# Owen-Liuyuxuan/FSNet

Hardware: AMD Instinct MI355X
Metric: training samples/sec (3-frame triplets) at 192x640, ResNet-18 depth+pose (higher is better)
Workload: dtype bf16; 1 GPU; KITTI Eigen-Zhou-shaped synthetic triplets, ResNet-18 depth+pose, 192x640, bf16, batch 12/GPU, full step (fwd+loss+bwd+clip35+Adam); inputs HBM-resident, no H2D in the timed region; global_batch=12, parallelism=dp1, encoder_pass=two chains (depth and pose encoder on two streams), autotune_steps=0, hipgraph_replays=557

## Files before the change

fsnet_amd/csrc/bn.hip:

```cpp
#include "bn_coeffs.h"
#include <algorithm>
#include <cstdlib>

namespace {

__device__ __forceinline__ int pow2_shift(int v) { return (v & (v - 1)) == 0 ? __ffs(v) - 1 : -1; }
__device__ __forceinline__ void split_vec(long i, int CG, int sh, int& cg, long& m) {
  if (sh >= 0) { cg = (int)(i & (CG - 1)); m = i >> sh; }
  else if (i < (1L << 31)) { const unsigned u = (unsigned)i, q = u / (unsigned)CG; cg = (int)(u - q * CG); m = q; }
  else { cg = (int)(i % CG); m = i / CG; }
}
__device__ __forceinline__ void split_row(long m, int H, int W, long& n, int& h, int& w) {
  if (m < (1L << 31)) {
    const unsigned u = (unsigned)m, q = u / (unsigned)W, nn = q / (unsigned)H;
    w = (int)(u - q * W); h = (int)(q - nn * H); n = nn;
  } else {
    w = (int)(m % W); const long q = m / W; h = (int)(q % H); n = q / H;
  }
}


constexpr int MAXC = 2048;

template <typename A> __host__ __device__ inline int bn_groups(const A& a) { return a.groups > 1 ? a.groups : 1; }
// ... 481 lines not shown
  }
  reduce_tail<V>(p, red, s1, s2, z, CG, cgl, pl, c, true);
}

template <typename T>
__global__ __launch_bounds__(256) void bn_bwd_apply_pool_kernel(const FsDual<FsBnBwdArgs, FsNoGeom> d) {
  extern __shared__ float bn_smem[];
  int G, z;
  const FsBnBwdArgs& p = bn_problem(d, G, z);
  constexpr int V = VecN<T>::N;
  const int C = p.C, CG = C / V, PL = 256 / CG;
  float* s_a = bn_smem; float* s_b = bn_smem + C; float* s_k = bn_smem + 2 * C;
  float* s_mean = bn_smem + 3 * C; float* s_istd = bn_smem + 4 * C; float* s_sh = bn_smem + 5 * C;
  const double* sums = p.sums + (long)z * FS_STAT_SLOTS * 2 * C;
  const double* sums_local = p.sums_local ? p.sums_local + (long)z * FS_STAT_SLOTS * 2 * C : nullptr;
  bn_bwd_coeffs(p, sums, sums_local, G, z, 0, C, true, bn_smem);
  const int cgl = threadIdx.x % CG, pl = threadIdx.x / CG, c = cgl * V;
  const T* __restrict__ yv = reinterpret_cast<const T*>(p.y);
  const T* __restrict__ xv = reinterpret_cast<const T*>(p.x);
  T* __restrict__ dx = reinterpret_cast<T*>(p.dx);
  const int H = p.H, W = p.W, Ho = H >> 1, Wo = W >> 1;
  const unsigned Qg = (unsigned)(p.M / G) / 4;
  for (unsigned q = blockIdx.x * PL + pl; q < Qg; q += gridDim.x * PL) {
    const unsigned qq = (unsigned)z * Qg + q, r = qq / (unsigned)Wo, nn = r / (unsigned)Ho;
    const int b = (int)(qq - r * Wo), a = (int)(r - nn * Ho);
    float g[4][V], x[4][V];
#pragma unroll
    for (int k = 0; k < 4; ++k) loadv<T>(xv + (((long)nn * H + 2 * a + (k >> 1)) * W + 2 * b + (k & 1)) * C + c, x[k]);
    pool_quad<T>(p, nn, a, b, c, g);
#pragma unroll
    for (int k = 0; k < 4; ++k) {
      const long m = ((long)nn * H + 2 * a + (k >> 1)) * W + 2 * b + (k & 1);
      pool_mask<T>(p, yv, m, c, x[k], s_k + c, s_sh + c, g[k]);
      float o[V];
#pragma unroll
      for (int j = 0; j < V; ++j) o[j] = bn_dx(g[k][j], x[k][j], s_mean[c + j], s_istd[c + j], s_k[c + j], s_a[c + j], s_b[c + j]);
      storev<T>(dx + m * C + c, o);
    }
  }
}

template <typename T, int CGB, bool POOL = false>
__global__ __launch_bounds__(256) void bn_bwd_reduce_kernel(const FsDual<FsBnBwdArgs, FsNoGeom> d) {
  int G, z;
  const FsBnBwdArgs& p = bn_problem(d, G, z);
  constexpr int V = VecN<T>::N;
  constexpr int PL = 256 / CGB;
  __shared__ float red[2][V][256];
  const int C = p.C, CG = C / V;
  const int cgl = threadIdx.x % CGB, pl = threadIdx.x / CGB;
  const int cg = blockIdx.y * CGB + cgl;
  const bool act = cg < CG;
  const int c = cg * V;
  const T* __restrict__ dout = reinterpret_cast<const T*>(p.dout);
  const T* __restrict__ yv = reinterpret_cast<const T*>(p.y);
  const T* __restrict__ xv = reinterpret_cast<const T*>(p.x);
  const long Mg = p.M / G, m_end = (z + 1) * Mg;
  float mean[V], istd[V], s1[V], s2[V];
#pragma unroll
  for (int j = 0; j < V; ++j) { mean[j] = act ? p.save_mean[z * C + c + j] : 0.f; istd[j] = act ? p.save_invstd[z * C + c + j] : 0.f; s1[j] = 0.f; s2[j] = 0.f; }
  if constexpr (POOL) {
    if (act) {
      float sc[V], sh[V];
#pragma unroll
      for (int j = 0; j < V; ++j) {
        sc[j] = p.gamma[c + j] * istd[j];
        sh[j] = (p.beta ? p.beta[c + j] : 0.f) - mean[j] * sc[j];
      }
      const long stride = (long)gridDim.x * PL;
      long m = z * Mg + (long)blockIdx.x * PL + pl;
      for (; m + stride < m_end; m += 2 * stride) {
        float g0[V], x0[V], g1[V], x1[V];
        loadv<T>(xv + m * C + c, x0);
        loadv<T>(xv + (m + stride) * C + c, x1);
        pool_grad<T>(p, m, c, g0);
        pool_grad<T>(p, m + stride, c, g1);
        pool_mask<T>(p, yv, m, c, x0, sc, sh, g0);
        pool_mask<T>(p, yv, m + stride, c, x1, sc, sh, g1);
#pragma unroll
        for (int j = 0; j < V; ++j) {
          s1[j] += g0[j] + g1[j];
          s2[j] += g0[j] * (x0[j] - mean[j]) * istd[j] + g1[j] * (x1[j] - mean[j]) * istd[j];
        }
      }
      for (; m < m_end; m += stride) {
        float g0[V], x0[V];
        loadv<T>(xv + m * C + c, x0);
        pool_grad<T>(p, m, c, g0);
        pool_mask<T>(p, yv, m, c, x0, sc, sh, g0);
#pragma unroll
        for (int j = 0; j < V; ++j) { s1[j] += g0[j]; s2[j] += g0[j] * (x0[j] - mean[j]) * istd[j]; }
      }
    }
  } else
  if (act) {
    const long stride = (long)gridDim.x * PL;
    long m = z * Mg + (long)blockIdx.x * PL + pl;
    if (dense_grad(p)) {
      const bool relu = p.relu != 0;
      long left = m < m_end ? (m_end - m + stride - 1) / stride : 0;
      long off = m * C + c;
      const long step = stride * C;
      uint4 d0, x0, y0, d1, x1, y1, d2, x2, y2;
      d0 = x0 = y0 = d1 = x1 = y1 = d2 = x2 = y2 = make_uint4(0, 0, 0, 0);
      auto req = [&](long o, uint4& dd, uint4& xx, uint4& yy) {
        dd = *reinterpret_cast<const uint4*>(dout + o); xx = *reinterpret_cast<const uint4*>(xv + o);
        if (relu) yy = *reinterpret_cast<const uint4*>(yv + o);
      };
      if constexpr (sizeof(T) == 2) {
        if (left > 0) req(off, d0, x0, y0);
        if (left > 1) req(off + step, d1, x1, y1);
        if (left > 2) req(off + 2 * step, d2, x2, y2);
        while (left > 0) {
          float g[V], xr[V];
          Unit<T>::unpack(d0, g); Unit<T>::unpack(x0, xr);
          if (relu) {
            float yy[V];
            Unit<T>::unpack(y0, yy);
#pragma unroll
            for (int j = 0; j < V; ++j) g[j] = yy[j] > 0.f ? g[j] : 0.f;
          }
          d0 = d1; x0 = x1; y0 = y1; d1 = d2; x1 = x2; y1 = y2;
          --left; off += step;
          if (left > 2) req(off + 2 * step, d2, x2, y2);
#pragma unroll
          for (int j = 0; j < V; ++j) { s1[j] += g[j]; s2[j] += g[j] * (xr[j] - mean[j]) * istd[j]; }
        }
        m = m_end;
      }
    }
    for (; m + stride < m_end; m += 2 * stride) {
      float g0[V], g1[V], x0[V], x1[V];
      masked_grad<T>(p, dout, yv, m, c, g0);
      masked_grad<T>(p, dout, yv, m + stride, c, g1);
      loadv<T>(xv + m * C + c, x0);
      loadv<T>(xv + (m + stride) * C + c, x1);
#pragma unroll
      for (int j = 0; j < V; ++j) {
        s1[j] += g0[j] + g1[j];
        s2[j] += g0[j] * (x0[j] - mean[j]) * istd[j] + g1[j] * (x1[j] - mean[j]) * istd[j];
      }
    }
    for (; m < m_end; m += stride) {
      float g0[V], x0[V];
      masked_grad<T>(p, dout, yv, m, c, g0);
      loadv<T>(xv + m * C + c, x0);
#pragma unroll
      for (int j = 0; j < V; ++j) { s1[j] += g0[j]; s2[j] += g0[j] * (x0[j] - mean[j]) * istd[j]; }
    }
  }
  reduce_tail<V>(p, red, s1, s2, z, CGB, cgl, pl, c, act);
}

template <typename T, bool POOL = false>
__global__ __launch_bounds__(256) void bn_bwd_apply_kernel(const FsDual<FsBnBwdArgs, FsNoGeom> d) {
  extern __shared__ float bn_smem[];
  int G, z;
  const FsBnBwdArgs& p = bn_problem(d, G, z);
  const int C = p.C;
  constexpr int V = VecN<T>::N;
  const int CG = C / V, cg_sh = pow2_shift(CG);
  const int SCG = gridDim.y > 1 ? 32 : CG, scg_sh = gridDim.y > 1 ? 5 : cg_sh;
  const int SC = SCG * V, c0 = (int)blockIdx.y * SC;
  float* s_a = bn_smem; float* s_b = bn_smem + SC; float* s_k = bn_smem + 2 * SC;
  float* s_mean = bn_smem + 3 * SC; float* s_istd = bn_smem + 4 * SC;
  const int Mg = p.M / G;
  const double* sums = p.sums + (long)z * FS_STAT_SLOTS * 2 * C;
  const double* sums_local = p.sums_local ? p.sums_local + (long)z * FS_STAT_SLOTS * 2 * C : nullptr;
  const T* __restrict__ dout = reinterpret_cast<const T*>(p.dout);
  const T* __restrict__ yv = reinterpret_cast<const T*>(p.y);
  const T* __restrict__ xv = reinterpret_cast<const T*>(p.x);
  const long total = (long)Mg * SCG;
  const long i0 = (long)blockIdx.x * 256 + threadIdx.x;
  float pg[V], px[V];
  if (i0 < total) {
    int cg; long m;
    split_vec(i0, SCG, scg_sh, cg, m);
    m += (long)z * Mg;
    if constexpr (POOL) pool_grad<T>(p, m, c0 + cg * V, pg);
    else masked_grad<T>(p, dout, yv, m, c0 + cg * V, pg);
    loadv<T>(xv + m * C + c0 + cg * V, px);
  }
  bn_bwd_coeffs(p, sums, sums_local, G, z, c0, SC, POOL, bn_smem);
  T* __restrict__ dx = reinterpret_cast<T*>(p.dx);
  T* __restrict__ gout = reinterpret_cast<T*>(p.g_out);
  const long stride = (long)gridDim.x * 256;
  if constexpr (!POOL) {
    if (scg_sh >= 0 && dense_grad(p)) {
      if (i0 >= total) return;
      const int cl = (int)(i0 & (SCG - 1)) * V;
      const long rows = stride >> scg_sh, step = rows * C;
      long off = ((long)z * Mg + (i0 >> scg_sh)) * C + c0 + cl;
      long left = (total - i0 + stride - 1) / stride;
      const bool relu = p.relu != 0;
      float ka[V], kb[V], kk[V], km[V], ki[V];
#pragma unroll
      for (int j = 0; j < V; ++j) { ka[j] = s_a[cl + j]; kb[j] = s_b[cl + j]; kk[j] = s_k[cl + j]; km[j] = s_mean[cl + j]; ki[j] = s_istd[cl + j]; }
      uint4 d1, x1, y1, d2, x2, y2;
      d1 = x1 = y1 = d2 = x2 = y2 = make_uint4(0, 0, 0, 0);
      if (left > 1) {
        d1 = *reinterpret_cast<const uint4*>(dout + off + step); x1 = *reinterpret_cast<const uint4*>(xv + off + step);
        if (relu) y1 = *reinterpret_cast<const uint4*>(yv + off + step);
      }
      if (left > 2) {
        d2 = *reinterpret_cast<const uint4*>(dout + off + 2 * step); x2 = *reinterpret_cast<const uint4*>(xv + off + 2 * step);
        if (relu) y2 = *reinterpret_cast<const uint4*>(yv + off + 2 * step);
      }
      float g[V], xr[V], o[V];
#pragma unroll
      for (int j = 0; j < V; ++j) { g[j] = pg[j]; xr[j] = px[j]; }
      for (;;) {
#pragma unroll
        for (int j = 0; j < V; ++j) o[j] = bn_dx(g[j], xr[j], km[j], ki[j], kk[j], ka[j], kb[j]);
        storev<T>(dx + off, o);
        if (gout) storev<T>(gout + off, g);
        if (--left == 0) break;
        off += step;
        Unit<T>::unpack(d1, g); Unit<T>::unpack(x1, xr);
        if (relu) {
          float yy[V];
          Unit<T>::unpack(y1, yy);
#pragma unroll
          for (int j = 0; j < V; ++j) g[j] = yy[j] > 0.f ? g[j] : 0.f;
        }
        d1 = d2; x1 = x2; y1 = y2;
        if (left > 2) {
          d2 = *reinterpret_cast<const uint4*>(dout + off + 2 * step); x2 = *reinterpret_cast<const uint4*>(xv + off + 2 * step);
          if (relu) y2 = *reinterpret_cast<const uint4*>(yv + off + 2 * step);
        }
      }
      return;
    }
  }
  for (long i = i0; i < total; i += stride) {
    int cg; long m;
    split_vec(i, SCG, scg_sh, cg, m);
    m += (long)z * Mg;
    const int cl = cg * V, c = c0 + cl;
    float g[V], xr[V], o[V];
#pragma unroll
    for (int j = 0; j < V; ++j) { g[j] = pg[j]; xr[j] = px[j]; }
    if (i + stride < total) {
      int cg2; long m2;
      split_vec(i + stride, SCG, scg_sh, cg2, m2);
      m2 += (long)z * Mg;
      if constexpr (POOL) pool_grad<T>(p, m2, c0 + cg2 * V, pg);
      else masked_grad<T>(p, dout, yv, m2, c0 + cg2 * V, pg);
      loadv<T>(xv + m2 * C + c0 + cg2 * V, px);
    }
    if constexpr (POOL) pool_mask<T>(p, yv, m, c, xr, s_k + cl, bn_smem + 5 * SC + cl, g);
#pragma unroll
    for (int j = 0; j < V; ++j) o[j] = bn_dx(g[j], xr[j], s_mean[cl + j], s_istd[cl + j], s_k[cl + j], s_a[cl + j], s_b[cl + j]);
    storev<T>(dx + m * C + c, o);
    if (gout) storev<T>(gout + m * C + c, g);
  }
}

int bn_slabs(int CG) { return (CG > 32 && (CG & (CG - 1)) == 0) ? CG / 32 : 1; }

bool bn_pool_quads(int CG) { return CG >= 1 && CG <= 32 && (CG & (CG - 1)) == 0; }

int grid_for(long items) {
  long b = (items + 255) / 256;
  const long cap = 512;
  if (b > cap) b = cap;
  if (b < 1) b = 1;
  return (int)b;
}

}

extern "C" int fs_bn_finalize(const FsBnApplyArgs* a, float* scale, float* shift, void* stream) {
  if (!a || !a->gamma || !a->beta || !a->save_mean || !a->save_invstd || !scale || !shift) return FS_EINVAL;
  if (!a->stats && (!a->running_mean || !a->running_var)) return FS_EINVAL;
  if (a->C <= 0 || a->C > MAXC || a->gamma2) return FS_EINVAL;
  const int G = bn_groups(*a);
  if (G > 1 && !a->stats) return FS_EINVAL;
  hipLaunchKernelGGL(bn_finalize_kernel, dim3((a->C + 255) / 256, G), dim3(256), 0, reinterpret_cast<hipStream_t>(stream),
                     *a, scale, shift);
  return fs_launch_status();
}

namespace {
int bn_apply_check(const FsBnApplyArgs* a) {
  if (!a || !a->x || (!a->y && !a->pool_y) || !a->gamma || !a->beta || !a->save_mean || !a->save_invstd) return FS_EINVAL;
  if (a->pool_y) {
    if (!a->pool_idx || !a->stats || a->res || a->gamma2 || a->pad_out || a->H <= 0 || a->W <= 0 || (a->H & 1) || (a->W & 1))
      return FS_EINVAL;
    if (a->M % (a->H * a->W) != 0 || (long)a->M * (a->C / 4) >= 0x7fffffffL) return FS_EINVAL;
    if (a->y && !dense(a->yN, a->yH, a->yW, a->H, a->W, a->C)) return FS_EINVAL;
  }
  if (!a->stats && (!a->running_mean || !a->running_var)) return FS_EINVAL;
  if (a->C % 8 != 0 || a->C > MAXC || a->M <= 0) return FS_EINVAL;
  if (a->gamma2 && (!a->res || !a->beta2 || !a->save_mean2 || !a->save_invstd2)) return FS_EINVAL;
  if (a->gamma2 && !a->stats2 && (!a->running_mean2 || !a->running_var2)) return FS_EINVAL;
  const int G = bn_groups(*a);
  if (a->M % G != 0 || (G > 1 && !a->stats)) return FS_EINVAL;
  return FS_OK;
}
int bn_bwd_check(const FsBnBwdArgs* a, bool apply) {
  if (!a || (!a->dout && !a->pool_dy) || !a->x || !a->sums || !a->save_mean || !a->save_invstd) return FS_EINVAL;
  if (apply && (!a->dx || !a->gamma)) return FS_EINVAL;
  if (a->C % 8 != 0 || a->C > MAXC || a->M <= 0) return FS_EINVAL;
  const int G = bn_groups(*a);
  if (a->M % G != 0) return FS_EINVAL;
  if (a->pool_dy) {
    if (!a->pool_idx || !a->gamma || a->fold || a->g_out || a->H <= 0 || a->W <= 0 || (a->H & 1) || (a->W & 1)) return FS_EINVAL;
    if (a->relu && !a->y && !a->beta) return FS_EINVAL;
    const long hw = (long)a->H * a->W;
    if (a->M % hw != 0 || (a->M / G) % hw != 0 || (long)a->M >= 0x7fffffffL) return FS_EINVAL;
    if (a->dout && !dense(a->gN, a->gH, a->gW, a->H, a->W, a->C)) return FS_EINVAL;
    if (a->y && !dense(a->yN, a->yH, a->yW, a->H, a->W, a->C)) return FS_EINVAL;
    return FS_OK;
  }
  if (a->relu && !a->y) return FS_EINVAL;
  return FS_OK;
}

template <typename A>
struct BnPair {
  FsDual<A, FsNoGeom> d;
  int G, G1;
  template <typename F> long larger(F extent) const {
    const long e = extent(d.a[0], G);
    return d.nprob == 2 ? std::max(e, (long)extent(d.a[1], G1)) : e;
  }
};
template <typename A, typename P, typename Check, typename Single>
bool bn_pair(const A* a, const A* b, P A::*pool, Check check, Single single, BnPair<A>& pr, int& status) {
  if ((status = check(a)) != FS_OK) return false;
  if (b) {
    if ((status = check(b)) != FS_OK) return false;
    const bool pooled = a->*pool != nullptr;
    if (b->C != a->C || pooled != (b->*pool != nullptr) || (pooled && (a->H != b->H || a->W != b->W))) {
      status = single(a);
      if (status == FS_OK) status = single(b);
      return false;
    }
  }
  pr.d.a[0] = *a; pr.d.a[1] = b ? *b : *a;
  pr.d.g[0].unused = pr.d.g[1].unused = 0;
  pr.d.nb0 = pr.G = bn_groups(*a);
  pr.d.nprob = b ? 2 : 1;
  pr.G1 = b ? bn_groups(*b) : 0;
  return true;
}

template <typename T> struct Elem { using type = T; };
template <typename F>
int by_dtype(int dtype, F launch) {
  if (dtype == FS_DTYPE_BF16) launch(Elem<bf16>{});
  else if (dtype == FS_DTYPE_F32) launch(Elem<float>{});
  else return FS_EINVAL;
  return fs_launch_status();
}
int dtype_lanes(int dtype) { return dtype == FS_DTYPE_BF16 ? 8 : 4; }

dim3 quad_grid(const long Qg, int CG, long cap, int groups) {
  return dim3((unsigned)std::min<long>((Qg + 256 / CG - 1) / (256 / CG), cap), 1, groups);
}
template <typename A> long quads_per_group(const A& x, int G) { return (x.M / G) / 4; }
template <typename A> long rows_per_group(const A& x, int G) { return x.M / G; }

template <int CGB>
int launch_reduce(const BnPair<FsBnBwdArgs>& pr, int dtype, hipStream_t st, int CG, long rows_per_block, long max_blocks) {
  const long Mg = pr.larger(rows_per_group<FsBnBwdArgs>);
  const dim3 grid((unsigned)std::min<long>((Mg + rows_per_block - 1) / rows_per_block, max_blocks), (CG + CGB - 1) / CGB,
                  pr.G + pr.G1);
  return by_dtype(dtype, [&](auto e) {
    using T = typename decltype(e)::type;
    if (pr.d.a[0].pool_dy) hipLaunchKernelGGL((bn_bwd_reduce_kernel<T, CGB, true>), grid, dim3(256), 0, st, pr.d);
    else hipLaunchKernelGGL((bn_bwd_reduce_kernel<T, CGB>), grid, dim3(256), 0, st, pr.d);
  });
}
}

extern "C" int fs_bn_apply2(const FsBnApplyArgs* a, const FsBnApplyArgs* b, int dtype, void* stream) {
  BnPair<FsBnApplyArgs> pr;
  int r;
  if (!bn_pair(a, b, &FsBnApplyArgs::pool_y, bn_apply_check,
               [&](const FsBnApplyArgs* x) { return fs_bn_apply2(x, nullptr, dtype, stream); }, pr, r)) return r;
  hipStream_t st = reinterpret_cast<hipStream_t>(stream);
  const int vec = dtype_lanes(dtype), nz = pr.G + pr.G1;
  const long items = pr.larger([&](const FsBnApplyArgs& x, int G) { return (long)(x.M / G) * (x.C / vec); });
  if (a->pool_y) {
    dim3 pgrid(std::min(2 * grid_for(items / 4), (int)((items / 4 + 255) / 256)), 1, nz);
    if (pgrid.x < 1) pgrid.x = 1;
    const unsigned plds = 2u * a->C * sizeof(float);
    return by_dtype(dtype, [&](auto e) {
      hipLaunchKernelGGL(bn_apply_pool_kernel<typename decltype(e)::type>, pgrid, dim3(256), plds, st, pr.d);
    });
  }
  const int nslab = bn_slabs(a->C / vec);
  dim3 grid(std::min(grid_for(items / nslab), std::max(32, grid_for(1L << 40) / nslab)), nslab, nz);
  const unsigned lds = ((a->gamma2 || (b && b->gamma2)) ? 4u : 2u) * (a->C / nslab) * sizeof(float);
  return by_dtype(dtype, [&](auto e) {
    hipLaunchKernelGGL(bn_apply_kernel<typename decltype(e)::type>, grid, dim3(256), lds, st, pr.d);
  });
}

extern "C" int fs_bn_apply(const FsBnApplyArgs* a, int dtype, void* stream) { return fs_bn_apply2(a, nullptr, dtype, stream); }

extern "C" int fs_bn_bwd_reduce2(const FsBnBwdArgs* a, const FsBnBwdArgs* b, int dtype, void* stream) {
  BnPair<FsBnBwdArgs> pr;
  int r;
  if (!bn_pair(a, b, &FsBnBwdArgs::pool_dy, [](const FsBnBwdArgs* x) { return bn_bwd_check(x, false); },
               [&](const FsBnBwdArgs* x) { return fs_bn_bwd_reduce2(x, nullptr, dtype, stream); }, pr, r)) return r;
  hipStream_t st = reinterpret_cast<hipStream_t>(stream);
  const int CG = a->C / dtype_lanes(dtype), nz = pr.G + pr.G1;
  if (a->pool_dy && bn_pool_quads(CG)) {
    const dim3 grid = quad_grid(pr.larger(quads_per_group<FsBnBwdArgs>), CG, 1024, nz);
    return by_dtype(dtype, [&](auto e) {
      hipLaunchKernelGGL(bn_bwd_reduce_pool_kernel<typename decltype(e)::type>, grid, dim3(256), 0, st, pr.d);
    });
  }
  const long wide_cap = std::max<long>(32, std::min<long>(512, 1024 / ((long)((CG + 31) / 32) * nz)));
  if (CG >= 32) return launch_reduce<32>(pr, dtype, st, CG, 16, wide_cap);
  if (CG >= 8) return launch_reduce<8>(pr, dtype, st, CG, 64, 1024);
  if (CG >= 4) return launch_reduce<4>(pr, dtype, st, CG, 128, 1024);
  return launch_reduce<2>(pr, dtype, st, CG, 256, 1024);
}

extern "C" int fs_bn_bwd_reduce(const FsBnBwdArgs* a, int dtype, void* stream) { return fs_bn_bwd_reduce2(a, nullptr, dtype, stream); }

extern "C" int fs_bn_bwd_apply2(const FsBnBwdArgs* a, const FsBnBwdArgs* b, int dtype, void* stream) {
  BnPair<FsBnBwdArgs> pr;
  int r;
  if (!bn_pair(a, b, &FsBnBwdArgs::pool_dy, [](const FsBnBwdArgs* x) { return bn_bwd_check(x, true); },
               [&](const FsBnBwdArgs* x) { return fs_bn_bwd_apply2(x, nullptr, dtype, stream); }, pr, r)) return r;
  hipStream_t st = reinterpret_cast<hipStream_t>(stream);
  const int vec = dtype_lanes(dtype), CG = a->C / vec, nz = pr.G + pr.G1;
  const int nslab = a->pool_dy ? 1 : bn_slabs(CG);
  const unsigned lds = (a->pool_dy ? 6u : 5u) * (a->C / nslab) * sizeof(float);
  if (a->pool_dy && bn_pool_quads(CG)) {
    const dim3 qgrid = quad_grid(pr.larger(quads_per_group<FsBnBwdArgs>), CG, 2048, nz);
    return by_dtype(dtype, [&](auto e) {
      hipLaunchKernelGGL(bn_bwd_apply_pool_kernel<typename decltype(e)::type>, qgrid, dim3(256), lds, st, pr.d);
    });
  }
  const long items = pr.larger([&](const FsBnBwdArgs& x, int G) { return (long)(x.M / G) * (x.C / vec); });
  dim3 grid(std::min(grid_for(items / nslab), std::max(32, grid_for(1L << 40) / nslab)), nslab, nz);
  return by_dtype(dtype, [&](auto e) {
    using T = typename decltype(e)::type;
    if (a->pool_dy) hipLaunchKernelGGL((bn_bwd_apply_kernel<T, true>), grid, dim3(256), lds, st, pr.d);
    else hipLaunchKernelGGL((bn_bwd_apply_kernel<T>), grid, dim3(256), lds, st, pr.d);
  });
}

extern "C" int fs_bn_bwd_apply(const FsBnBwdArgs* a, int dtype, void* stream) { return fs_bn_bwd_apply2(a, nullptr, dtype, stream); }
```

fsnet_amd/csrc/heads.hip:

```cpp
#include "common.h"
#include "fsnet_hip_internal.h"
#include <algorithm>

namespace {

template <int K>
__device__ __forceinline__ void head_fwd_row(const float* __restrict__ logits, const float* sb, float* __restrict__ depth,
                                             float* __restrict__ disp, long m, int Cl, float inv_rng, float max_d,
                                             float sc = 0.f, float min_d = 0.f) {
  float v[K];
  float mx = -INFINITY;
#pragma unroll
  for (int k = 0; k < K; k += 4) {
    float4 t = *reinterpret_cast<const float4*>(logits + m * Cl + k);
    v[k] = t.x; v[k + 1] = t.y; v[k + 2] = t.z; v[k + 3] = t.w;
  }
#pragma unroll
  for (int k = 0; k < K; ++k) { v[k] = fminf(fmaxf(v[k], -10.f), 10.f); mx = fmaxf(mx, v[k]); }
  float se = 0.f, sd = 0.f;
#pragma unroll
  for (int k = 0; k < K; ++k) { float e = expf(v[k] - mx); se += e; sd += e * sb[k]; }
  float d = sd / se;
  if (sc != 0.f) {
    d = d * sc;
    const float mn = min_d * sc, mx2 = max_d * sc;
    depth[m] = d;
    disp[m] = (1.f / d - 1.f / mx2) / (1.f / mn - 1.f / mx2);
    return;
  }
  depth[m] = d;
  disp[m] = (1.f / d - 1.f / max_d) * inv_rng;
}

template <int K, typename T>
__device__ __forceinline__ void head_bwd_row(const float* __restrict__ logits, const float* sb,
                                             const float* __restrict__ d_depth, const float* __restrict__ d_disp,
                                             T* __restrict__ dlogits, long m, int Cl, float inv_rng,
                                             float sc = 0.f, float min_d = 0.f, float max_d = 0.f) {
  float v[K], raw[K];
  float mx = -INFINITY;
#pragma unroll
  for (int k = 0; k < K; k += 4) {
    float4 t = *reinterpret_cast<const float4*>(logits + m * Cl + k);
    raw[k] = t.x; raw[k + 1] = t.y; raw[k + 2] = t.z; raw[k + 3] = t.w;
  }
#pragma unroll
  for (int k = 0; k < K; ++k) { v[k] = fminf(fmaxf(raw[k], -10.f), 10.f); mx = fmaxf(mx, v[k]); }
  float se = 0.f, sd = 0.f;
#pragma unroll
  for (int k = 0; k < K; ++k) { v[k] = expf(v[k] - mx); se += v[k]; sd += v[k] * sb[k]; }
  float d = sd / se;
  float g = (d_depth ? d_depth[m] : 0.f);
  if (sc != 0.f) {
    const float ds = d * sc;
    if (d_disp) g += d_disp[m] * (-1.f / (ds * ds)) / (1.f / (min_d * sc) - 1.f / (max_d * sc));
    g *= sc;
  } else if (d_disp) g += d_disp[m] * (-inv_rng / (d * d));
  float o[K];
#pragma unroll
  for (int k = 0; k < K; ++k) {
    float pk = v[k] / se;
    bool inside = raw[k] >= -10.f && raw[k] <= 10.f;
    o[k] = inside ? pk * (sb[k] - d) * g : 0.f;
  }
#pragma unroll
  for (int k = 0; k < K; k += 4) store4<T>(dlogits + m * Cl + k, &o[k]);
}

template <int K>
__global__ __launch_bounds__(256) void depth_head_fwd_kernel(const float* __restrict__ logits,
                                                             const float* __restrict__ bins, float* __restrict__ depth,
                                                             float* __restrict__ disp, long M, int Cl, float min_d,
                                                             float max_d) {
  __shared__ float sb[K];
  if (threadIdx.x < K) sb[threadIdx.x] = bins[threadIdx.x];
  __syncthreads();
  const float inv_rng = 1.f / (1.f / min_d - 1.f / max_d);
  for (long m = (long)blockIdx.x * 256 + threadIdx.x; m < M; m += (long)gridDim.x * 256)
    head_fwd_row<K>(logits, sb, depth, disp, m, Cl, inv_rng, max_d);
}

template <int K, typename T>
__global__ __launch_bounds__(256) void depth_head_bwd_kernel(const float* __restrict__ logits,
                                                             const float* __restrict__ bins,
                                                             const float* __restrict__ d_depth,
                                                             const float* __restrict__ d_disp, T* __restrict__ dlogits,
                                                             long M, int Cl, float min_d, float max_d) {
  __shared__ float sb[K];
  if (threadIdx.x < K) sb[threadIdx.x] = bins[threadIdx.x];
  __syncthreads();
  const float inv_rng = 1.f / (1.f / min_d - 1.f / max_d);
  for (long m = (long)blockIdx.x * 256 + threadIdx.x; m < M; m += (long)gridDim.x * 256)
    head_bwd_row<K, T>(logits, sb, d_depth, d_disp, dlogits, m, Cl, inv_rng);
}

struct HeadBlocks { int start[FS_HEAD_MAX + 1]; };

template <int K>
__global__ __launch_bounds__(256) void depth_head_fwd_multi_kernel(const FsHeadBatch hb, const HeadBlocks blk,
                                                                   const float* __restrict__ bins, int Cl, float min_d,
                                                                   float max_d) {
  __shared__ float sb[K];
  if (threadIdx.x < K) sb[threadIdx.x] = bins[threadIdx.x];
  __syncthreads();
  const float inv_rng = 1.f / (1.f / min_d - 1.f / max_d);
  int s = 0;
  while (s + 1 < hb.n && (int)blockIdx.x >= blk.start[s + 1]) ++s;
  const long nb = blk.start[s + 1] - blk.start[s], lb = blockIdx.x - blk.start[s];
  const long rows_img = hb.nimg > 0 ? hb.M[s] / hb.nimg : 0;
  for (long m = lb * 256 + threadIdx.x; m < hb.M[s]; m += nb * 256) {
    const float sc = hb.P2 ? hb.P2[(m / rows_img) * 12] / hb.base_fx : 0.f;
    head_fwd_row<K>(hb.logits[s], sb, hb.depth[s], hb.disp[s], m, Cl, inv_rng, max_d, sc, min_d);
  }
}

template <int K, typename T>
__global__ __launch_bounds__(256) void depth_head_bwd_multi_kernel(const FsHeadBatch hb, const HeadBlocks blk,
                                                                   const float* __restrict__ bins, int Cl, float min_d,
                                                                   float max_d) {
  __shared__ float sb[K];
  if (threadIdx.x < K) sb[threadIdx.x] = bins[threadIdx.x];
  __syncthreads();
  const float inv_rng = 1.f / (1.f / min_d - 1.f / max_d);
  int s = 0;
  while (s + 1 < hb.n && (int)blockIdx.x >= blk.start[s + 1]) ++s;
  const long nb = blk.start[s + 1] - blk.start[s], lb = blockIdx.x - blk.start[s];
  const long rows_img = hb.nimg > 0 ? hb.M[s] / hb.nimg : 0;
  for (long m = lb * 256 + threadIdx.x; m < hb.M[s]; m += nb * 256) {
    const float sc = hb.P2 ? hb.P2[(m / rows_img) * 12] / hb.base_fx : 0.f;
    head_bwd_row<K, T>(hb.logits[s], sb, hb.d_depth[s], hb.d_disp[s], reinterpret_cast<T*>(hb.dlogits[s]), m, Cl, inv_rng,
                       sc, min_d, max_d);
  }
}

struct Dual {
  float v; float d[6];
};
__device__ inline Dual dconst(float c) { Dual r; r.v = c; for (int i = 0; i < 6; ++i) r.d[i] = 0.f; return r; }
__device__ inline Dual dvar(float c, int i) { Dual r = dconst(c); r.d[i] = 1.f; return r; }
__device__ inline Dual operator+(const Dual& a, const Dual& b) { Dual r; r.v = a.v + b.v; for (int i = 0; i < 6; ++i) r.d[i] = a.d[i] + b.d[i]; return r; }
__device__ inline Dual operator-(const Dual& a, const Dual& b) { Dual r; r.v = a.v - b.v; for (int i = 0; i < 6; ++i) r.d[i] = a.d[i] - b.d[i]; return r; }
__device__ inline Dual operator*(const Dual& a, const Dual& b) { Dual r; r.v = a.v * b.v; for (int i = 0; i < 6; ++i) r.d[i] = a.d[i] * b.v + a.v * b.d[i]; return r; }
__device__ inline Dual operator/(const Dual& a, const Dual& b) { Dual r; r.v = a.v / b.v; for (int i = 0; i < 6; ++i) r.d[i] = (a.d[i] - r.v * b.d[i]) / b.v; return r; }
__device__ inline Dual dneg(const Dual& a) { Dual r; r.v = -a.v; for (int i = 0; i < 6; ++i) r.d[i] = -a.d[i]; return r; }
__device__ inline Dual dsqrt(const Dual& a) { Dual r; r.v = sqrtf(a.v); float k = r.v > 0.f ? 0.5f / r.v : 0.f; for (int i = 0; i < 6; ++i) r.d[i] = k * a.d[i]; return r; }
__device__ inline Dual dsin(const Dual& a) { Dual r; r.v = sinf(a.v); float k = cosf(a.v); for (int i = 0; i < 6; ++i) r.d[i] = k * a.d[i]; return r; }
__device__ inline Dual dcos(const Dual& a) { Dual r; r.v = cosf(a.v); float k = -sinf(a.v); for (int i = 0; i < 6; ++i) r.d[i] = k * a.d[i]; return r; }

__device__ inline void pose_matrix(const float in[6], int invert, Dual M[3][4]) {
  Dual vx = dvar(in[0], 0), vy = dvar(in[1], 1), vz = dvar(in[2], 2);
  Dual tx = dvar(in[3], 3), ty = dvar(in[4], 4), tz = dvar(in[5], 5);
  Dual angle = dsqrt(vx * vx + vy * vy + vz * vz);
  Dual den = angle + dconst(1e-7f);
  Dual x = vx / den, y = vy / den, z = vz / den;
  Dual ca = dcos(angle), sa = dsin(angle);
  Dual Cc = dconst(1.f) - ca;
  Dual xs = x * sa, ys = y * sa, zs = z * sa;
  Dual xC = x * Cc, yC = y * Cc, zC = z * Cc;
  Dual xyC = x * yC, yzC = y * zC, zxC = z * xC;
  Dual R[3][3];
  R[0][0] = x * xC + ca; R[0][1] = xyC - zs;    R[0][2] = zxC + ys;
  R[1][0] = xyC + zs;    R[1][1] = y * yC + ca; R[1][2] = yzC - xs;
  R[2][0] = zxC - ys;    R[2][1] = yzC + xs;    R[2][2] = z * zC + ca;
  if (!invert) {
    for (int i = 0; i < 3; ++i) for (int j = 0; j < 3; ++j) M[i][j] = R[i][j];
    M[0][3] = tx; M[1][3] = ty; M[2][3] = tz;
  } else {
    Dual nt[3] = {dneg(tx), dneg(ty), dneg(tz)};
    for (int i = 0; i < 3; ++i) {
      for (int j = 0; j < 3; ++j) M[i][j] = R[j][i];
      M[i][3] = R[0][i] * nt[0] + R[1][i] * nt[1] + R[2][i] * nt[2];
    }
  }
}

__global__ __launch_bounds__(64) void pose_tail_fwd_kernel(const float* __restrict__ x, float* __restrict__ axisangle,
                                                           float* __restrict__ translation, float* __restrict__ Tm,
                                                           int hw, int Cx, int nframes, int invert, float scale) {
  const int b = blockIdx.x, lane = threadIdx.x;
  const int nout = 6 * nframes;
  __shared__ float mean[64];
  for (int c = 0; c < nout; ++c) {
    float s = 0.f;
    for (int i = lane; i < hw; i += 64) s += x[((long)b * hw + i) * Cx + c];
    s = wave_sum(s);
    if (lane == 0) mean[c] = scale * (s / (float)hw);
  }
  __syncthreads();
  if (lane < nout) {
    int f = lane / 6, k = lane % 6;
    if (k < 3) axisangle[((long)b * nframes + f) * 3 + k] = mean[lane];
    else translation[((long)b * nframes + f) * 3 + (k - 3)] = mean[lane];
  }
  if (lane == 0) {
    float in[6] = {mean[0], mean[1], mean[2], mean[3], mean[4], mean[5]};
    Dual M[3][4];
    pose_matrix(in, invert, M);
    float* o = Tm + (long)b * 16;
    for (int i = 0; i < 3; ++i) for (int j = 0; j < 4; ++j) o[i * 4 + j] = M[i][j].v;
    o[12] = 0.f; o[13] = 0.f; o[14] = 0.f; o[15] = 1.f;
  }
}

template <typename T>
__global__ __launch_bounds__(64) void pose_tail_bwd_kernel(const float* __restrict__ x, const float* __restrict__ dT,
                                                           T* __restrict__ dx, int hw, int Cx, int nframes,
                                                           int invert, float scale) {
  const int b = blockIdx.x, lane = threadIdx.x;
  __shared__ float mean[8];
  __shared__ float gin[8];
  for (int c = 0; c < 6; ++c) {
    float s = 0.f;
    for (int i = lane; i < hw; i += 64) s += x[((long)b * hw + i) * Cx + c];
    s = wave_sum(s);
    if (lane == 0) mean[c] = scale * (s / (float)hw);
  }
  __syncthreads();
  if (lane == 0) {
    float in[6] = {mean[0], mean[1], mean[2], mean[3], mean[4], mean[5]};
    Dual M[3][4];
    pose_matrix(in, invert, M);
    const float* g = dT + (long)b * 16;
    for (int k = 0; k < 6; ++k) {
      float a = 0.f;
      for (int i = 0; i < 3; ++i) for (int j = 0; j < 4; ++j) a += g[i * 4 + j] * M[i][j].d[k];
      gin[k] = a * scale / (float)hw;
    }
  }
  __syncthreads();
  for (int i = lane; i < hw * Cx; i += 64) {
    int c = i % Cx;
    dx[(long)b * hw * Cx + i] = ElemTraits<T>::from_f(c < 6 ? gin[c] : 0.f);
  }
}

int grid_for(long items) {
  long b = (items + 255) / 256;
  return (int)std::max<long>(1, std::min<long>(b, 8192));
}

}

extern "C" int fs_depth_head_fwd(const float* logits, const float* bins, float* depth, float* disp, int64_t M, int K,
                                 int Cl, float min_depth, float max_depth, void* stream) {
  if (!logits || !bins || !depth || !disp || Cl < K) return FS_EINVAL;
  hipStream_t st = reinterpret_cast<hipStream_t>(stream);
  dim3 grid(grid_for(M));
  if (K == 16) hipLaunchKernelGGL(depth_head_fwd_kernel<16>, grid, dim3(256), 0, st, logits, bins, depth, disp, (long)M, Cl, min_depth, max_depth);
  else if (K == 32) hipLaunchKernelGGL(depth_head_fwd_kernel<32>, grid, dim3(256), 0, st, logits, bins, depth, disp, (long)M, Cl, min_depth, max_depth);
  else if (K == 64) hipLaunchKernelGGL(depth_head_fwd_kernel<64>, grid, dim3(256), 0, st, logits, bins, depth, disp, (long)M, Cl, min_depth, max_depth);
  else return FS_EINVAL;
  return fs_launch_status();
}

extern "C" int fs_depth_head_bwd(const float* logits, const float* bins, const float* d_depth, const float* d_disp,
                                 void* dlogits, int64_t M, int K, int Cl, float min_depth, float max_depth, int dtype,
                                 void* stream) {
  if (!logits || !bins || !dlogits || Cl < K) return FS_EINVAL;
  hipStream_t st = reinterpret_cast<hipStream_t>(stream);
  dim3 grid(grid_for(M));
#define FS_DH(KK, TT) hipLaunchKernelGGL((depth_head_bwd_kernel<KK, TT>), grid, dim3(256), 0, st, logits, bins, d_depth, d_disp, (TT*)dlogits, (long)M, Cl, min_depth, max_depth)
  if (dtype == FS_DTYPE_BF16) {
    if (K == 16) FS_DH(16, bf16); else if (K == 32) FS_DH(32, bf16); else if (K == 64) FS_DH(64, bf16); else return FS_EINVAL;
  } else if (dtype == FS_DTYPE_F32) {
    if (K == 16) FS_DH(16, float); else if (K == 32) FS_DH(32, float); else if (K == 64) FS_DH(64, float); else return FS_EINVAL;
  } else return FS_EINVAL;
#undef FS_DH
  return fs_launch_status();
}

namespace {
bool head_blocks(const FsHeadBatch* hb, bool bwd, HeadBlocks& blk, int& total) {
  if (!hb || hb->n < 1 || hb->n > FS_HEAD_MAX) return false;
  if (hb->P2 && (hb->nimg < 1 || !(hb->base_fx > 0.f))) return false;
  total = 0;
  for (int s = 0; s < hb->n; ++s) {
    if (!hb->logits[s] || hb->M[s] <= 0) return false;
    if (hb->P2 && hb->M[s] % hb->nimg != 0) return false;
    if (bwd ? !hb->dlogits[s] : (!hb->depth[s] || !hb->disp[s])) return false;
    blk.start[s] = total;
    total += grid_for(hb->M[s]);
  }
  blk.start[hb->n] = total;
  return true;
}
}

extern "C" int fs_depth_head_fwd_multi(const FsHeadBatch* hb, const float* bins, int K, int Cl, float min_depth,
                                       float max_depth, void* stream) {
  HeadBlocks blk; int total = 0;
  if (!bins || Cl < K || !head_blocks(hb, false, blk, total)) return FS_EINVAL;
  hipStream_t st = reinterpret_cast<hipStream_t>(stream);
  dim3 grid(total);
  if (K == 16) hipLaunchKernelGGL(depth_head_fwd_multi_kernel<16>, grid, dim3(256), 0, st, *hb, blk, bins, Cl, min_depth, max_depth);
  else if (K == 32) hipLaunchKernelGGL(depth_head_fwd_multi_kernel<32>, grid, dim3(256), 0, st, *hb, blk, bins, Cl, min_depth, max_depth);
  else if (K == 64) hipLaunchKernelGGL(depth_head_fwd_multi_kernel<64>, grid, dim3(256), 0, st, *hb, blk, bins, Cl, min_depth, max_depth);
  else return FS_EINVAL;
  return fs_launch_status();
}

extern "C" int fs_depth_head_bwd_multi(const FsHeadBatch* hb, const float* bins, int K, int Cl, float min_depth,
                                       float max_depth, int dtype, void* stream) {
  HeadBlocks blk; int total = 0;
  if (!bins || Cl < K || !head_blocks(hb, true, blk, total)) return FS_EINVAL;
  hipStream_t st = reinterpret_cast<hipStream_t>(stream);
  dim3 grid(total);
#define FS_DHM(KK, TT) hipLaunchKernelGGL((depth_head_bwd_multi_kernel<KK, TT>), grid, dim3(256), 0, st, *hb, blk, bins, Cl, min_depth, max_depth)
  if (dtype == FS_DTYPE_BF16) {
    if (K == 16) FS_DHM(16, bf16); else if (K == 32) FS_DHM(32, bf16); else if (K == 64) FS_DHM(64, bf16); else return FS_EINVAL;
  } else if (dtype == FS_DTYPE_F32) {
    if (K == 16) FS_DHM(16, float); else if (K == 32) FS_DHM(32, float); else if (K == 64) FS_DHM(64, float); else return FS_EINVAL;
  } else return FS_EINVAL;
#undef FS_DHM
  return fs_launch_status();
}

extern "C" int fs_pose_tail_fwd(const float* x, float* axisangle, float* translation, float* T, int B, int hw, int Cx,
                                int nframes, int invert, float scale, void* stream) {
  if (!x || !axisangle || !translation || !T || nframes < 1 || 6 * nframes > Cx || 6 * nframes > 64) return FS_EINVAL;
  hipStream_t st = reinterpret_cast<hipStream_t>(stream);
  hipLaunchKernelGGL(pose_tail_fwd_kernel, dim3(B), dim3(64), 0, st, x, axisangle, translation, T, hw, Cx, nframes, invert, scale);
  return fs_launch_status();
}

extern "C" int fs_pose_tail_bwd(const float* x, const float* dT, void* dx, int B, int hw, int Cx, int nframes,
                                int invert, float scale, int dtype, void* stream) {
  if (!x || !dT || !dx || 6 * nframes > Cx) return FS_EINVAL;
  hipStream_t st = reinterpret_cast<hipStream_t>(stream);
  if (dtype == FS_DTYPE_BF16) hipLaunchKernelGGL(pose_tail_bwd_kernel<bf16>, dim3(B), dim3(64), 0, st, x, dT, (bf16*)dx, hw, Cx, nframes, invert, scale);
  else if (dtype == FS_DTYPE_F32) hipLaunchKernelGGL(pose_tail_bwd_kernel<float>, dim3(B), dim3(64), 0, st, x, dT, (float*)dx, hw, Cx, nframes, invert, scale);
  else return FS_EINVAL;
  return fs_launch_status();
}
```

fsnet_amd/csrc/pool_upsample.hip:

```cpp
#include "common.h"
#include "fsnet_hip_internal.h"
#include <algorithm>

namespace {

struct FsPoolPair { const void* in1; void* out1; uint8_t* idx1; const void* add1; int n0; };

template <typename T>
__global__ __launch_bounds__(256) void maxpool_fwd_kernel(const T* __restrict__ x, T* __restrict__ y,
                                                          uint8_t* __restrict__ idx, int N, int H, int W, int C,
                                                          int Ho, int Wo, FsPoolPair pr) {
  constexpr int VN = VecN<T>::N;
  const int CG = C / VN;
  const long total = (long)N * Ho * Wo * CG;
  for (long i = (long)blockIdx.x * 256 + threadIdx.x; i < total; i += (long)gridDim.x * 256) {
    int cg = (int)(i % CG); long m = i / CG;
    int wo = (int)(m % Wo); long q = m / Wo; int ho = (int)(q % Ho); long n = q / Ho;
    const T* xs = x; T* ys = y; uint8_t* is = idx;
    if (n >= pr.n0) {
      n -= pr.n0; m -= (long)pr.n0 * Ho * Wo;
      xs = reinterpret_cast<const T*>(pr.in1); ys = reinterpret_cast<T*>(pr.out1); is = pr.idx1;
    }
    float best[VN];
    int bi[VN];
// ... 122 lines not shown
    if (i < ta) {
      int cg = (int)(i % CGa); long m = i / CGa;
      int x = (int)(m % w); long q = m / w; int y = (int)(q % h); long n = q / h;
      float acc[V];
#pragma unroll
      for (int j = 0; j < V; ++j) acc[j] = 0.f;
      for (int dy = 0; dy < 2; ++dy)
        for (int dx = 0; dx < 2; ++dx) {
          float g[V];
          fold_load<T, V>(dpad, n, 2 * y + dy, 2 * x + dx, H, W, C, cg * V, g);
#pragma unroll
          for (int j = 0; j < V; ++j) acc[j] += g[j];
        }
      stc<T, V>(da + m * Ca + cg * V, acc);
    } else {
      long k = i - ta;
      int cg = (int)(k % CGb); long m = k / CGb;
      int x = (int)(m % W); long q = m / W; int y = (int)(q % H); long n = q / H;
      float g[V];
      fold_load<T, V>(dpad, n, y, x, H, W, C, Ca + cg * V, g);
      stc<T, V>(db + m * Cb + cg * V, g);
    }
  }
}

template <typename T> __device__ __forceinline__ float round_to(float v);
template <> __device__ __forceinline__ float round_to<float>(float v) { return v; }
template <> __device__ __forceinline__ float round_to<bf16>(float v) { return bf16_bits_to_f(f_to_bf16_bits(v)); }

template <typename T, int V>
__global__ __launch_bounds__(256) void upcat_pad_bwd_bn_kernel(const T* __restrict__ dpad, T* __restrict__ da,
                                                               T* __restrict__ db, int N, int h, int w, int Ca, int Cb,
                                                               const T* __restrict__ yact, const T* __restrict__ xraw,
                                                               const float* __restrict__ mean,
                                                               const float* __restrict__ invstd, double* __restrict__ sums,
                                                               const int nA) {
  const int H = 2 * h, W = 2 * w, C = Ca + Cb;
  const int CGa = Ca / V, CGb = Cb / V;
  if ((int)blockIdx.x >= nA) {
    const long tb = (long)N * H * W * CGb;
    const int bx = (int)blockIdx.x - nA, nB = (int)gridDim.x - nA;
    for (long k = (long)bx * 256 + threadIdx.x; k < tb; k += (long)nB * 256) {
      int cg = (int)(k % CGb); long m = k / CGb;
      int x = (int)(m % W); long q = m / W; int y = (int)(q % H); long n = q / H;
      float g[V];
      fold_load<T, V>(dpad, n, y, x, H, W, C, Ca + cg * V, g);
      stc<T, V>(db + m * Cb + cg * V, g);
    }
    return;
  }
  __shared__ float red[2][V][256];
  const int cg = threadIdx.x % CGa, c = cg * V;
  float mu[V], is[V], s1[V], s2[V];
#pragma unroll
  for (int j = 0; j < V; ++j) { mu[j] = mean[c + j]; is[j] = invstd[c + j]; s1[j] = 0.f; s2[j] = 0.f; }
  const long ta = (long)N * h * w * CGa;
  for (long i = (long)blockIdx.x * 256 + threadIdx.x; i < ta; i += (long)nA * 256) {
    long m = i / CGa;
    int x = (int)(m % w); long q = m / w; int y = (int)(q % h); long n = q / h;
    float acc[V], yy[V], xr[V];
    ldc<T, V>(yact + m * Ca + c, yy);
    ldc<T, V>(xraw + m * Ca + c, xr);
#pragma unroll
    for (int j = 0; j < V; ++j) acc[j] = 0.f;
    for (int dy = 0; dy < 2; ++dy)
      for (int dx = 0; dx < 2; ++dx) {
        float g[V];
        fold_load<T, V>(dpad, n, 2 * y + dy, 2 * x + dx, H, W, C, c, g);
#pragma unroll
        for (int j = 0; j < V; ++j) acc[j] += g[j];
      }
#pragma unroll
    for (int j = 0; j < V; ++j) {
      const float g = yy[j] > 0.f ? round_to<T>(acc[j]) : 0.f;
      acc[j] = g;
      s1[j] += g; s2[j] += g * (xr[j] - mu[j]) * is[j];
    }
    stc<T, V>(da + m * Ca + c, acc);
  }
#pragma unroll
  for (int j = 0; j < V; ++j) { red[0][j][threadIdx.x] = s1[j]; red[1][j][threadIdx.x] = s2[j]; }
  __syncthreads();
  const int PL = 256 / CGa;
  for (int t = threadIdx.x; t < CGa * 2 * V; t += 256) {
    const int g2 = t % CGa, kj = t / CGa, kind = kj / V, j = kj % V;
    float a = 0.f;
    for (int k = 0; k < PL; ++k) a += red[kind][j][k * CGa + g2];
    double* sl = sums + (long)(blockIdx.x % FS_STAT_SLOTS) * 2 * Ca;
    atomicAdd(sl + kind * Ca + g2 * V + j, (double)a);
  }
}

template <typename T, int VL>
__device__ __forceinline__ void channel_sum_body(const T* __restrict__ x, float* __restrict__ out, long M, int C, int Creal,
                                                 int CGB, int bx, int by, int gx) {
  __shared__ float red[VL][256];
  const int CG = C / VL;
  const int PL = 256 / CGB;
  const int cgl = threadIdx.x % CGB, pl = threadIdx.x / CGB;
  const int cg = by * CGB + cgl;
  float s[VL];
#pragma unroll
  for (int j = 0; j < VL; ++j) s[j] = 0.f;
  auto ld = [&](long m, float* v) {
    if constexpr (VL == 4) load4<T>(x + m * C + cg * 4, v);
    else loadv<T>(x + m * C + cg * VL, v);
  };
  if (cg < CG) {
    const long stride = (long)gx * PL;
    long m = (long)bx * PL + pl;
    for (; m + 3 * stride < M; m += 4 * stride) {
      float v0[VL], v1[VL], v2[VL], v3[VL];
      ld(m, v0); ld(m + stride, v1); ld(m + 2 * stride, v2); ld(m + 3 * stride, v3);
#pragma unroll
      for (int j = 0; j < VL; ++j) s[j] += (v0[j] + v1[j]) + (v2[j] + v3[j]);
    }
    for (; m < M; m += stride) {
      float v0[VL];
      ld(m, v0);
#pragma unroll
      for (int j = 0; j < VL; ++j) s[j] += v0[j];
    }
  }
#pragma unroll
  for (int j = 0; j < VL; ++j) red[j][threadIdx.x] = s[j];
  __syncthreads();
  if (cg < CG) {
    for (int j = pl; j < VL; j += PL) {
      float a = 0.f;
      for (int k = 0; k < PL; ++k) a += red[j][k * CGB + cgl];
      if (cg * VL + j < Creal) atomicAdd(out + cg * VL + j, a);
    }
  }
}

template <typename T, int VL>
__global__ __launch_bounds__(256) void channel_sum_kernel(const T* __restrict__ x, float* __restrict__ out, long M,
                                                          int C, int Creal, int CGB) {
  channel_sum_body<T, VL>(x, out, M, C, Creal, CGB, (int)blockIdx.x, (int)blockIdx.y, (int)gridDim.x);
}

constexpr int FS_CSUM_MAX = 16;
struct CsumBatch { const void* x[FS_CSUM_MAX]; float* out[FS_CSUM_MAX]; long M[FS_CSUM_MAX]; int C[FS_CSUM_MAX], Creal[FS_CSUM_MAX],
                   CGB[FS_CSUM_MAX], gx[FS_CSUM_MAX], start[FS_CSUM_MAX + 1]; int n; };
template <typename T, int VL>
__global__ __launch_bounds__(256) void channel_sum_multi_kernel(const CsumBatch c) {
  int k = 0;
  while (k + 1 < c.n && (int)blockIdx.x >= c.start[k + 1]) ++k;
  const int lb = (int)blockIdx.x - c.start[k];
  const int gx = c.gx[k];
  channel_sum_body<T, VL>(reinterpret_cast<const T*>(c.x[k]), c.out[k], c.M[k], c.C[k], c.Creal[k], c.CGB[k], lb % gx, lb / gx, gx);
}

int grid_for(long items) {
  long b = (items + 255) / 256;
  return (int)std::max<long>(1, std::min<long>(b, 8192));
}

}

#define DISPATCH(KERNEL, GRID, ...)                                                                   \
  if (dtype == FS_DTYPE_BF16) hipLaunchKernelGGL(KERNEL<bf16>, GRID, dim3(256), 0, st, __VA_ARGS__);  \
  else if (dtype == FS_DTYPE_F32) hipLaunchKernelGGL(KERNEL<float>, GRID, dim3(256), 0, st, __VA_ARGS__); \
  else return FS_EINVAL;

extern "C" int fs_maxpool_fwd2(const void* x, void* y, uint8_t* idx, int N, const void* x1, void* y1, uint8_t* idx1, int N1,
                               int H, int W, int C, int dtype, void* stream) {
  const int vn = dtype == FS_DTYPE_BF16 ? 8 : 4;
  if (!x || !y || !idx || C % vn != 0 || N <= 0) return FS_EINVAL;
  if (x1 && (!y1 || !idx1 || N1 <= 0)) return FS_EINVAL;
  if (!x1) N1 = 0;
  hipStream_t st = reinterpret_cast<hipStream_t>(stream);
  int Ho = (H + 2 - 3) / 2 + 1, Wo = (W + 2 - 3) / 2 + 1;
  const FsPoolPair pr{x1, y1, idx1, nullptr, x1 ? N : 0x7fffffff};
  dim3 grid(grid_for((long)(N + N1) * Ho * Wo * (C / vn)));
  if (dtype == FS_DTYPE_BF16)
    hipLaunchKernelGGL(maxpool_fwd_kernel<bf16>, grid, dim3(256), 0, st, (const bf16*)x, (bf16*)y, idx, N + N1, H, W, C, Ho, Wo, pr);
  else if (dtype == FS_DTYPE_F32)
    hipLaunchKernelGGL(maxpool_fwd_kernel<float>, grid, dim3(256), 0, st, (const float*)x, (float*)y, idx, N + N1, H, W, C, Ho, Wo, pr);
  else return FS_EINVAL;
  return fs_launch_status();
}

extern "C" int fs_maxpool_fwd(const void* x, void* y, uint8_t* idx, int N, int H, int W, int C, int dtype,
                              void* stream) {
  return fs_maxpool_fwd2(x, y, idx, N, nullptr, nullptr, nullptr, 0, H, W, C, dtype, stream);
}

extern "C" int fs_maxpool_bwd2(const void* dy, const uint8_t* idx, const void* addend, void* dx, int N, const void* dy1,
                               const uint8_t* idx1, const void* addend1, void* dx1, int N1, int H, int W, int C, int dtype,
                               void* stream) {
  const int vn = dtype == FS_DTYPE_BF16 ? 8 : 4;
  if (!dy || !dx || !idx || C % vn != 0 || N <= 0) return FS_EINVAL;
  if (dy1 && (!dx1 || !idx1 || N1 <= 0)) return FS_EINVAL;
  if (!dy1) N1 = 0;
  hipStream_t st = reinterpret_cast<hipStream_t>(stream);
  int Ho = (H + 2 - 3) / 2 + 1, Wo = (W + 2 - 3) / 2 + 1;
  const FsPoolPair pr{dy1, dx1, const_cast<uint8_t*>(idx1), addend1, dy1 ? N : 0x7fffffff};
  dim3 grid(grid_for((long)(N + N1) * H * W * (C / vn)));
  if (dtype == FS_DTYPE_BF16)
    hipLaunchKernelGGL(maxpool_bwd_kernel<bf16>, grid, dim3(256), 0, st, (const bf16*)dy, idx, (const bf16*)addend, (bf16*)dx, N + N1, H, W, C, Ho, Wo, pr);
  else if (dtype == FS_DTYPE_F32)
    hipLaunchKernelGGL(maxpool_bwd_kernel<float>, grid, dim3(256), 0, st, (const float*)dy, idx, (const float*)addend, (float*)dx, N + N1, H, W, C, Ho, Wo, pr);
  else return FS_EINVAL;
  return fs_launch_status();
}

extern "C" int fs_maxpool_bwd(const void* dy, const uint8_t* idx, const void* addend, void* dx, int N, int H, int W,
                              int C, int dtype, void* stream) {
  return fs_maxpool_bwd2(dy, idx, addend, dx, N, nullptr, nullptr, nullptr, nullptr, 0, H, W, C, dtype, stream);
}

extern "C" int fs_upcat_pad_fwd(const void* a, const void* b, void* out, int N, int h, int w, int Ca, int Cb,
                                int dtype, void* stream) {
  if (!a || !out || (Cb > 0 && !b) || Ca % 4 != 0 || Cb % 4 != 0) return FS_EINVAL;
  hipStream_t st = reinterpret_cast<hipStream_t>(stream);
  const bool wide = dtype == FS_DTYPE_BF16 && Ca % 8 == 0 && Cb % 8 == 0;
  dim3 grid(grid_for((long)N * (2 * h + 2) * (2 * w + 2) * ((Ca + Cb) / (wide ? 8 : 4))));
  if (wide)
    hipLaunchKernelGGL((upcat_pad_fwd_kernel<bf16, 8>), grid, dim3(256), 0, st, (const bf16*)a, (const bf16*)b, (bf16*)out, N, h, w, Ca, Cb);
  else if (dtype == FS_DTYPE_BF16)
    hipLaunchKernelGGL((upcat_pad_fwd_kernel<bf16, 4>), grid, dim3(256), 0, st, (const bf16*)a, (const bf16*)b, (bf16*)out, N, h, w, Ca, Cb);
  else if (dtype == FS_DTYPE_F32)
    hipLaunchKernelGGL((upcat_pad_fwd_kernel<float, 4>), grid, dim3(256), 0, st, (const float*)a, (const float*)b, (float*)out, N, h, w, Ca, Cb);
  else return FS_EINVAL;
  return fs_launch_status();
}

extern "C" int fs_upcat_pad_bwd(const void* dpad, void* da, void* db, int N, int h, int w, int Ca, int Cb, int dtype,
                                void* stream) {
  if (!dpad || !da || (Cb > 0 && !db) || Ca % 4 != 0 || Cb % 4 != 0) return FS_EINVAL;
  hipStream_t st = reinterpret_cast<hipStream_t>(stream);
  const bool wide = dtype == FS_DTYPE_BF16 && Ca % 8 == 0 && Cb % 8 == 0;
  const int V = wide ? 8 : 4;
  dim3 grid(grid_for((long)N * h * w * (Ca / V) + (long)N * 4 * h * w * (Cb / V)));
  if (wide)
    hipLaunchKernelGGL((upcat_pad_bwd_kernel<bf16, 8>), grid, dim3(256), 0, st, (const bf16*)dpad, (bf16*)da, (bf16*)db, N, h, w, Ca, Cb);
  else if (dtype == FS_DTYPE_BF16)
    hipLaunchKernelGGL((upcat_pad_bwd_kernel<bf16, 4>), grid, dim3(256), 0, st, (const bf16*)dpad, (bf16*)da, (bf16*)db, N, h, w, Ca, Cb);
  else if (dtype == FS_DTYPE_F32)
    hipLaunchKernelGGL((upcat_pad_bwd_kernel<float, 4>), grid, dim3(256), 0, st, (const float*)dpad, (float*)da, (float*)db, N, h, w, Ca, Cb);
  else return FS_EINVAL;
  return fs_launch_status();
}

extern "C" int fs_upcat_pad_bwd_bn(const void* dpad, void* da, void* db, int N, int h, int w, int Ca, int Cb, const void* y,
                                   const void* x, const float* mean, const float* invstd, double* sums, int dtype,
                                   void* stream) {
  if (!dpad || !da || (Cb > 0 && !db) || !y || !x || !mean || !invstd || !sums || Ca % 4 != 0 || Cb % 4 != 0 || Ca <= 0)
    return FS_EINVAL;
  hipStream_t st = reinterpret_cast<hipStream_t>(stream);
  const bool wide = dtype == FS_DTYPE_BF16 && Ca % 8 == 0 && Cb % 8 == 0;
  const int V = wide ? 8 : 4;
  const int CGa = Ca / V;
  if (CGa > 256 || 256 % CGa != 0) return FS_EINVAL;
  const long ta = (long)N * h * w * CGa, tb = (long)N * 4 * h * w * (Cb / V);
  const int nA = (int)std::max<long>(1, std::min<long>((ta + 511) / 512, 512));
  const int nB = Cb > 0 ? grid_for(tb) : 0;
  dim3 grid(nA + nB);
  if (wide)
    hipLaunchKernelGGL((upcat_pad_bwd_bn_kernel<bf16, 8>), grid, dim3(256), 0, st, (const bf16*)dpad, (bf16*)da, (bf16*)db, N, h, w, Ca, Cb,
                       (const bf16*)y, (const bf16*)x, mean, invstd, sums, nA);
  else if (dtype == FS_DTYPE_BF16)
    hipLaunchKernelGGL((upcat_pad_bwd_bn_kernel<bf16, 4>), grid, dim3(256), 0, st, (const bf16*)dpad, (bf16*)da, (bf16*)db, N, h, w, Ca, Cb,
                       (const bf16*)y, (const bf16*)x, mean, invstd, sums, nA);
  else if (dtype == FS_DTYPE_F32)
    hipLaunchKernelGGL((upcat_pad_bwd_bn_kernel<float, 4>), grid, dim3(256), 0, st, (const float*)dpad, (float*)da, (float*)db, N, h, w, Ca, Cb,
                       (const float*)y, (const float*)x, mean, invstd, sums, nA);
  else return FS_EINVAL;
  return fs_launch_status();
}

extern "C" int fs_channel_sum_multi(const void* const* x, float* const* out, const int64_t* M, const int32_t* C,
                                    const int32_t* Creal, int n, int dtype, void* stream) {
  if (!x || !out || !M || !C || !Creal || n < 1 || n > FS_CSUM_MAX) return FS_EINVAL;
  const int es = dtype == FS_DTYPE_BF16 ? 2 : 4;
  const int VW = 16 / es;
  CsumBatch b;
  int blocks = 0;
  bool wide = true;
  for (int i = 0; i < n; ++i) {
    if (!x[i] || !out[i] || C[i] % 4 != 0 || M[i] <= 0) return FS_EINVAL;
    wide = wide && (C[i] % VW == 0 && VW != 4);
  }
  const int VL = wide ? VW : 4;
  for (int i = 0; i < n; ++i) {
    const int CG = C[i] / VL;
    int CGB = 1;
    while (CGB < CG && CGB < 64) CGB <<= 1;
    const int PL = 256 / CGB;
    const int gx = (int)std::max<long>(1, std::min<long>((M[i] + 4L * PL - 1) / (4L * PL), 256));
    const int gy = (CG + CGB - 1) / CGB;
    b.x[i] = x[i]; b.out[i] = out[i]; b.M[i] = M[i]; b.C[i] = C[i]; b.Creal[i] = Creal[i]; b.CGB[i] = CGB; b.gx[i] = gx;
    b.start[i] = blocks;
    blocks += gx * gy;
  }
  b.start[n] = blocks; b.n = n;
  hipStream_t st = reinterpret_cast<hipStream_t>(stream);
  if (dtype == FS_DTYPE_BF16) {
    if (wide) hipLaunchKernelGGL((channel_sum_multi_kernel<bf16, 8>), dim3(blocks), dim3(256), 0, st, b);
    else hipLaunchKernelGGL((channel_sum_multi_kernel<bf16, 4>), dim3(blocks), dim3(256), 0, st, b);
  } else if (dtype == FS_DTYPE_F32) {
    hipLaunchKernelGGL((channel_sum_multi_kernel<float, 4>), dim3(blocks), dim3(256), 0, st, b);
  } else return FS_EINVAL;
  return fs_launch_status();
}

extern "C" int fs_channel_sum(const void* x, float* out, int64_t M, int C, int Creal, int dtype, void* stream) {
  if (!x || !out || C % 4 != 0 || M <= 0) return FS_EINVAL;
  hipStream_t st = reinterpret_cast<hipStream_t>(stream);
  const int es = dtype == FS_DTYPE_BF16 ? 2 : 4;
// ... 17 lines not shown
```

fsnet_amd/engine/nets.py:

```python
import os
import weakref

import torch

from ..hip import ops
from ..hip.binding import raw_stream
from ..hip.conv import ConvOp, run_specs
from .runtime import RT, grad_of

STAT_SLOTS = ops.STAT_SLOTS
FOLD_BN = os.environ.get("FSNET_AMD_BN_FOLD", "1").strip().lower() not in ("0", "off", "false", "no")


class StatsPool:

    def __init__(self, device, capacity=1 << 21):
        self.buf = torch.zeros(capacity, dtype=torch.float64, device=device)
        self.off = 0
        self.high = 0
        self.dirty = False
        self.epoch = -1
        ops.register_prezero(self, StatsPool._prezero, device)

    def _prezero(self):
        self.off = 0
        self.epoch = ops.PREZERO_EPOCH[0]
        if not self.dirty:
            return []
        self.dirty = False
        return [self.buf[:self.high]]

    def reset(self):
        if self.dirty:
            self.buf[:self.high].zero_()
            self.dirty = False
        self.off = 0

    def span(self, a, b):
        if a is None or b is None or a.untyped_storage().data_ptr() != self.buf.untyped_storage().data_ptr() \
                or b.untyped_storage().data_ptr() != self.buf.untyped_storage().data_ptr():
            return None
        oa, ob = a.storage_offset(), b.storage_offset()
        if oa + a.numel() != ob:
            return None
        return self.buf[oa:ob + b.numel()]

    def take(self, C, groups=1):
        n = groups * STAT_SLOTS * 2 * C
        shape = (STAT_SLOTS, 2, C) if groups == 1 else (groups, STAT_SLOTS, 2, C)
        if self.off + n > self.buf.numel():
            return torch.zeros(shape, dtype=torch.float64, device=self.buf.device)
        v = self.buf[self.off:self.off + n].view(shape)
        self.off += n
        self.high = max(self.high, self.off)
        self.dirty = True
        return v


_PENDING_JOIN = set()
_PENDING_KEEP = []
_DEFERRED = {}
_CALLBACK_QUEUED = [None]
_ACTIVE_CHAINS = set()


_STREAM_OBJS = {}


def _current_stream(device=None):
    from ..hip.binding import raw_stream
    idx = torch.cuda.current_device() if device is None or device.index is None else device.index
    key = (idx, raw_stream(idx))
    s = _STREAM_OBJS.get(key)
    if s is None:
        s = _STREAM_OBJS[key] = torch.cuda.current_stream(idx)
    return s


def _run_param_grads(*item, bias_later=None):
    lanes = item[1] if item[0] == "lanes" else [item]
    run_specs([op.wgrad_spec(dc, x, gw, pro=pro) for (op, dc, x, gw, gb, nb, pro) in lanes])
    for (op, dc, x, gw, gb, nb, pro) in lanes:
        if gb is not None:
            if bias_later is not None:
                bias_later.append((dc, gb, nb))
            else:
                ops.channel_sum(dc, gb, nb)


_INLINE_BIAS = {}


def _inline_bias_list(dev):
    if not (RT.dp is not None and dev.type == "cuda"):
        return None
    cur = _current_stream(dev)
    return _INLINE_BIAS.setdefault(cur.cuda_stream, (cur, []))[1]


def drop_inline_bias():
    for ent in _INLINE_BIAS.values():
        ent[1].clear()


def flush_inline_bias(cur=None):
    for key in ([cur.cuda_stream] if cur is not None else list(_INLINE_BIAS.keys())):
        ent = _INLINE_BIAS.get(key)
        if ent is None or not ent[1]:
            continue
        chain, items = ent
        with torch.cuda.stream(chain):
            ops.channel_sum_multi(items)
        items.clear()


def accumulate_param_grads_multi(cls, ops_, dcs, xs, pros):
    lanes = []
    for cl, op, dc, x, pro in zip(cls, ops_, dcs, xs, pros):
        gw = grad_of(cl.m.weight)
        gb = grad_of(cl.m.bias) if cl.m.bias is not None else None
        if gw is None:
            if gb is not None:
                ops.channel_sum(dc, gb, cl.m.bias.numel())
            continue
        lanes.append((op, dc, x, gw, gb, cl.m.bias.numel() if gb is not None else 0, pro))
    if not lanes:
        return
    item = lanes[0] if len(lanes) == 1 else ("lanes", lanes)
    dc0 = lanes[0][1]
    mode = RT.wgrad_streams if (dc0.is_cuda and RT.overlap and (RT.dp is None or RT.dp.wgrad_companions)) else 0
    if mode:
        _defer_param_grads(_current_stream(dc0.device), item)
        return
    _run_param_grads(*item, bias_later=_inline_bias_list(dc0.device))


def _drop_stale():
    if _CALLBACK_QUEUED[0] is not None and _CALLBACK_QUEUED[0] != torch._C._current_graph_task_id():
        for stale in _DEFERRED.values():
            stale[1].clear()
        _ACTIVE_CHAINS.clear()
        _LATE.clear()
        _AT_END.clear()


def _defer_param_grads(cur, item):
    _drop_stale()
    ent = _DEFERRED.get(cur.cuda_stream)
    if ent is None:
        ent = _DEFERRED[cur.cuda_stream] = (cur, [])
    ent[1].append(item)
    _ACTIVE_CHAINS.add(cur.cuda_stream)
    _queue_end_of_backward()
    if len(ent[1]) >= (RT.wgrad_flush_even if RT.even_chains else RT.wgrad_flush):
        flush_deferred(cur)


_BATCH_NO = [0]
HANDOVERS = {"late": 0, "shared": 0}
_ENCODER_END = [False]
_AT_END = []
_LATE = []
_CHAINS_BEGUN = [None, []]


def _issue_batch(chain, ws, mine, ev=None):
    if ev is None:
        ws.wait_stream(chain)
    else:
        ws.wait_event(ev)
    with torch.cuda.stream(ws):
        if RT._marks is not None:
            _BATCH_NO[0] += 1
            tag = "wg.%s.%d" % ("pose" if RT.is_side(chain) else "depth", _BATCH_NO[0])
            RT.mark(tag + ".start")
        sums = []
        for it in mine:
            _run_param_grads(*it, bias_later=sums)
        if sums:
            ops.channel_sum_multi(sums)
        if RT._marks is not None:
            RT.mark(tag + ".end(%d)" % len(mine))
    _PENDING_JOIN.add((chain, ws))


def _position(chain):
    import ctypes as C
    from ..hip.binding import check, lib
    tok = C.c_ulonglong(0)
    check(lib.fs_capture_position(C.c_void_p(chain.cuda_stream), C.byref(tok)), "fs_capture_position")
    return tok.value


def issue_late(chain=None, advanced=False):
    if not _LATE:
        return
    mine = [e for e in _LATE if chain is None or e[1].cuda_stream == chain.cuda_stream]
    if advanced and mine:
        here = _position(chain)
        mine = [e for e in mine if e[4] != here]
    if not mine:
        return
    ids = {id(e) for e in mine}
    _LATE[:] = [e for e in _LATE if id(e) not in ids]
    for ent in mine:
        if ent[2] is None:
            ent[3](ent[0])
        else:
            _issue_batch(ent[1], ent[2], ent[3], ev=ent[0])


def issue_advanced(device):
    if _LATE:
        _drop_stale()
        issue_late(_current_stream(device), advanced=True)


def late_call(chain, fn):
    if not (RT.wgrad_late and torch.cuda.is_current_stream_capturing() and torch._C._current_graph_task_id() >= 0):
        return False
    _drop_stale()
    issue_late(chain, advanced=True)
    ev = torch.cuda.Event()
    ev.record(chain)
    _LATE.append((ev, chain, None, fn, _position(chain)))
    _queue_end_of_backward()
    return True


def flush_deferred(cur=None, now=False):
    late = (RT.wgrad_late and not now and torch.cuda.is_current_stream_capturing()
            and torch._C._current_graph_task_id() >= 0)
    for key in ([cur.cuda_stream] if cur is not None else list(_DEFERRED.keys())):
        ent = _DEFERRED.get(key)
        if ent is None or not ent[1]:
            continue
        chain, items = ent
        issue_late(chain, advanced=late)
        ws = RT.companion_stream(chain.device, chain)[1]
        ev = None
        capturing = late or torch.cuda.is_current_stream_capturing()
        if capturing:
            ev = torch.cuda.Event()
            ev.record(chain)
        mine = list(items)
        if (RT.wgrad_balance and RT.even_chains and capturing and _ENCODER_END[0] and RT.dp is None and not RT.is_side(chain)
                and len(items) >= 2 and torch._C._current_graph_task_id() >= 0):
            side = RT.side_stream(chain.device)
            others = [side, RT.companion_stream(chain.device, side)[1]][:RT.wgrad_balance]
            n = 1 + len(others)
            _AT_END.append((ev, chain, [(o, items[1 + k::n]) for k, o in enumerate(others)]))
            HANDOVERS["shared"] += 1
            mine = items[0::n]
        if late:
            _LATE.append((ev, chain, ws, mine, _position(chain)))
            HANDOVERS["late"] += 1
        else:
            _issue_batch(chain, ws, mine, ev=ev)
        _PENDING_KEEP.extend(items)
        ent[1].clear()
    if not late:
        issue_late(cur)


def chain_ends(device):
    if (RT.wgrad_late and (_LATE or _AT_END) and device.type == "cuda" and torch.cuda.is_current_stream_capturing()
            and torch._C._current_graph_task_id() >= 0):
        RT.nop(device)
        issue_late(_current_stream(device))


def chain_begins(device):
    if not (RT.wgrad_late and device.type == "cuda" and RT.overlap and RT.wgrad_streams
            and torch.cuda.is_current_stream_capturing()):
        return
    task = torch._C._current_graph_task_id()
    if task < 0:
        return
    _drop_stale()
    if _CHAINS_BEGUN[0] != task:
        _CHAINS_BEGUN[0], _CHAINS_BEGUN[1] = task, []
    cur = _current_stream(device)
    begun = _CHAINS_BEGUN[1]
    if any(c.cuda_stream == cur.cuda_stream for c in begun):
        return
    begun.append(cur)
    if len(begun) == 2:
        first = begun[0]
        ws = RT.companion_stream(device, first)[1]
        ws.wait_stream(cur)
        with torch.cuda.stream(ws):
            RT.nop(device)
        _PENDING_JOIN.add((first, ws))


def _end_of_backward():
    _CALLBACK_QUEUED[0] = None
    flush_tail()
    flush_inline_bias()
    flush_deferred(now=True)
    for ev, chain, parts in _AT_END:
        for ws, mine in parts:
            if mine:
                _issue_batch(chain, ws, mine, ev=ev)
    _AT_END.clear()
    _ENCODER_END[0] = False
    _ACTIVE_CHAINS.clear()
    _BATCH_NO[0] = 0
    join_companions()


def join_companions():
    if not _PENDING_JOIN:
        return
    if torch.cuda.is_current_stream_capturing():
        return
    for cur, ws in list(_PENDING_JOIN):
        cur.wait_stream(ws)
    _PENDING_JOIN.clear()
    _PENDING_KEEP.clear()


_TAIL_SINK = [None]
_TAIL = []


def _queue_end_of_backward():
    task = torch._C._current_graph_task_id()
    if _CALLBACK_QUEUED[0] != task:
        torch.autograd.Variable._execution_engine.queue_callback(_end_of_backward)
        _CALLBACK_QUEUED[0] = task


def defer_to_tail(items, runner, device):
    if _TAIL and _CALLBACK_QUEUED[0] != torch._C._current_graph_task_id():
        _TAIL.clear()
    chain = _current_stream(device)
    ev = torch.cuda.Event()
    ev.record(chain)
    runner.tail_pending = True
    _TAIL.append((ev, chain, items, runner))
    _queue_end_of_backward()


def flush_tail():
    for ev, chain, items, runner in _TAIL:
        side = RT.side_stream(chain.device)
        side.wait_event(ev)
        with torch.cuda.stream(side):
            sums = []
            for it in items:
                _run_param_grads(*it, bias_later=sums)
            if sums:
                ops.channel_sum_multi(sums)
            runner.tail_pending = False
            if RT.dp is not None and runner.m._pending == 0:
                RT.dp.grads_ready(runner.m)
        _PENDING_JOIN.add((chain, side))
        _PENDING_KEEP.extend(items)
    _TAIL.clear()


def pending_companions():
    return {ws for _, ws in _PENDING_JOIN}


def join_companions_final():
    flush_inline_bias()
    flush_deferred(now=True)
    issue_late()
    if not _PENDING_JOIN:
        return
    cur = torch.cuda.current_stream()
    for ws in {ws for _, ws in _PENDING_JOIN}:
        cur.wait_stream(ws)
    _PENDING_JOIN.clear()
    _PENDING_KEEP.clear()


_PACK_REGISTRY = {}
_PACK_TABLES = {}


def pack_everything(arena=None):
    for key in list(_PACK_REGISTRY.keys()):
        pack_all(key, arena)


_PACK_PENDING = {}


def pack_everything_async(arena):
    dev = arena.data.device if arena is not None else None
    if not (RT.pack_overlap and RT.overlap and dev is not None and dev.type == "cuda"):
        _PACK_PENDING.clear()
        pack_everything(arena)
        if arena is not None:
            arena.flush_zero()
        return
    cur = _current_stream(dev)
    ps = RT.pack_stream(dev)
    ps.wait_stream(cur)
    with torch.cuda.stream(ps):
        pack_everything(arena)
        ops.prezero_all(dev)
    arena.flush_zero()
    _PACK_PENDING[dev.index] = (ps, {ps.cuda_stream})


def join_pack(device):
    ent = _PACK_PENDING.get(device.index)
    if ent is None:
        return
    cur = _current_stream(device)
    if cur.cuda_stream in ent[1]:
        return
    cur.wait_stream(ent[0])
    ent[1].add(cur.cuda_stream)


def pack_all(key, arena=None):
    import ctypes as C
    from ..hip.binding import FsPackDesc, lib, check, stream_ptr
    from ..hip.conv import dtype_code
    dtype, device = key
    refs = _PACK_REGISTRY.get(key, [])
    alive = [(r, r()) for r in refs]
    if any(l is None for _, l in alive):
        refs[:] = [r for r, l in alive if l is not None]
    layers = [l for _, l in alive if l is not None and l._version() != l._packed and l.m.weight.is_cuda
              and (arena is None or arena.owns(l.m.weight))]
    if not layers:
        return
    sig = tuple((l.m.weight.data_ptr(), l._op.w_f.data_ptr(), l._op.w_d.data_ptr() if l._op.need_dgrad else 0,
                 l._op.Co, l._op.Ci, l._op.R, l._op.S, l._op.stride) for l in layers)
    ent = _PACK_TABLES.get((key, sig))
    if ent is None:
        arr = (FsPackDesc * len(layers))()
        blocks = 0
        for d, l in zip(arr, layers):
            op, w = l._op, l.m.weight
            assert w.dtype == torch.float32 and w.data.is_contiguous()
            d.w, d.dst_f = w.data_ptr(), op.w_f.data_ptr()
            d.Co, d.Ci, d.R, d.S = op.Co, op.Ci, op.R, op.S
            d.rows_f, d.cs_f, d.k_f = op.Co_p, op.Ci_p, op.kf_p
            if op.need_dgrad:
                d.dst_d, d.rows_d, d.cs_d, d.k_d = op.w_d.data_ptr(), op.rows_d, op.Co_p, op.kd_p
            else:
                d.dst_d, d.rows_d, d.cs_d, d.k_d = None, 0, 1, 1
            d.tap_order_d = 1 if getattr(op, "s2_classes", False) else 0
            d.block_start = blocks
            blocks += int(lib.fs_pack_tile_blocks(op.Co, op.Ci, op.R, op.S))
        raw = bytes(arr)
        tab = torch.frombuffer(bytearray(raw), dtype=torch.uint8).to(device)
        ent = _PACK_TABLES[(key, sig)] = (tab, len(layers), blocks)
    tab, n, blocks = ent
    check(lib.fs_pack_weights_multi(tab.data_ptr(), n, blocks, dtype_code(dtype), stream_ptr()), "pack_weights_multi")
    for l in layers:
        l._after_pack(device)


class ConvLayer:

    def __init__(self, conv, valid_over_padded=False, need_dgrad=True):
        self.m = conv
        k = conv.kernel_size
        self.R, self.S = int(k[0]), int(k[1])
        s = conv.stride
        self.stride = int(s[0]) if isinstance(s, (tuple, list)) else int(s)
        p = conv.padding
        pad = int(p[0]) if isinstance(p, (tuple, list)) else int(p)
        self.pad = 0 if valid_over_padded else pad
        self.need_dgrad = need_dgrad
        self._op = None
        self._key = None
        self._owner = None
        self._packed = None
        self._bias = None

    def ready(self, dtype, device):
        key = (dtype, device)
        if _PACK_PENDING:
            join_pack(device)
        if self._key != key or self._owner != id(self):
            w = self.m.weight
            self._op = ConvOp(w.shape[1], w.shape[0], self.R, self.S, self.stride, self.pad, dtype, device,
                              need_dgrad=self.need_dgrad)
            self._key, self._packed, self._owner = key, None, id(self)
            _PACK_REGISTRY.setdefault(key, []).append(weakref.ref(self))
        if self._version() != self._packed:
            pack_all(key)
        return self._op

    def _version(self):
        w = self.m.weight
        return (w._version, RT.weights_epoch, w.data_ptr())

    def _after_pack(self, device):
        b = self.m.bias
        if b is not None:
            if self._op.Co_p == b.numel():
                self._bias = b.data
            else:
                if self._bias is None or self._bias.numel() != self._op.Co_p or self._bias.data_ptr() == b.data_ptr():
                    self._bias = torch.zeros(self._op.Co_p, dtype=torch.float32, device=device)
                self._bias[: b.numel()].copy_(b.data)
        self._packed = self._version()

    @property
    def bias(self):
        return self._bias

    def accumulate_param_grads(self, op, dc, x, pro=None):
        gw = grad_of(self.m.weight)
        gb = grad_of(self.m.bias) if self.m.bias is not None else None
        if gw is None:
            if gb is not None:
                ops.channel_sum(dc, gb, self.m.bias.numel())
            return
        item = (op, dc, x, gw, gb, self.m.bias.numel() if gb is not None else 0, pro)
        if _TAIL_SINK[0] is not None:
            _TAIL_SINK[0].append(item)
            return
        mode = RT.wgrad_streams if (dc.is_cuda and RT.overlap and (RT.dp is None or RT.dp.wgrad_companions)) else 0
        if mode:
            _defer_param_grads(_current_stream(dc.device), item)
            return
        _run_param_grads(*item, bias_later=_inline_bias_list(dc.device))


def bn_tensors(bn):
    c = bn.__dict__.get("_fs_tensors")
    w = bn.weight
    if c is None or c[0] != w.data_ptr() or c[1] != bn.running_mean.data_ptr():
        d = {"weight": w.data, "bias": bn.bias.data, "running_mean": bn.running_mean,
             "running_var": bn.running_var, "num_batches_tracked": bn.num_batches_tracked}
        c = (w.data_ptr(), bn.running_mean.data_ptr(), d)
        bn.__dict__["_fs_tensors"] = c
    return c[2]


def _dp_stats(stats):
    if RT.dp is not None:
        RT.dp.allreduce_small(stats)
        return RT.dp.world
    return 1


_BWD_POOLS = {}


def bwd_pool_reset(device):
    key = (device, raw_stream(device.index))
    p = _BWD_POOLS.get(key)
    if p is None:
        p = _BWD_POOLS[key] = StatsPool(device)
    if p.epoch != ops.PREZERO_EPOCH[0]:
        p.reset()
    return p


def _bwd_sums(c, st):
    return _BWD_POOLS[(c.device, raw_stream(c.device.index))].take(c.shape[-1], st.groups)


def _bn_bwd(dout, y, c, bn, st, H, W, relu=True, fold=False, g_out=None, sums=None):
    dc = torch.empty_like(c)
    reduced = sums is not None
    if sums is None:
        sums = _bwd_sums(c, st)
    sync = RT.dp is not None and st.count != float("inf")
    ops.bn_backward(dout, y, c, bn.weight.data, st, dc, grad_of(bn.weight), grad_of(bn.bias), H, W, relu=relu,
                    fold=fold, g_out=g_out, sums=sums, sums_zeroed=True, reduced=reduced,
                    allreduce=(RT.dp.allreduce_small if sync else None))
    return dc


def _check_train_bn(bn, what):
    if not bn.training:
        raise NotImplementedError(
            "%s: BatchNorm in eval mode inside a training step is only implemented for the ResNet encoders "
            "(norm_eval / frozen_stages); the reference has no such switch for this module" % what)


def _exchange(pool, tensors, out_of_place=False):
    if RT.dp is None:
        return 1, list(tensors)
    base = pool.buf.untyped_storage().data_ptr() if pool is not None else None
    idx = [i for i, t in enumerate(tensors) if t is not None]
    inside = [i for i in idx if base is not None and tensors[i].untyped_storage().data_ptr() == base]
    res = list(tensors)
    runs, cur = [], []
    for i in sorted(inside, key=lambda i: tensors[i].storage_offset()):
        if cur and tensors[cur[-1]].storage_offset() + tensors[cur[-1]].numel() == tensors[i].storage_offset():
            cur.append(i)
        else:
            if cur:
                runs.append(cur)
            cur = [i]
    if cur:
        runs.append(cur)
    for run in runs:
        lo = tensors[run[0]].storage_offset()
        hi = tensors[run[-1]].storage_offset() + tensors[run[-1]].numel()
        view = pool.buf[lo:hi]
        if out_of_place:
            out = torch.empty_like(view)
            RT.dp.allreduce_small(view, out=out)
            for i in run:
                o = tensors[i].storage_offset() - lo
                res[i] = out[o:o + tensors[i].numel()].view(tensors[i].shape)
        else:
            RT.dp.allreduce_small(view)
    for i in idx:
        if i in inside:
            continue
        if out_of_place:
            res[i] = torch.empty_like(tensors[i])
            RT.dp.allreduce_small(tensors[i], out=res[i])
        else:
            RT.dp.allreduce_small(tensors[i])
    return RT.dp.world, res


class ResNetRunner:

    def __init__(self, module, first_stage=0, last_stage=None):
        self.m = module
        self.first_stage = first_stage
        self.stem = ConvLayer(module.conv1, need_dgrad=False) if first_stage == 0 else None
        self.stages = []
        for i in range(first_stage, module.num_stages if last_stage is None else last_stage):
            blocks = []
            for blk in getattr(module, "layer%d" % (i + 1)):
                if hasattr(blk, "conv3"):
                    units = [(ConvLayer(blk.conv1), blk.bn1), (ConvLayer(blk.conv2), blk.bn2),
                             (ConvLayer(blk.conv3), blk.bn3)]
                else:
                    units = [(ConvLayer(blk.conv1), blk.bn1), (ConvLayer(blk.conv2), blk.bn2)]
                ds = None
                if blk.downsample is not None:
                    ds = (ConvLayer(blk.downsample[0]), blk.downsample[1])
                blocks.append((units, ds))
            self.stages.append(blocks)
        self.pool = None
        self._solo = None

    def signature(self, train):
        sig = []

        def unit(cl, bn):
            w = cl.m.weight
            sig.append((tuple(w.shape[2:]), w.shape[0], cl.stride, cl.pad, bool(train and bn.training), w.requires_grad,
                        bn.weight.requires_grad, bn.bias.requires_grad))
        if self.stem is None:
            raise NotImplementedError("a pass entered after the stem does not run as a lane")
        unit(self.stem, self.m.bn1)
        sig[0] = sig[0][:1] + ("stem",) + sig[0][2:]
        for blocks in self.stages:
            for units, ds in blocks:
                for cl, bn in units:
                    unit(cl, bn)
                    sig[-1] = sig[-1] + (cl.m.weight.shape[1],)
                sig.append(None if ds is None else "ds")
                if ds is not None:
                    unit(*ds)
        return tuple(sig)

    def forward(self, x, train, groups=1):
        if self._solo is None:
            self._solo = EncoderPass([self])
        feats, ctx = self._solo.forward([x], train, [groups])
        return feats[0], ctx

    def backward(self, ctx, gfeats, in_mask=None):
        g = self._solo.backward(ctx, [gfeats], in_mask=(None if in_mask is None else [in_mask]))
        return None if g is None else g[0]


class EncoderPass:

    def __init__(self, runners, need_feat0=None):
        self.R = list(runners)
        self.nl = len(self.R)
        self.pool = None
        self.need_feat0 = list(need_feat0) if need_feat0 is not None else [True] * self.nl

    def _lanes(self, per_runner):
        return [per_runner(r) for r in self.R]

    def _ready(self, cls, xs):
        return [cl.ready(x.dtype, x.device) for cl, x in zip(cls, xs)]

    def _unit_fwd_fold(self, cls, bns, xs, pros):
        ops_ = self._ready(cls, xs)
        stats = [self.pool.take(op.Co_p, G) for op, G in zip(ops_, self.groups)]
        specs = [op.forward_spec(x, stats=s, stat_groups=G, pro=p) for op, x, s, G, p in zip(ops_, xs, stats, self.groups, pros)]
        run_specs(specs)
        world, _ = _exchange(self.pool, stats)
        cs, sts, fins = [], [], []
        for op, x, sp, s, G, bn in zip(ops_, xs, specs, stats, self.groups, bns):
            N, H, W, _ = x.shape
            Ho, Wo = op.out_hw(H, W)
            st = ops.BnState(op.Co_p, x.device, G, affine=True)
            st.count = float((N // G) * Ho * Wo * world)
            cs.append(sp.out); sts.append(st); fins.append((s, bn_tensors(bn), st.count, True))
        return cs, sts, fins

    def _can_fold(self, bns, nxt_cls, c_shapes, xs, train):
        if not (FOLD_BN and train and bns[0].training):
            return False
        for bn, ncl, (N, H, W), x, G in zip(bns, nxt_cls, c_shapes, xs, self.groups):
            nop = ncl.ready(x.dtype, x.device)
            if not (nop.can_fold_input(N, H, W) and nop.can_fuse_bn_bwd(N, H, W, G) and N * H * W >= 1):
                return False
        return True

    def _unit_fwd(self, cls, bns, xs, train, relu=True, res=None, ds_c=None, ds_stats=None, ds_bn=None, pros=None):
        nl = self.nl
        ops_ = self._ready(cls, xs)
        bt = train and bns[0].training
        assert all((train and bn.training) == bt for bn in bns), "lanes disagree on a BatchNorm's mode"
        assert ds_bn is None or all((train and b.training) == bt for b in ds_bn), "main and downsample BatchNorm modes differ"
        Gs = [G if bt else 1 for G in self.groups]
        stats = [self.pool.take(op.Co_p, G) if bt else None for op, G in zip(ops_, Gs)]
        pros = pros if pros is not None else [None] * nl
        specs = [op.forward_spec(x, stats=s, stat_groups=G, pro=p) for op, x, s, G, p in zip(ops_, xs, stats, Gs, pros)]
# ... 318 lines not shown
        y0 = ctx["y0"]
        add0 = [gfeats[l][0] for l in range(nl)]
        if RT.stem_flush:
            flush_deferred(_current_stream())
        if ctx.get("stem_fused"):
            dc0 = self._bn_bwd(add0, None, ctx["c0"], [r.m.bn1 for r in self.R], ctx["st0"], relu=True,
                               pools=[(dout[l], ctx["idx"][l]) for l in range(nl)])
        else:
            d0 = ops.maxpool_bwd_multi(dout, ctx["idx"], y0[0].shape[1], y0[0].shape[2], add0)
            dc0 = self._bn_bwd(d0, y0, ctx["c0"], [r.m.bn1 for r in self.R], ctx["st0"], relu=True)
        stems = [r.stem for r in self.R]
        self._param_grads(stems, self._ready(stems, xs), dc0, xs)
        RT.mark(tag + ".bwd.end")
        flush_deferred(_current_stream())
        _ENCODER_END[0] = False
        chain_ends(xs[0].device)


class DepthDecoderRunner:
    def __init__(self, module):
        self.m = module
        self.up0, self.up1, self.disp = {}, {}, {}
        for i in range(4, -1, -1):
            b0 = module.convs[("upconv", i, 0)]
            b1 = module.convs[("upconv", i, 1)]
            self.up0[i] = (ConvLayer(b0.sequence[0]), b0.sequence[1])
            self.up1[i] = (ConvLayer(b1.sequence[0], valid_over_padded=True), b1.sequence[1])
        for s in module.scales:
            self.disp[s] = ConvLayer(module.convs[("dispconv", s)], valid_over_padded=True)
        self.unc = {s: ConvLayer(module.convs[("uncertain_logz", s)], valid_over_padded=True)
                    for s in module.scales if ("uncertain_logz", s) in module.convs}
        self.pool = None
        self._border0 = None
        self.tail_pending = False

    def forward(self, feats, train, P2=None):
        m = self.m
        dev, dt = feats[-1].device, feats[-1].dtype
        if self.pool is None or self.pool.buf.device != dev:
            self.pool = StatsPool(dev)
        self.pool.reset()
        if train:
            _check_train_bn(self.up0[4][1], "DepthDecoder")
        base_fx = getattr(m, "base_fx", None)
        if base_fx is None or P2 is None:
            P2, base_fx = None, None
        else:
            P2 = P2.detach().to(dev, torch.float32).contiguous()
        ctx = {"lv": {}, "feats": feats, "P2": P2, "base_fx": base_fx}
        outs = {}
        x = feats[-1]
        K = int(m.num_output_channels)
        aside = bool(RT.overlap and dev.type == "cuda" and RT.wgrad_streams)
        cur = _current_stream(dev) if aside else None
        ws = RT.companion_stream(dev, cur)[1] if aside else None
        put_off, used_ws = None, False

        def head(i, lv, y1p):
            cld = self.disp[i]
            opd = cld.ready(dt, dev)
            lv["logits"] = opd.forward(y1p, bias=cld.bias, out_f32=True)
            if i in self.unc:
                clu = self.unc[i]
                opu = clu.ready(dt, dev)
                lv["unc"] = ops.sigmoid_head_fwd(opu.forward(y1p, bias=clu.bias, out_f32=True))

        for i in range(4, -1, -1):
            cl0, bn0 = self.up0[i]
            op0 = cl0.ready(dt, dev)
            N, h, w, _ = x.shape
            st_a = self.pool.take(op0.Co_p) if train else None
            c0 = op0.forward(x, bias=cl0.bias, stats=st_a)
            if put_off is not None:
                ev, j, lvj, yj = put_off
                ws.wait_event(ev)
                with torch.cuda.stream(ws):
                    head(j, lvj, yj)
                put_off, used_ws = None, True
            world = _dp_stats(st_a) if train else 1
            y0 = torch.empty(N, h, w, op0.Co_p, dtype=dt, device=dev)
            s0 = ops.BnState(op0.Co_p, dev)
            ops.bn_apply(c0, st_a, bn_tensors(bn0), s0, y0, h, w, N * h * w * world, relu=True, track=train)
            skip = feats[i - 1] if (m.use_skips and i > 0) else None
            xcat = ops.upcat_pad_fwd(y0, skip)
            cl1, bn1 = self.up1[i]
            op1 = cl1.ready(dt, dev)
            H2, W2 = 2 * h, 2 * w
            st_b = self.pool.take(op1.Co_p) if train else None
            c1 = op1.forward(xcat, bias=cl1.bias, stats=st_b)
            world = _dp_stats(st_b) if train else 1
            y1p = torch.empty(N, H2 + 2, W2 + 2, op1.Co_p, dtype=dt, device=dev)
            s1 = ops.BnState(op1.Co_p, dev)
            ops.bn_apply(c1, st_b, bn_tensors(bn1), s1, y1p, H2, W2, N * H2 * W2 * world, relu=True, pad_out=True,
                         track=train)
            lv = dict(x=x, c0=c0, y0=y0, s0=s0, xcat=xcat, c1=c1, y1p=y1p, s1=s1, h=h, w=w,
                      Cs=(skip.shape[3] if skip is not None else 0))
            if i in m.scales:
                if aside and i > 0:
                    ev = torch.cuda.Event()
                    ev.record(cur)
                    put_off = (ev, i, lv, y1p)
                else:
                    head(i, lv, y1p)
            ctx["lv"][i] = lv
            x = y1p[:, 1:-1, 1:-1]
        if used_ws:
            cur.wait_stream(ws)
        sc = [i for i in range(4, -1, -1) if "logits" in ctx["lv"][i]]
        if getattr(m, "sigmoid_head", False):
            a, bq = 1.0 / float(m.max_depth), 1.0 / float(m.min_depth) - 1.0 / float(m.max_depth)
            scale = None if P2 is None else (P2[:, 0, 0] / float(base_fx)).view(-1, 1, 1, 1)
            for i in sc:
                lv = ctx["lv"][i]
                u = ops.sigmoid_head_fwd(lv["logits"])
                inv = torch.reciprocal(a + bq * u)
                depth = inv if scale is None else inv * scale
                lv["sig"] = (u, depth)
                outs[i] = (lv["logits"], depth, u)
            return outs, ctx
        if sc:
            heads = ops.depth_head_fwd_multi([ctx["lv"][i]["logits"] for i in sc], m.depth_bins, K, m.min_depth,
                                             m.max_depth, P2=P2, base_fx=base_fx)
            for i, (depth, disp) in zip(sc, heads):
                lv = ctx["lv"][i]
                outs[i] = (lv["logits"], depth, disp) + ((lv["unc"],) if "unc" in lv else ())
        return outs, ctx

    def backward(self, ctx, g_depth, g_disp, g_unc=None):
        g_unc = g_unc or {}
        m = self.m
        feats = ctx["feats"]
        dev, dt = feats[-1].device, feats[-1].dtype
        K = int(m.num_output_channels)
        gfeats = [None] * 5
        bwd_pool_reset(dev)
        chain_begins(dev)
        RT.mark("ddec.bwd.start")
        tail = RT.dp is not None and RT.dp.decoder_tail and RT.overlap and dev.type == "cuda" and \
            torch._C._current_graph_task_id() >= 0
        if tail:
            _TAIL_SINK[0] = []
        try:
            return self._backward(ctx, g_depth, g_disp, g_unc, gfeats, dev, dt, K)
        finally:
            items, _TAIL_SINK[0] = _TAIL_SINK[0], None
            if items:
                defer_to_tail(items, self, dev)

    def _backward(self, ctx, g_depth, g_disp, g_unc, gfeats, dev, dt, K):
        m = self.m
        feats = ctx["feats"]

        sc = [i for i in range(5) if i in m.scales and (g_depth.get(i) is not None or g_disp.get(i) is not None)]
        dls = {}
        if sc and getattr(m, "sigmoid_head", False):
            a, bq = 1.0 / float(m.max_depth), 1.0 / float(m.min_depth) - 1.0 / float(m.max_depth)
            for i in sc:
                u, depth = ctx["lv"][i]["sig"]
                du = g_disp[i] if g_disp.get(i) is not None else torch.zeros_like(u)
                if g_depth.get(i) is not None:
                    du = du - g_depth[i] * depth * (bq / (a + bq * u))
                dls[i] = ops.sigmoid_head_bwd(u, du, self.disp[i].ready(dt, dev).Co_p, dt)
        elif sc:
            res = ops.depth_head_bwd_multi([ctx["lv"][i]["logits"] for i in sc], m.depth_bins,
                                           [g_depth.get(i) for i in sc], [g_disp.get(i) for i in sc], K, m.min_depth,
                                           m.max_depth, dt, P2=ctx["P2"], base_fx=ctx["base_fx"])
            dls = dict(zip(sc, res))

        def disp_grad(i):
            lv = ctx["lv"][i]
            y1p = lv["y1p"]
            G = None
            if i in dls:
                cld = self.disp[i]
                opd = cld.ready(dt, dev)
                dl = dls[i]
                cld.accumulate_param_grads(opd, dl, y1p)
                G = opd.dgrad(dl, y1p.shape[1], y1p.shape[2])
            if i in self.unc and g_unc.get(i) is not None:
                clu = self.unc[i]
                opu = clu.ready(dt, dev)
                dlu = ops.sigmoid_head_bwd(lv["unc"], g_unc[i], opu.Co_p, dt)
                clu.accumulate_param_grads(opu, dlu, y1p)
                G = opu.dgrad(dlu, y1p.shape[1], y1p.shape[2], addend=G)
            if G is not None:
                return G, False
            key = (tuple(y1p.shape), y1p.dtype, y1p.device)
            if self._border0 is None or self._border0[0] != key:
                self._border0 = (key, torch.zeros_like(y1p))
            return self._border0[1], True

        Gp, _ = disp_grad(0)
        for i in range(0, 5):
            issue_advanced(dev)
            lv = ctx["lv"][i]
            h, w = lv["h"], lv["w"]
            H2, W2 = 2 * h, 2 * w
            cl1, bn1 = self.up1[i]
            op1 = cl1.ready(dt, dev)
            y1_int = lv["y1p"][:, 1:-1, 1:-1]
            dc1 = _bn_bwd(Gp, y1_int, lv["c1"], bn1, lv["s1"], H2, W2, relu=True, fold=True)
            cl1.accumulate_param_grads(op1, dc1, lv["xcat"])
            dxcat = op1.dgrad(dc1, H2 + 2, W2 + 2)
            cl0, bn0 = self.up0[i]
            op0 = cl0.ready(dt, dev)
            sums0 = _bwd_sums(lv["c0"], lv["s0"])
            d_y0, d_skip = ops.upcat_pad_bwd(dxcat, h, w, op0.Co_p, lv["Cs"], bn=(lv["y0"], lv["c0"], lv["s0"], sums0))
            if i > 0 and lv["Cs"]:
                gfeats[i - 1] = d_skip
            dc0 = _bn_bwd(d_y0, None, lv["c0"], bn0, lv["s0"], h, w, sums=sums0)
            cl0.accumulate_param_grads(op0, dc0, lv["x"])
            if i < 4:
                Gp, fresh = disp_grad(i + 1)
                interior = Gp[:, 1:-1, 1:-1]
                op0.dgrad(dc0, h, w, out=interior, addend=None if fresh else interior)
            else:
                gfeats[4] = op0.dgrad(dc0, h, w)
        RT.mark("ddec.bwd.end")
        flush_deferred(_current_stream())
        return gfeats


class PoseDecoderRunner:
    def __init__(self, module):
        self.m = module
        self.cl = [ConvLayer(module.convs["squeeze"]), ConvLayer(module.convs[("pose", 0)]),
                   ConvLayer(module.convs[("pose", 1)]), ConvLayer(module.convs[("pose", 2)])]

    def forward(self, feat, invert):
        dt, dev = feat.dtype, feat.device
        acts = [feat]
        x = feat
        for j in range(3):
            op = self.cl[j].ready(dt, dev)
            x = op.forward(x, bias=self.cl[j].bias, relu=True)
            acts.append(x)
        op = self.cl[3].ready(dt, dev)
        x3 = op.forward(x, bias=self.cl[3].bias, out_f32=True)
        nf = int(self.m.num_frames_to_predict_for)
        if isinstance(invert, tuple):
            G = len(invert)
            B = x3.shape[0] // G
            outs = [ops.pose_tail_fwd(x3[g * B:(g + 1) * B], nf, invert[g]) for g in range(G)]
            aa, tr, T = (tuple(o[i] for o in outs) for i in range(3))
        else:
            aa, tr, T = ops.pose_tail_fwd(x3, nf, invert)
        return aa, tr, T, {"acts": acts, "x3": x3, "invert": invert, "nf": nf}

    def backward(self, ctx, dT):
        acts, x3 = ctx["acts"], ctx["x3"]
        dt, dev = acts[0].dtype, acts[0].device
        chain_begins(dev)
        RT.mark("pdec.bwd.start")
        if isinstance(ctx["invert"], tuple):
            G = len(ctx["invert"])
            B = x3.shape[0] // G
            d = torch.empty(x3.shape, dtype=dt, device=dev)
            for g in range(G):
                ops.pose_tail_bwd(x3[g * B:(g + 1) * B], dT[g], ctx["nf"], ctx["invert"][g], dt, out=d[g * B:(g + 1) * B])
        else:
            d = ops.pose_tail_bwd(x3, dT, ctx["nf"], ctx["invert"], dt)
        for j in range(3, -1, -1):
            op = self.cl[j].ready(dt, dev)
            xin = acts[j]
            self.cl[j].accumulate_param_grads(op, d, xin)
            d = op.dgrad(d, xin.shape[1], xin.shape[2], mask=(xin if j > 0 else None))
        if RT.lanes:
            flush_deferred(_current_stream())
        return d
```

fsnet_amd/hip/binding.py:

```python
import ctypes as C
import os

_HERE = os.path.dirname(os.path.abspath(__file__))
LIB_PATH = os.path.join(os.path.dirname(_HERE), "lib", "libfsnet_hip.so")

FS_DTYPE_F32 = 0
FS_DTYPE_BF16 = 1


class FsError(RuntimeError):
    pass


class FsConvArgs(C.Structure):
    _fields_ = [
        ("src", C.c_void_p), ("wgt", C.c_void_p), ("dst", C.c_void_p), ("bias", C.c_void_p),
        ("addend", C.c_void_p), ("mask", C.c_void_p), ("stats", C.c_void_p), ("ktab", C.c_void_p),
        ("sN", C.c_int64), ("sH", C.c_int64), ("sW", C.c_int64),
        ("dN", C.c_int64), ("dH", C.c_int64), ("dW", C.c_int64),
        ("aN", C.c_int64), ("aH", C.c_int64), ("aW", C.c_int64),
        ("mN", C.c_int64), ("mH", C.c_int64), ("mW", C.c_int64),
        ("src_bytes", C.c_int64), ("wgt_bytes", C.c_int64),
        ("Hs", C.c_int32), ("Ws", C.c_int32), ("Hd", C.c_int32), ("Wd", C.c_int32),
        ("M", C.c_int32), ("Co", C.c_int32), ("Co_p", C.c_int32), ("nchunks", C.c_int32), ("kg", C.c_int32),
        ("hb_mul", C.c_int32), ("hb_add", C.c_int32), ("sgn", C.c_int32), ("dshift", C.c_int32),
        ("relu", C.c_int32), ("out_f32", C.c_int32), ("N", C.c_int32), ("Cs", C.c_int32),
        ("wgt_row_bytes", C.c_int64),
        ("grp_imgs", C.c_int32), ("ncls", C.c_int32), ("cls_nch", C.c_int32 * 4), ("cls_ktab_off", C.c_int32 * 4), ("cls_wgt_off", C.c_int64 * 4),
        ("bnb_x", C.c_void_p), ("bnb_mean", C.c_void_p), ("bnb_invstd", C.c_void_p),
        ("stat_group_rows", C.c_int32),
        ("pro_a", C.c_void_p), ("pro_b", C.c_void_p), ("pro_c", C.c_void_p), ("pro_m", C.c_void_p), ("pro_src2", C.c_void_p),
        ("pro_mode", C.c_int32), ("pro_relu", C.c_int32), ("pro_group_imgs", C.c_int32), ("force_impl", C.c_int32),
        ("bnb_scale", C.c_void_p), ("bnb_shift", C.c_void_p),
        ("pro_stats", C.c_void_p), ("pro_stats_local", C.c_void_p),
        ("pro_gamma", C.c_void_p), ("pro_beta", C.c_void_p),
        ("pro_mean", C.c_void_p), ("pro_invstd", C.c_void_p),
        ("pro_save_a", C.c_void_p), ("pro_save_b", C.c_void_p),
        ("pro_running_mean", C.c_void_p), ("pro_running_var", C.c_void_p),
        ("pro_nbt", C.c_void_p),
        ("pro_dgamma", C.c_void_p), ("pro_dbeta", C.c_void_p),
        ("pro_dst", C.c_void_p),
        ("pro_count", C.c_double), ("pro_eps", C.c_float), ("pro_momentum", C.c_float),
        ("ds_src", C.c_void_p), ("ds_wgt", C.c_void_p), ("ds_wgt_row_bytes", C.c_int64),
    ]


class FsWgradArgs(C.Structure):
    _fields_ = [
        ("dy", C.c_void_p), ("x", C.c_void_p), ("dw", C.c_void_p), ("ktab", C.c_void_p),
        ("sN", C.c_int64), ("sH", C.c_int64), ("sW", C.c_int64),
        ("Hs", C.c_int32), ("Ws", C.c_int32), ("Hd", C.c_int32), ("Wd", C.c_int32),
        ("M", C.c_int32), ("Cd", C.c_int32),
        ("Co", C.c_int32), ("Ci", C.c_int32), ("R", C.c_int32), ("S", C.c_int32),
        ("stride", C.c_int32), ("pad", C.c_int32), ("ncolgroups", C.c_int32),
        ("workspace", C.c_void_p), ("workspace_elems", C.c_int64), ("x_bytes", C.c_int64), ("use_halo", C.c_int32),
        ("pix_per_split", C.c_int32), ("nsplit", C.c_int32), ("ws_rows", C.c_int32), ("ws_cols", C.c_int32),
        ("pro_a", C.c_void_p), ("pro_b", C.c_void_p), ("pro_relu", C.c_int32), ("pro_group_imgs", C.c_int32),
    ]


class FsPackDesc(C.Structure):
    _fields_ = [
        ("w", C.c_void_p), ("dst_f", C.c_void_p), ("dst_d", C.c_void_p),
        ("k_f", C.c_int64), ("k_d", C.c_int64), ("block_start", C.c_int64),
        ("Co", C.c_int32), ("Ci", C.c_int32), ("R", C.c_int32), ("S", C.c_int32),
        ("rows_f", C.c_int32), ("cs_f", C.c_int32), ("rows_d", C.c_int32), ("cs_d", C.c_int32),
        ("tap_order_d", C.c_int32),
    ]


class FsAugArgs(C.Structure):
    _fields_ = [
        ("src", C.c_void_p), ("minv", C.c_void_p), ("iplan", C.c_void_p), ("fplan", C.c_void_p),
        ("image", C.c_void_p), ("original", C.c_void_p), ("mask", C.c_void_p),
        ("mean", C.c_float * 3), ("std", C.c_float * 3),
        ("B", C.c_int32), ("F", C.c_int32), ("Hs", C.c_int32), ("Ws", C.c_int32), ("H", C.c_int32), ("W", C.c_int32),
    ]


class FsHeadBatch(C.Structure):
    _fields_ = [
        ("logits", C.c_void_p * 4), ("depth", C.c_void_p * 4), ("disp", C.c_void_p * 4),
        ("d_depth", C.c_void_p * 4), ("d_disp", C.c_void_p * 4), ("dlogits", C.c_void_p * 4),
        ("M", C.c_int64 * 4), ("n", C.c_int32), ("nimg", C.c_int32), ("P2", C.c_void_p), ("base_fx", C.c_float),
        ("reserved", C.c_int32),
    ]


class FsResizeArgs(C.Structure):
    _fields_ = [
        ("src", C.c_void_p), ("dims", C.c_void_p), ("image", C.c_void_p),
        ("mean", C.c_float * 3), ("std", C.c_float * 3),
        ("B", C.c_int32), ("F", C.c_int32), ("Hs", C.c_int32), ("Ws", C.c_int32), ("H", C.c_int32), ("W", C.c_int32),
        ("iplan", C.c_void_p), ("fplan", C.c_void_p), ("original", C.c_void_p), ("mask", C.c_void_p),
    ]


class FsBnApplyArgs(C.Structure):
    _fields_ = [
        ("x", C.c_void_p), ("res", C.c_void_p), ("y", C.c_void_p),
        ("stats", C.c_void_p), ("stats2", C.c_void_p),
        ("gamma", C.c_void_p), ("beta", C.c_void_p), ("gamma2", C.c_void_p), ("beta2", C.c_void_p),
        ("running_mean", C.c_void_p), ("running_var", C.c_void_p),
        ("running_mean2", C.c_void_p), ("running_var2", C.c_void_p),
        ("num_batches_tracked", C.c_void_p), ("num_batches_tracked2", C.c_void_p),
        ("save_mean", C.c_void_p), ("save_invstd", C.c_void_p),
        ("save_mean2", C.c_void_p), ("save_invstd2", C.c_void_p),
        ("count", C.c_double), ("eps", C.c_float), ("momentum", C.c_float),
        ("yN", C.c_int64), ("yH", C.c_int64), ("yW", C.c_int64),
        ("M", C.c_int32), ("C", C.c_int32), ("H", C.c_int32), ("W", C.c_int32),
        ("relu", C.c_int32), ("pad_out", C.c_int32), ("groups", C.c_int32),
        ("pool_y", C.c_void_p), ("pool_idx", C.c_void_p),
    ]


class FsBnBwdArgs(C.Structure):
    _fields_ = [
        ("dout", C.c_void_p), ("y", C.c_void_p), ("x", C.c_void_p), ("dx", C.c_void_p), ("g_out", C.c_void_p),
        ("sums", C.c_void_p), ("sums_local", C.c_void_p),
        ("gamma", C.c_void_p), ("save_mean", C.c_void_p), ("save_invstd", C.c_void_p),
        ("dgamma", C.c_void_p), ("dbeta", C.c_void_p),
        ("count", C.c_double),
        ("gN", C.c_int64), ("gH", C.c_int64), ("gW", C.c_int64),
        ("yN", C.c_int64), ("yH", C.c_int64), ("yW", C.c_int64),
        ("M", C.c_int32), ("C", C.c_int32), ("H", C.c_int32), ("W", C.c_int32),
        ("relu", C.c_int32), ("fold", C.c_int32), ("groups", C.c_int32),
        ("pool_dy", C.c_void_p), ("pool_idx", C.c_void_p), ("beta", C.c_void_p),
    ]


class FsPhotoArgs(C.Structure):
    _fields_ = [
        ("img0", C.c_void_p), ("img_src", C.c_void_p * 2), ("patched_mask", C.c_void_p),
        ("depth", C.c_void_p * 4), ("geo", C.c_void_p),
        ("pred", C.c_void_p), ("ov", C.c_void_p), ("ident", C.c_void_p), ("sel", C.c_void_p),
        ("loss_sums", C.c_void_p), ("mask_sum", C.c_void_p),
        ("d_depth", C.c_void_p * 4), ("dP", C.c_void_p), ("gout", C.c_void_p),
        ("dh", C.c_int32 * 4), ("dw", C.c_int32 * 4),
        ("B", C.c_int32), ("H", C.c_int32), ("W", C.c_int32), ("S", C.c_int32),
        ("noise_seed", C.c_int32), ("noise_seed_ptr", C.c_void_p),
        ("lut_ptrs", C.c_void_p), ("mei", C.c_void_p), ("warp_mask", C.c_void_p), ("motion_mask", C.c_void_p),
        ("no_overlap_mask", C.c_int32), ("reserved0", C.c_int32),
    ]


class FsSmoothArgs(C.Structure):
    _fields_ = [
        ("disp", C.c_void_p * 4), ("color", C.c_void_p * 4), ("d_disp", C.c_void_p * 4),
        ("disp_sum", C.c_void_p), ("sm_sums", C.c_void_p), ("dot", C.c_void_p), ("gout", C.c_void_p),
        ("h", C.c_int32 * 4), ("w", C.c_int32 * 4), ("scale_id", C.c_int32 * 4),
        ("B", C.c_int32), ("S", C.c_int32),
    ]


class FsPostOptArgs(C.Structure):
    _fields_ = [
        ("image", C.c_void_p), ("depth", C.c_void_p), ("vo", C.c_void_p), ("centres", C.c_void_p),
        ("out", C.c_void_p), ("labels", C.c_void_p), ("nseg", C.c_void_p),
        ("workspace", C.c_void_p), ("workspace_bytes", C.c_int64),
        ("rgb_mean", C.c_double * 3), ("rgb_std", C.c_double * 3),
        ("lab_dist_weight", C.c_float), ("depth_dist_weight", C.c_float), ("image_dist_weight", C.c_float),
        ("lambda0", C.c_double), ("lambda1", C.c_double), ("lambda2", C.c_double),
        ("B", C.c_int32), ("H", C.c_int32), ("W", C.c_int32), ("K", C.c_int32), ("iter_num", C.c_int32),
        ("max_points", C.c_int32),
    ]


class FsFlowArgs(C.Structure):
    _fields_ = [
        ("img0", C.c_void_p), ("img1", C.c_void_p), ("flow", C.c_void_p),
        ("workspace", C.c_void_p), ("workspace_bytes", C.c_int64),
        ("pyr_scale", C.c_double), ("poly_sigma", C.c_double),
        ("B", C.c_int32), ("H", C.c_int32), ("W", C.c_int32), ("levels", C.c_int32), ("winsize", C.c_int32),
        ("iterations", C.c_int32), ("poly_n", C.c_int32), ("flags", C.c_int32),
    ]


class FsMotionMaskArgs(C.Structure):
    _fields_ = [
        ("flow", C.c_void_p), ("P2", C.c_void_p), ("pose", C.c_void_p), ("mask", C.c_void_p),
        ("threshold", C.c_float), ("mode", C.c_int32),
        ("B", C.c_int32), ("H", C.c_int32), ("W", C.c_int32),
    ]


ABI_VERSION = 15
_lib = None


def load_library(path=None):
    global _lib
    if _lib is not None:
        return _lib
    path = path or os.environ.get("FSNET_HIP_LIB", LIB_PATH)
    import torch
    if not os.path.exists(path):
        raise FsError(
            "libfsnet_hip.so not found at %s — the HIP kernel library is required (no CPU fallback). "
            "Build it with `python fsnet_amd/csrc/build.py` or __graft_entry__.build()." % path)
    handle = C.CDLL(path)
    from . import signatures
    signatures.declare(handle)
    got = int(handle.fs_abi_version())
    if got != ABI_VERSION:
        raise FsError("libfsnet_hip.so at %s reports ABI %d, this binding is written against ABI %d (FS_ABI_VERSION "
                      "in include/fsnet_hip.h): rebuild it with `python fsnet_amd/csrc/build.py`" % (path, got, ABI_VERSION))
    _lib = handle
    return _lib


class _LazyLib:
    def __getattr__(self, name):
        return getattr(load_library(), name)


lib = _LazyLib()


def check(status, what=""):
    if status != 0:
        raise FsError("libfsnet_hip call %s failed with status %d" % (what, status))


def raw_stream(device_index=None):
    import torch
    if device_index is None:
        device_index = torch._C._cuda_getDevice()
    return torch._C._cuda_getCurrentRawStream(device_index)


def stream_ptr():
    return C.c_void_p(raw_stream())
```

fsnet_amd/hip/ops.py:

```python
import ctypes as C
import os

import torch

from .binding import (lib, check, stream_ptr, FsBnApplyArgs, FsBnBwdArgs, FsFlowArgs, FsMotionMaskArgs, FsPhotoArgs,
                      FsPostOptArgs, FsSmoothArgs)
from .conv import dtype_code, _timed, BN_EPS, BN_MOMENTUM, Spec, run_specs

STAT_SLOTS = 8


def _p(t):
    return t.data_ptr() if t is not None else None


def nchw_to_nhwc(a, b, cp, dtype, out=None):
    a = a.contiguous()
    N, Ca, H, W = a.shape
    Cb = 0
    if b is not None:
        b = b.contiguous()
        Cb = b.shape[1]
    if out is None:
        out = torch.empty(N, H, W, cp, dtype=dtype, device=a.device)
    assert out.shape == (N, H, W, cp) and out.is_contiguous() and out.dtype == dtype
    check(lib.fs_nchw_to_nhwc(a.data_ptr(), _p(b), out.data_ptr(), N, Ca, Cb, H, W, cp, dtype_code(dtype),
                              stream_ptr()), "nchw_to_nhwc")
    return out


class BnState:
    __slots__ = ("mean", "invstd", "count", "groups", "scale", "shift")

    def __init__(self, C, device, groups=1, affine=False):
        self.mean = torch.empty(groups * C, dtype=torch.float32, device=device)
        self.invstd = torch.empty(groups * C, dtype=torch.float32, device=device)
        self.count = 0.0
        self.groups = groups
        self.scale = torch.empty(groups * C, dtype=torch.float32, device=device) if affine else None
        self.shift = torch.empty(groups * C, dtype=torch.float32, device=device) if affine else None


def bn_finalize(stats, bn, st, Cc, count, track=True, groups=1):
    a = FsBnApplyArgs()
    a.groups = groups
    assert st.groups == groups and st.scale is not None
    a.stats = _p(stats)
    a.gamma, a.beta = bn["weight"].data_ptr(), bn["bias"].data_ptr()
    if track or stats is None:
        a.running_mean, a.running_var = bn["running_mean"].data_ptr(), bn["running_var"].data_ptr()
        a.num_batches_tracked = bn["num_batches_tracked"].data_ptr() if track else None
    a.save_mean, a.save_invstd = st.mean.data_ptr(), st.invstd.data_ptr()
    st.count = float(count)
    a.count, a.eps, a.momentum = float(count), BN_EPS, BN_MOMENTUM
    a.C = Cc
    check(lib.fs_bn_finalize(C.byref(a), st.scale.data_ptr(), st.shift.data_ptr(), stream_ptr()), "bn_finalize")
    return st


def bn_apply(x, stats, bn, st, y, H, W, count, **kw):
    run_specs([bn_apply_spec(x, stats, bn, st, y, H, W, count, **kw)])
    return y


def bn_apply_spec(x, stats, bn, st, y, H, W, count, relu=True, pad_out=False, res=None, stats2=None, bn2=None, st2=None,
                  track=True, groups=1, pool=None):
    a = FsBnApplyArgs()
    a.groups = groups
    assert st.groups == groups and (st2 is None or st2.groups == groups)
    Cc = x.shape[-1]
    a.x, a.res, a.y = x.data_ptr(), _p(res), _p(y)
    if pool is not None:
        assert pool[0].is_contiguous() and pool[1].is_contiguous() and pool[0].shape == (x.shape[0], H // 2, W // 2, Cc)
        assert stats is not None and res is None and bn2 is None and not pad_out and H % 2 == 0 and W % 2 == 0
        a.pool_y, a.pool_idx = pool[0].data_ptr(), pool[1].data_ptr()
    else:
        assert y is not None
    a.stats, a.stats2 = _p(stats), _p(stats2)
    a.gamma, a.beta = bn["weight"].data_ptr(), bn["bias"].data_ptr()
    if track or stats is None:
        a.running_mean, a.running_var = bn["running_mean"].data_ptr(), bn["running_var"].data_ptr()
        a.num_batches_tracked = bn["num_batches_tracked"].data_ptr()
    a.save_mean, a.save_invstd = st.mean.data_ptr(), st.invstd.data_ptr()
    st.count = float(count)
    if bn2 is not None:
        a.gamma2, a.beta2 = bn2["weight"].data_ptr(), bn2["bias"].data_ptr()
        if track or stats2 is None:
            a.running_mean2, a.running_var2 = bn2["running_mean"].data_ptr(), bn2["running_var"].data_ptr()
            a.num_batches_tracked2 = bn2["num_batches_tracked"].data_ptr() if track else None
        a.save_mean2, a.save_invstd2 = st2.mean.data_ptr(), st2.invstd.data_ptr()
        st2.count = float(count)
    a.count, a.eps, a.momentum = float(count), BN_EPS, BN_MOMENTUM
    if pad_out:
        assert y.shape[1] == H + 2 and y.shape[2] == W + 2
    if y is not None:
        a.yN, a.yH, a.yW = y.stride(0), y.stride(1), y.stride(2)
    a.M, a.C, a.H, a.W = x.shape[0] * H * W, Cc, H, W
    a.relu, a.pad_out = int(relu), int(pad_out)
    nb = x.numel() * x.element_size() * (1 + (y is not None) + (res is not None))
    if pool is not None:
        nb += pool[0].numel() * pool[0].element_size() + pool[1].numel()
    return Spec(["bn_apply"], a, dtype_code(x.dtype), "bn_apply_pool" if pool is not None else "bn_apply", nb,
                lambda: "[%d,%d,%d,%d]%s%s%s" % (x.shape[0], H, W, Cc, " +res" if res is not None else "",
                                                 " pad" if pad_out else "", " +pool" if pool is not None else ""),
                y, "bn_apply")


def bn_backward(dout, y, x, gamma, st, dx, dgamma, dbeta, H, W, relu=True, fold=False, g_out=None, sums=None,
                allreduce=None, sums_zeroed=False, reduced=False, phase="all", glob=None, pool=None):
    bn_backward_multi([dict(dout=dout, y=y, x=x, gamma=gamma, st=st, dx=dx, dgamma=dgamma, dbeta=dbeta, H=H, W=W, relu=relu,
                            fold=fold, g_out=g_out, sums=sums, sums_zeroed=sums_zeroed, reduced=reduced, glob=glob, pool=pool)],
                      allreduce=allreduce, phase=phase)
    return None if phase == "reduce" else dx


def _bn_bwd_call(dout, y, x, gamma, st, dx, dgamma, dbeta, H, W, relu=True, fold=False, g_out=None, sums=None,
                 sums_zeroed=False, reduced=False, glob=None, pool=None):
    if reduced:
        assert sums is not None and not fold and g_out is None
        relu, y = False, None
    Cc = x.shape[-1]
    a = FsBnBwdArgs()
    if sums is None:
        sums = torch.zeros(st.groups * STAT_SLOTS, 2, Cc, dtype=torch.float64, device=x.device)
    elif not sums_zeroed and not reduced:
        sums.zero_()
    a.dout, a.y, a.x, a.dx, a.g_out = _p(dout), _p(y), x.data_ptr(), _p(dx), _p(g_out)
    if pool is not None:
        assert not reduced and not fold and g_out is None and pool[0].is_contiguous() and pool[1].is_contiguous()
        assert (dout is None or dout.is_contiguous()) and (y is None or y.is_contiguous())
        a.pool_dy, a.pool_idx, a.beta = pool[0].data_ptr(), pool[1].data_ptr(), pool[2].data_ptr()
    else:
        assert dout is not None
    a.sums = sums.data_ptr()
    a.gamma, a.save_mean, a.save_invstd = gamma.data_ptr(), st.mean.data_ptr(), st.invstd.data_ptr()
    a.dgamma, a.dbeta = _p(dgamma), _p(dbeta)
    a.count = st.count
    a.groups = st.groups
    if dout is not None:
        a.gN, a.gH, a.gW = dout.stride(0), dout.stride(1), dout.stride(2)
    if y is not None:
        a.yN, a.yH, a.yW = y.stride(0), y.stride(1), y.stride(2)
    a.M, a.C, a.H, a.W = x.shape[0] * H * W, Cc, H, W
    a.relu, a.fold = int(relu), int(fold)
    shape = (x.shape[0], H, W, Cc)
    return dict(a=a, code=dtype_code(x.dtype), nb=x.numel() * x.element_size(), sums=sums, reduced=reduced, glob=glob,
                has_y=y is not None, has_g=g_out is not None, has_dout=dout is not None,
                shp=lambda: "[%d,%d,%d,%d]%s%s" % (shape + (" fold" if fold else "", " pool" if pool is not None else "")))


def bn_backward_multi(calls, allreduce=None, phase="all", span=None):
    cs = [_bn_bwd_call(**c) for c in calls]
    if phase != "apply":
        run_specs([Spec(["bn_bwd_reduce"], c["a"], c["code"], "bn_bwd_reduce", c["nb"] * (1 + c["has_dout"] + c["has_y"]), c["shp"], None,
                        "bn_bwd_reduce") for c in cs if not c["reduced"]])
    if phase == "reduce":
        return
    pending = [c for c in cs if c["glob"] is None] if allreduce is not None else []
    if len(pending) == 2 and span is not None:
        both = span(pending[0]["sums"], pending[1]["sums"])
        if both is not None:
            out = torch.empty_like(both)
            allreduce(both, out=out)
            n0 = pending[0]["sums"].numel()
            pending[0]["glob"] = out[:n0].view(pending[0]["sums"].shape)
            pending[1]["glob"] = out[n0:].view(pending[1]["sums"].shape)
            pending = []
    for c in pending:
        c["glob"] = torch.empty_like(c["sums"])
        allreduce(c["sums"], out=c["glob"])
    for c in cs:
        if c["glob"] is not None:
            c["a"].sums_local, c["a"].sums = c["sums"].data_ptr(), c["glob"].data_ptr()
    run_specs([Spec(["bn_bwd_apply"], c["a"], c["code"], "bn_bwd_apply", c["nb"] * (2 + c["has_dout"] + c["has_y"] + c["has_g"]), c["shp"],
                    None, "bn_bwd_apply") for c in cs])


def maxpool_fwd(x):
    return maxpool_fwd_multi([x])[0]


def maxpool_fwd_multi(xs):
    outs = []
    for x in xs:
        N, H, W, Cc = x.shape
        Ho, Wo = (H - 1) // 2 + 1, (W - 1) // 2 + 1
        outs.append((torch.empty(N, Ho, Wo, Cc, dtype=x.dtype, device=x.device),
                     torch.empty(N, Ho, Wo, Cc, dtype=torch.uint8, device=x.device)))
    if len(xs) == 2 and xs[0].shape[1:] == xs[1].shape[1:] and xs[0].dtype == xs[1].dtype:
        x, x1 = xs
        (y, idx), (y1, idx1) = outs
        N, H, W, Cc = x.shape
        _timed("maxpool_fwd", sum(t.numel() * t.element_size() * 1.25 + o[1].numel() for t, o in zip(xs, outs)),
               lambda: check(lib.fs_maxpool_fwd2(x.data_ptr(), y.data_ptr(), idx.data_ptr(), N, x1.data_ptr(), y1.data_ptr(),
                                                 idx1.data_ptr(), x1.shape[0], H, W, Cc, dtype_code(x.dtype), stream_ptr()),
                             "maxpool_fwd"), tag=str(tuple(x.shape)) + " || " + str(tuple(x1.shape)))
        return outs
    for x, (y, idx) in zip(xs, outs):
        N, H, W, Cc = x.shape
        _timed("maxpool_fwd", x.numel() * x.element_size() * 1.25 + idx.numel(),
               lambda: check(lib.fs_maxpool_fwd(x.data_ptr(), y.data_ptr(), idx.data_ptr(), N, H, W, Cc, dtype_code(x.dtype),
                                                stream_ptr()), "maxpool_fwd"), tag=str(tuple(x.shape)))
    return outs


def maxpool_bwd(dy, idx, H, W, addend=None):
    return maxpool_bwd_multi([dy], [idx], H, W, [addend])[0]


def maxpool_bwd_multi(dys, idxs, H, W, addends):
    dxs = [torch.empty(dy.shape[0], H, W, dy.shape[3], dtype=dy.dtype, device=dy.device) for dy in dys]
    work = lambda dx, idx, ad: dx.numel() * dx.element_size() * (1.25 + (ad is not None)) + idx.numel()
    if len(dys) == 2 and dys[0].shape[1:] == dys[1].shape[1:] and dys[0].dtype == dys[1].dtype:
        dy, dy1 = dys
        Cc = dy.shape[3]
        _timed("maxpool_bwd", sum(work(dx, i, a) for dx, i, a in zip(dxs, idxs, addends)),
               lambda: check(lib.fs_maxpool_bwd2(dy.data_ptr(), idxs[0].data_ptr(), _p(addends[0]), dxs[0].data_ptr(),
                                                 dy.shape[0], dy1.data_ptr(), idxs[1].data_ptr(), _p(addends[1]),
                                                 dxs[1].data_ptr(), dy1.shape[0], H, W, Cc, dtype_code(dy.dtype),
                                                 stream_ptr()), "maxpool_bwd"),
               tag=str(tuple(dxs[0].shape)) + " || " + str(tuple(dxs[1].shape)))
        return dxs
    for dy, idx, ad, dx in zip(dys, idxs, addends, dxs):
        _timed("maxpool_bwd", work(dx, idx, ad),
               lambda: check(lib.fs_maxpool_bwd(dy.data_ptr(), idx.data_ptr(), _p(ad), dx.data_ptr(), dy.shape[0], H, W,
                                                dy.shape[3], dtype_code(dy.dtype), stream_ptr()), "maxpool_bwd"),
               tag=str(tuple(dx.shape)))
    return dxs


def upcat_pad_fwd(a, b):
    N, h, w, Ca = a.shape
    Cb = b.shape[3] if b is not None else 0
    out = torch.empty(N, 2 * h + 2, 2 * w + 2, Ca + Cb, dtype=a.dtype, device=a.device)
    _timed("upcat_pad_fwd", (a.numel() + (b.numel() if b is not None else 0) + out.numel()) * a.element_size(),
           lambda: check(lib.fs_upcat_pad_fwd(a.data_ptr(), _p(b), out.data_ptr(), N, h, w, Ca, Cb, dtype_code(a.dtype),
                                              stream_ptr()), "upcat_pad_fwd"), tag=str(tuple(out.shape)))
    return out


def upcat_pad_bwd(dpad, h, w, Ca, Cb, bn=None):
    N = dpad.shape[0]
    da = torch.empty(N, h, w, Ca, dtype=dpad.dtype, device=dpad.device)
    db = torch.empty(N, 2 * h, 2 * w, Cb, dtype=dpad.dtype, device=dpad.device) if Cb else None
    nbytes = (da.numel() + (db.numel() if db is not None else 0) + dpad.numel()) * da.element_size()
    if bn is not None:
        y, x, st, sums = bn
        assert y.is_contiguous() and x.is_contiguous() and y.shape == da.shape == x.shape and st.groups == 1
        assert sums.dtype == torch.float64 and sums.numel() == STAT_SLOTS * 2 * Ca
        _timed("upcat_pad_bwd", nbytes + 2 * da.numel() * da.element_size(),
               lambda: check(lib.fs_upcat_pad_bwd_bn(dpad.data_ptr(), da.data_ptr(), _p(db), N, h, w, Ca, Cb, y.data_ptr(),
                                                     x.data_ptr(), st.mean.data_ptr(), st.invstd.data_ptr(), sums.data_ptr(),
                                                     dtype_code(dpad.dtype), stream_ptr()), "upcat_pad_bwd_bn"),
               tag=str(tuple(dpad.shape)) + " bn")
        return da, db
    _timed("upcat_pad_bwd", nbytes,
           lambda: check(lib.fs_upcat_pad_bwd(dpad.data_ptr(), da.data_ptr(), _p(db), N, h, w, Ca, Cb,
                                              dtype_code(dpad.dtype), stream_ptr()), "upcat_pad_bwd"),
           tag=str(tuple(dpad.shape)))
    return da, db


def channel_sum(x, out, creal):
    Cc = x.shape[-1]
    M = x.numel() // Cc
    _timed("channel_sum", x.numel() * x.element_size(),
           lambda: check(lib.fs_channel_sum(x.data_ptr(), out.data_ptr(), M, Cc, creal, dtype_code(x.dtype),
                                            stream_ptr()), "channel_sum"), tag=str(tuple(x.shape)))


def channel_sum_multi(items):
    items = list(items)
    if len(items) == 1:
        return channel_sum(*items[0])
    for i in range(0, len(items), 16):
        chunk = items[i:i + 16]
        n = len(chunk)
        code = dtype_code(chunk[0][0].dtype)
        assert all(dtype_code(x.dtype) == code for x, _, _ in chunk)
        xs = (C.c_void_p * n)(*[x.data_ptr() for x, _, _ in chunk])
        outs = (C.c_void_p * n)(*[o.data_ptr() for _, o, _ in chunk])
        Ms = (C.c_int64 * n)(*[x.numel() // x.shape[-1] for x, _, _ in chunk])
        Cs = (C.c_int32 * n)(*[x.shape[-1] for x, _, _ in chunk])
        Cr = (C.c_int32 * n)(*[int(cr) for _, _, cr in chunk])
        _timed("channel_sum", sum(x.numel() * x.element_size() for x, _, _ in chunk),
               lambda: check(lib.fs_channel_sum_multi(xs, outs, Ms, Cs, Cr, n, code, stream_ptr()), "channel_sum_multi"),
               tag="%d tensors" % n)


def depth_head_fwd(logits, bins, K, min_depth, max_depth):
    N, H, W, Cl = logits.shape
    depth = torch.empty(N, 1, H, W, dtype=torch.float32, device=logits.device)
    disp = torch.empty(N, 1, H, W, dtype=torch.float32, device=logits.device)
    check(lib.fs_depth_head_fwd(logits.data_ptr(), bins.data_ptr(), depth.data_ptr(), disp.data_ptr(), N * H * W, K,
                                Cl, float(min_depth), float(max_depth), stream_ptr()), "depth_head_fwd")
    return depth, disp


def depth_head_bwd(logits, bins, d_depth, d_disp, K, min_depth, max_depth, dtype):
    N, H, W, Cl = logits.shape
    dl = torch.empty(N, H, W, Cl, dtype=dtype, device=logits.device)
    check(lib.fs_depth_head_bwd(logits.data_ptr(), bins.data_ptr(), _p(d_depth), _p(d_disp), dl.data_ptr(),
                                N * H * W, K, Cl, float(min_depth), float(max_depth), dtype_code(dtype),
                                stream_ptr()), "depth_head_bwd")
    return dl


def _head_scale(hb, logits_list, P2, base_fx):
    if P2 is None or base_fx is None:
        return
    assert P2.is_cuda and P2.dtype == torch.float32 and P2.is_contiguous() and P2.shape[1:] == (3, 4)
    assert P2.shape[0] == logits_list[0].shape[0]
    hb.P2, hb.base_fx, hb.nimg = P2.data_ptr(), float(base_fx), P2.shape[0]


def depth_head_fwd_multi(logits_list, bins, K, min_depth, max_depth, P2=None, base_fx=None):
    from .binding import FsHeadBatch
    hb = FsHeadBatch()
    _head_scale(hb, logits_list, P2, base_fx)
    hb.n = len(logits_list)
    Cl = logits_list[0].shape[3]
    outs = []
    for s, lg in enumerate(logits_list):
        N, H, W, c = lg.shape
        assert c == Cl and lg.dtype == torch.float32 and lg.is_contiguous()
        depth = torch.empty(N, 1, H, W, dtype=torch.float32, device=lg.device)
        disp = torch.empty(N, 1, H, W, dtype=torch.float32, device=lg.device)
        hb.logits[s], hb.depth[s], hb.disp[s], hb.M[s] = lg.data_ptr(), depth.data_ptr(), disp.data_ptr(), N * H * W
        outs.append((depth, disp))
    check(lib.fs_depth_head_fwd_multi(C.byref(hb), bins.data_ptr(), K, Cl, float(min_depth), float(max_depth),
                                      stream_ptr()), "depth_head_fwd_multi")
    return outs


def depth_head_bwd_multi(logits_list, bins, d_depths, d_disps, K, min_depth, max_depth, dtype, P2=None, base_fx=None):
    from .binding import FsHeadBatch
    hb = FsHeadBatch()
    _head_scale(hb, logits_list, P2, base_fx)
    hb.n = len(logits_list)
    Cl = logits_list[0].shape[3]
    outs = []
    for s, lg in enumerate(logits_list):
        N, H, W, c = lg.shape
        assert c == Cl
        dl = torch.empty(N, H, W, Cl, dtype=dtype, device=lg.device)
        hb.logits[s], hb.dlogits[s], hb.M[s] = lg.data_ptr(), dl.data_ptr(), N * H * W
        hb.d_depth[s], hb.d_disp[s] = _p(d_depths[s]), _p(d_disps[s])
        outs.append(dl)
    check(lib.fs_depth_head_bwd_multi(C.byref(hb), bins.data_ptr(), K, Cl, float(min_depth), float(max_depth),
                                      dtype_code(dtype), stream_ptr()), "depth_head_bwd_multi")
    return outs


def pose_tail_fwd(x, nframes, invert, scale=0.01):
    B, h, w, Cx = x.shape
    aa = torch.empty(B, nframes, 1, 3, dtype=torch.float32, device=x.device)
    tr = torch.empty(B, nframes, 1, 3, dtype=torch.float32, device=x.device)
    T = torch.empty(B, 4, 4, dtype=torch.float32, device=x.device)
    check(lib.fs_pose_tail_fwd(x.data_ptr(), aa.data_ptr(), tr.data_ptr(), T.data_ptr(), B, h * w, Cx, nframes,
                               int(invert), float(scale), stream_ptr()), "pose_tail_fwd")
    return aa, tr, T


def pose_tail_bwd(x, dT, nframes, invert, dtype, scale=0.01, out=None):
    B, h, w, Cx = x.shape
    dx = torch.empty(B, h, w, Cx, dtype=dtype, device=x.device) if out is None else out
    assert dx.shape == x.shape and dx.is_contiguous() and dx.dtype == dtype and x.is_contiguous()
    check(lib.fs_pose_tail_bwd(x.data_ptr(), dT.data_ptr(), dx.data_ptr(), B, h * w, Cx, nframes, int(invert),
                               float(scale), dtype_code(dtype), stream_ptr()), "pose_tail_bwd")
    return dx


class PhotometricLoss:

    def __init__(self, B, H, W, scales, device, min_depth, max_depth, want_pred=True, overlapped_mask=True):
        self.B, self.H, self.W = B, H, W
        self.overlapped_mask = bool(overlapped_mask)
        self.scales = list(scales)
        S = self.S = len(self.scales)
        self.device = device
        f32, f64, u8 = torch.float32, torch.float64, torch.uint8
        self.geo = torch.zeros(B, 48, dtype=f32, device=device)
        self.want_pred = bool(want_pred)
        self.pred = self.ov = None
        if self.want_pred:
            self.pred = torch.empty(S, 2, B, 3, H, W, dtype=f32, device=device)
            self.ov = torch.empty(S, 2, B, H, W, dtype=u8, device=device)
        self.ident = torch.empty(B, 2, H, W, dtype=f32, device=device)
        self.sel = torch.empty(S, B, H, W, dtype=u8, device=device)
        self.n_acc = S * B + B + S * B + 2 * S * B + S * B
        self.acc = torch.zeros(self.n_acc, dtype=f64, device=device)
        o = 0
        self.loss_sums = self.acc[o:o + S * B]; o += S * B
        self.mask_sum = self.acc[o:o + B]; o += B
        self.disp_sum = self.acc[o:o + S * B]; o += S * B
        self.sm_sums = self.acc[o:o + 2 * S * B]; o += 2 * S * B
        self.dot = self.acc[o:o + S * B]
        self.out = torch.zeros(2 * S + 1, dtype=f64, device=device)
        self.hw = [(H >> s, W >> s) for s in self.scales]
        self.color = [None] * S
        self.bwd_tiles = int(lib.fs_photo_fused_bwd_tiles(H, W))
        self.dP = torch.zeros(self.S * B * self.bwd_tiles, 2, 12, dtype=f32, device=device)
        sizes = [B * h * w for (h, w) in self.hw]
        self._dd_flat = torch.zeros(sum(sizes), dtype=f32, device=device)
        self.d_depth, o = [], 0
        for n_el, (h, w) in zip(sizes, self.hw):
            self.d_depth.append(self._dd_flat[o:o + n_el].view(B, 1, h, w))
            o += n_el
        self.d_disp = [torch.empty(B, 1, h, w, dtype=f32, device=device) for (h, w) in self.hw]
        self.dT = [torch.zeros(B, 4, 4, dtype=f32, device=device) for _ in range(2)]
        self.pyr = [None if s == 0 else torch.empty(B, 3, H >> s, W >> s, dtype=f32, device=device)
                    for s in self.scales]
        lv = [i for i, s in enumerate(self.scales) if s != 0]
        self._pyr_n = len(lv)
        self._pyr_outs = (C.c_void_p * max(len(lv), 1))(*[self.pyr[i].data_ptr() for i in lv])
        self._pyr_hs = (C.c_int32 * max(len(lv), 1))(*[self.hw[i][0] for i in lv])
        self._pyr_ws = (C.c_int32 * max(len(lv), 1))(*[self.hw[i][1] for i in lv])
        self._pa = FsPhotoArgs()
        self._sa = FsSmoothArgs()
        self.seed_buf = torch.zeros(1, dtype=torch.int32, device=device)
        self._prefetched = None
        self.fisheye = False
        self.motion_mask = None
        self.lut_table = self.mei = self.warp_mask = None
        self._lut_keep = None
        self._clean_acc = self._clean_dd = False
        register_prezero(self, lambda o: o._prezero(), device)

    def stage_fisheye(self, tables, mei_rows):
        B, dev = self.B, self.device
        if self.lut_table is None:
            self.lut_table = torch.zeros(B, dtype=torch.int64, device=dev)
            self.mei = torch.zeros(B, 8, dtype=torch.float32, device=dev)
            self.warp_mask = torch.empty(B, self.H, self.W, dtype=torch.float32, device=dev)
        assert len(tables) == B and all(t.shape == (4, self.H, self.W) and t.is_contiguous() for t in tables)
        ptrs = [t.data_ptr() for t in tables]
        if self._lut_keep is not None and self._lut_keep[1] == ptrs and bool((self._lut_keep[2] == mei_rows).all()):
            self.fisheye = True
            return
        self.lut_table.copy_(torch.tensor(ptrs, dtype=torch.int64).pin_memory(), non_blocking=True)
        self.mei.copy_(torch.from_numpy(mei_rows.copy()).pin_memory(), non_blocking=True)
        self._lut_keep = (list(tables), ptrs, mei_rows.copy())
        self.fisheye = True

    def prefetch(self, img0, srcs, patched_mask):
        st = stream_ptr()
        pa = self._pa
        pa.img0 = img0.data_ptr()
        pa.img_src[0], pa.img_src[1] = srcs[0].data_ptr(), srcs[1].data_ptr()
        pa.patched_mask = _p(patched_mask)
        pa.ident, pa.mask_sum = self.ident.data_ptr(), self.mask_sum.data_ptr()
        pa.geo = self.geo.data_ptr()
        pa.B, pa.H, pa.W, pa.S = self.B, self.H, self.W, self.S
        self._input_only(img0, C.byref(pa), st)
        self._prefetched = (img0.data_ptr(), srcs[0].data_ptr(), srcs[1].data_ptr(), _p(patched_mask))

    def _prezero(self):
        self._clean_acc = self._clean_dd = True
        return [self.acc, self._dd_flat]

    def _input_only(self, img0, pa, st):
        if getattr(self, "_clean_acc", False):
            _join_pack(img0.device)
        else:
            self.acc.zero_()
        self._clean_acc = False
        if self._pyr_n:
            check(lib.fs_color_pyramid_multi(img0.data_ptr(), self._pyr_outs, self._pyr_hs, self._pyr_ws, self._pyr_n,
                                             self.B, self.H, self.W, st), "color_pyramid_multi")
        check(lib.fs_photo_identity_rows(pa, st), "photo_identity_rows")

    def _fill(self, img0, srcs, patched_mask, depths, disps, noise_seed, gout):
        pa, sa = self._pa, self._sa
        pa.img0 = img0.data_ptr()
        pa.img_src[0], pa.img_src[1] = srcs[0].data_ptr(), srcs[1].data_ptr()
        pa.patched_mask = _p(patched_mask)
        pa.geo = self.geo.data_ptr()
        pa.no_overlap_mask = 0 if self.overlapped_mask else 1
        pa.pred, pa.ov, pa.ident, pa.sel = _p(self.pred), _p(self.ov), self.ident.data_ptr(), self.sel.data_ptr()
        pa.loss_sums, pa.mask_sum = self.loss_sums.data_ptr(), self.mask_sum.data_ptr()
        pa.dP = self.dP.data_ptr()
        pa.gout = _p(gout)
        pa.B, pa.H, pa.W, pa.S = self.B, self.H, self.W, self.S
        pa.noise_seed = -1 if noise_seed is None else int(noise_seed)
        pa.noise_seed_ptr = self.seed_buf.data_ptr() if noise_seed is None else None
        if self.fisheye:
            pa.lut_ptrs, pa.mei, pa.warp_mask = self.lut_table.data_ptr(), self.mei.data_ptr(), self.warp_mask.data_ptr()
        else:
            pa.lut_ptrs = pa.mei = pa.warp_mask = None
        pa.motion_mask = _p(self.motion_mask)
        sa.disp_sum, sa.sm_sums, sa.dot = self.disp_sum.data_ptr(), self.sm_sums.data_ptr(), self.dot.data_ptr()
        sa.gout = _p(gout)
        sa.B, sa.S = self.B, self.S
        for i, (h, w) in enumerate(self.hw):
            pa.depth[i] = depths[i].data_ptr()
            pa.dh[i], pa.dw[i] = h, w
            pa.d_depth[i] = self.d_depth[i].data_ptr()
            sa.disp[i] = disps[i].data_ptr()
            sa.color[i] = (img0 if self.scales[i] == 0 else self.pyr[i]).data_ptr()
            sa.d_disp[i] = self.d_disp[i].data_ptr()
# ... 590 lines not shown
```

fsnet_amd/hip/signatures.py:

```python
import ctypes as C

P = C.c_void_p
I = C.c_int
L = C.c_int64
F = C.c_float
D = C.c_double

SIGNATURES = {
    "fs_abi_version": (C.c_int, []),
    "fs_target_arch": (C.c_char_p, []),
    "fs_debug_timestamp": (C.c_int, [P, P]),
    "fs_capture_position": (C.c_int, [P, P]),
    "fs_conv_igemm": (C.c_int, [P, I, P]),
    "fs_conv_igemm2": (C.c_int, [P, P, I, P]),
    "fs_conv3x3_halo2": (C.c_int, [P, P, I, P]),
    "fs_conv3x3_halo2_plan": (C.c_int, [P, P, I, P]),
    "fs_conv3x3_s2d": (C.c_int, [P, I, P]),
    "fs_conv3x3_s2d2": (C.c_int, [P, P, I, P]),
    "fs_conv_stem2": (C.c_int, [P, P, I, P]),
    "fs_conv_wgrad2": (C.c_int, [P, P, I, P]),
    "fs_conv_wgrad2_plan": (C.c_int, [P, P, I, P]),
    "fs_bn_apply2": (C.c_int, [P, P, I, P]),
    "fs_bn_bwd_reduce2": (C.c_int, [P, P, I, P]),
    "fs_bn_bwd_apply2": (C.c_int, [P, P, I, P]),
    "fs_maxpool_fwd2": (C.c_int, [P, P, P, I, P, P, P, I, I, I, I, I, P]),
    "fs_maxpool_bwd2": (C.c_int, [P, P, P, P, I, P, P, P, P, I, I, I, I, I, P]),
    "fs_conv3x3_halo": (C.c_int, [P, I, P]),
    "fs_conv3x3_halo_plan": (C.c_int, [P, I, P]),
    "fs_conv1x1": (C.c_int, [P, I, P]),
    "fs_conv_stem": (C.c_int, [P, I, P]),
    "fs_conv_wgrad": (C.c_int, [P, I, P]),
    "fs_conv_wgrad_plan": (C.c_int, [P, I, P]),
    "fs_pack_weights": (C.c_int, [P, P, I, I, I, I, I, I, L, I, I, P]),
    "fs_sigmoid_head_fwd": (C.c_int, [P, P, L, I, P]),
    "fs_sigmoid_head_bwd": (C.c_int, [P, P, P, L, I, I, P]),
    "fs_distill_fwd": (C.c_int, [P, P, P, L, P, P]),
    "fs_distill_bwd": (C.c_int, [P, P, P, L, P, P, P, P]),
    "fs_resize_linear": (C.c_int, [P, P, I, I, I, I, I, P]),
    "fs_depth_eval": (C.c_int, [P, P, I, I, I, I, I, P, P, P]),
    "fs_depth_eval_masked": (C.c_int, [P, P, P, I, I, I, I, I, F, F, I, P, P, P]),
    "fs_lidar_mei_depth": (C.c_int, [P, P, L, P, P, I, I, I, P, P, P, L, P]),
    "fs_lidar_mei_depth_workspace_bytes": (C.c_int64, [I, I, I]),
    "fs_lidar_pinhole_depth": (C.c_int, [P, P, L, P, I, I, I, P, P, L, P]),
    "fs_lidar_pinhole_depth_workspace_bytes": (C.c_int64, [I, I, I]),
    "fs_lidar_nusc_depth_u16": (C.c_int, [P, P, L, P, I, I, I, I, P, P, L, P]),
    "fs_lidar_nusc_depth_workspace_bytes": (C.c_int64, [I, I, I, I]),
    "fs_depth_errors9": (C.c_int, [P, P, I, I, D, I, I, I, P, L, P, P]),
    "fs_depth_errors9_workspace_bytes": (C.c_int64, [I, I, I]),
    "fs_depth_quantize_u16": (C.c_int, [P, P, F, I, I, P]),
    "fs_cost_volume": (C.c_int, [P, P, P, P, P, P, P, P, P, P, P, I, I, I, I, I, I, I, I, P]),
    "fs_postopt": (C.c_int, [P, P]),
    "fs_postopt_workspace_bytes": (C.c_int64, [I, I, I, I]),
    "fs_optflow_farneback": (C.c_int, [P, P]),
    "fs_optflow_workspace_bytes": (C.c_int64, [P]),
    "fs_optflow_level_image": (C.c_int, [P, I, P, P]),
    "fs_motion_mask": (C.c_int, [P, P]),
    "fs_augment_masks": (C.c_int, [P, P, P, P, P, I, I, I, I, I, P]),
    "fs_copy_multi": (C.c_int, [P, P, P, I, P]),
    "fs_zero_multi": (C.c_int, [P, P, I, P]),
    "fs_pack_tile_blocks": (C.c_int64, [C.c_int, C.c_int, C.c_int, C.c_int]),
    "fs_pack_weights_multi": (C.c_int, [P, I, L, I, P]),
    "fs_nchw_to_nhwc": (C.c_int, [P, P, P, I, I, I, I, I, I, I, P]),
    "fs_bn_apply": (C.c_int, [P, I, P]),
    "fs_bn_finalize": (C.c_int, [P, P, P, P]),
    "fs_bn_bwd_reduce": (C.c_int, [P, I, P]),
    "fs_bn_bwd_apply": (C.c_int, [P, I, P]),
    "fs_maxpool_fwd": (C.c_int, [P, P, P, I, I, I, I, I, P]),
    "fs_maxpool_bwd": (C.c_int, [P, P, P, P, I, I, I, I, I, P]),
    "fs_upcat_pad_fwd": (C.c_int, [P, P, P, I, I, I, I, I, I, P]),
    "fs_upcat_pad_bwd": (C.c_int, [P, P, P, I, I, I, I, I, I, P]),
    "fs_upcat_pad_bwd_bn": (C.c_int, [P, P, P, I, I, I, I, I, P, P, P, P, P, I, P]),
    "fs_channel_sum": (C.c_int, [P, P, L, I, I, I, P]),
    "fs_channel_sum_multi": (C.c_int, [P, P, P, P, P, I, I, P]),
    "fs_depth_head_fwd": (C.c_int, [P, P, P, P, L, I, I, F, F, P]),
    "fs_depth_head_bwd": (C.c_int, [P, P, P, P, P, L, I, I, F, F, I, P]),
    "fs_depth_head_fwd_multi": (C.c_int, [P, P, I, I, F, F, P]),
    "fs_depth_head_bwd_multi": (C.c_int, [P, P, I, I, F, F, I, P]),
    "fs_pose_tail_fwd": (C.c_int, [P, P, P, P, I, I, I, I, I, F, P]),
    "fs_pose_tail_bwd": (C.c_int, [P, P, P, I, I, I, I, I, F, I, P]),
    "fs_photo_setup": (C.c_int, [P, P, P, P, I, P, I, P]),
    "fs_mei_lut": (C.c_int, [P, I, I, F, F, F, F, D, D, D, P]),
    "fs_mei_stage_mask": (C.c_int, [P, P, P, I, I, I, P]),
    "fs_mei_points": (C.c_int, [P, P, P, I, I, I, P]),
    "fs_photo_identity": (C.c_int, [P, P]),
    "fs_photo_identity_rows": (C.c_int, [P, P]),
    "fs_photo_identity_strip_rows": (C.c_int, []),
    "fs_photo_fused_fwd": (C.c_int, [P, P]),
    "fs_photo_fused_bwd": (C.c_int, [P, P]),
    "fs_photo_fused_bwd_tiles": (C.c_int64, [I, I]),
    "fs_photo_pose_grad": (C.c_int, [P, P, P, P, I, I, I, P]),
    "fs_augment_frames": (C.c_int, [P, P]),
    "fs_resize_frames": (C.c_int, [P, P]),
    "fs_augment_frames_masked": (C.c_int, [P, P, P]),
    "fs_resize_frames_masked": (C.c_int, [P, P, P]),
    "fs_color_pyramid": (C.c_int, [P, P, I, I, I, I, I, P]),
    "fs_color_pyramid_multi": (C.c_int, [P, P, P, P, I, I, I, I, P]),
    "fs_smooth_mean": (C.c_int, [P, P]),
    "fs_smooth_fwd": (C.c_int, [P, P]),
    "fs_smooth_bwd": (C.c_int, [P, P]),
    "fs_loss_finalize": (C.c_int, [P, P, P, P, P, P, P]),
    "fs_sumsq": (C.c_int, [P, L, P, P, P]),
    "fs_counter_incr": (C.c_int, [P, P]),
    "fs_adam_step": (C.c_int, [P, P, P, P, L, F, F, F, F, F, I, F, P, F, P, P, P]),
    "fs_adamw_step": (C.c_int, [P, P, P, P, L, F, F, F, F, F, I, I, F, P, F, P, P, P, I, P]),
    "fs_sgd_step": (C.c_int, [P, P, P, L, F, F, F, I, F, I, F, P, F, P, P, P, I, P]),
}


def declare(lib):
    for name, (res, args) in SIGNATURES.items():
        fn = getattr(lib, name)
        fn.restype = res
        fn.argtypes = args
```

include/fsnet_hip.h:

```cpp
#ifndef FSNET_HIP_H
#define FSNET_HIP_H
#include <stdint.h>

#ifdef __cplusplus
extern "C" {
#endif

#define FS_OK 0
#define FS_EINVAL 1
#define FS_ELAUNCH 2

#define FS_DTYPE_F32 0
#define FS_DTYPE_BF16 1

#define FS_STAT_SLOTS 8

#define FS_ABI_VERSION 15
int fs_abi_version(void);
const char* fs_target_arch(void);
int fs_debug_timestamp(void* slot, void* stream);
int fs_capture_position(void* stream, unsigned long long* token);

typedef struct FsConvArgs {
  const void* src;
// ... 117 lines not shown

#define FS_AUG_IPLAN 8
#define FS_AUG_FPLAN 4
typedef struct FsAugArgs {
  const uint8_t* src;
  const double* minv;
  const int32_t* iplan;
  const float* fplan;
  float* image;
  float* original;
  double* mask;
  float mean[3];
  float std[3];
  int32_t B, F, Hs, Ws, H, W;
} FsAugArgs;
int fs_augment_frames(const FsAugArgs* args, void* stream);

typedef struct FsResizeArgs {
  const uint8_t* src;
  const int32_t* dims;
  float* image;
  float mean[3];
  float std[3];
  int32_t B, F, Hs, Ws, H, W;
  const int32_t* iplan;
  const float* fplan;
  float* original;
  double* mask;
} FsResizeArgs;
int fs_resize_frames(const FsResizeArgs* args, void* stream);

int fs_augment_frames_masked(const FsAugArgs* args, const uint8_t* mask_src, void* stream);
int fs_resize_frames_masked(const FsResizeArgs* args, const uint8_t* mask_src, void* stream);

int fs_resize_linear(const float* src, float* dst, int h, int w, int H, int W, int invert, void* stream);
int fs_depth_eval(const float* pred, const float* gt, int B, int h, int w, int H, int W, void* scratch,
                  double* out16, void* stream);
int fs_depth_eval_masked(const float* pred, const float* gt, const uint8_t* mask, int B, int h, int w, int H, int W,
                         float lo, float hi, int crop, void* scratch, double* out16, void* stream);

int fs_lidar_mei_depth(const float* points, const int64_t* offsets, int64_t n_points, const double* T,
                       const double* mei, int G, int H, int W, float* depth, uint8_t* close_mask, void* workspace,
                       int64_t workspace_bytes, void* stream);
int64_t fs_lidar_mei_depth_workspace_bytes(int G, int H, int W);

int fs_lidar_pinhole_depth(const float* points, const int64_t* offsets, int64_t n_points, const double* P, int G, int H,
                           int W, float* depth, void* workspace, int64_t workspace_bytes, void* stream);
int64_t fs_lidar_pinhole_depth_workspace_bytes(int G, int H, int W);

int fs_lidar_nusc_depth_u16(const float* points, const int64_t* offsets, int64_t n_points, const double* M, int G, int C,
                            int H, int W, void* depth_u16, void* workspace, int64_t workspace_bytes, void* stream);
int64_t fs_lidar_nusc_depth_workspace_bytes(int G, int C, int H, int W);

int fs_depth_errors9(const void* pred, const void* gt, int pred_is_u16, int gt_is_u16, double scale, int N, int H, int W,
                     void* workspace, int64_t workspace_bytes, double* out, void* stream);
int64_t fs_depth_errors9_workspace_bytes(int N, int H, int W);
int fs_depth_quantize_u16(const float* depth, void* out, float scale, int H, int W, void* stream);

typedef struct FsPostOptArgs {
  const float* image;
  const float* depth;
  const float* vo;
  const float* centres;
  float* out;
  int32_t* labels;
  int32_t* nseg;
  void* workspace;
  int64_t workspace_bytes;
  double rgb_mean[3];
  double rgb_std[3];
  float lab_dist_weight, depth_dist_weight, image_dist_weight;
  double lambda0, lambda1, lambda2;
  int32_t B, H, W, K, iter_num, max_points;
} FsPostOptArgs;
int fs_postopt(const FsPostOptArgs* args, void* stream);
int64_t fs_postopt_workspace_bytes(int B, int H, int W, int K);

typedef struct FsFlowArgs {
  const uint8_t* img0;
  const uint8_t* img1;
  float* flow;
  void* workspace;
  int64_t workspace_bytes;
  double pyr_scale;
  double poly_sigma;
  int32_t B, H, W, levels, winsize, iterations, poly_n, flags;
} FsFlowArgs;
int fs_optflow_farneback(const FsFlowArgs* args, void* stream);
int64_t fs_optflow_workspace_bytes(const FsFlowArgs* args);
int fs_optflow_level_image(const FsFlowArgs* args, int level, float* out, void* stream);

typedef struct FsMotionMaskArgs {
  const float* flow;
  const double* P2;
  const double* pose;
  uint8_t* mask;
  float threshold;
  int32_t mode;
  int32_t B, H, W;
} FsMotionMaskArgs;
int fs_motion_mask(const FsMotionMaskArgs* args, void* stream);

int fs_augment_masks(const uint8_t* src, const double* minv, const int32_t* dims, const int32_t* iplan, float* out,
                     int B, int Hs, int Ws, int H, int W, void* stream);

#define FS_COPY_MAX 16
int fs_copy_multi(const void* const* src, void* const* dst, const int64_t* bytes, int n, void* stream);
int fs_zero_multi(void* const* dst, const int64_t* bytes, int n, void* stream);

int fs_cost_volume(const void* cur, const void* look, const float* K, const float* inv_K, const float* poses,
                   const float* bins, void* cat, float* confidence, float* lowest, float* cost_f32, float* missing,
                   int B, int F, int h, int w, int C, int D, int Ci_p, int dtype, void* stream);

int fs_nchw_to_nhwc(const float* a, const float* b, void* dst, int N, int Ca, int Cb, int H, int W,
                    int Cp, int dtype, void* stream);

typedef struct FsBnApplyArgs {
  const void* x;
  const void* res;
  void* y;
  const double* stats;  const double* stats2;
  const float* gamma;   const float* beta;
  const float* gamma2;  const float* beta2;
  float* running_mean;  float* running_var;
  float* running_mean2; float* running_var2;
  int64_t* num_batches_tracked; int64_t* num_batches_tracked2;
  float* save_mean;  float* save_invstd;
  float* save_mean2; float* save_invstd2;
  double count;
  float eps, momentum;
  int64_t yN, yH, yW;
  int32_t M, C, H, W;
  int32_t relu, pad_out;
  int32_t groups;
  void* pool_y; uint8_t* pool_idx;
} FsBnApplyArgs;
int fs_bn_apply(const FsBnApplyArgs* args, int dtype, void* stream);
int fs_bn_apply2(const FsBnApplyArgs* a0, const FsBnApplyArgs* a1, int dtype, void* stream);
int fs_bn_finalize(const FsBnApplyArgs* args, float* scale, float* shift, void* stream);

typedef struct FsBnBwdArgs {
  const void* dout; const void* y; const void* x;
  void* dx; void* g_out;
  double* sums; const double* sums_local;
  const float* gamma; const float* save_mean; const float* save_invstd;
  float* dgamma; float* dbeta;
  double count;
  int64_t gN, gH, gW;
  int64_t yN, yH, yW;
  int32_t M, C, H, W;
  int32_t relu, fold;
  int32_t groups;
  const void* pool_dy; const uint8_t* pool_idx; const float* beta;
} FsBnBwdArgs;
int fs_bn_bwd_reduce(const FsBnBwdArgs* args, int dtype, void* stream);
int fs_bn_bwd_apply(const FsBnBwdArgs* args, int dtype, void* stream);
int fs_bn_bwd_reduce2(const FsBnBwdArgs* a0, const FsBnBwdArgs* a1, int dtype, void* stream);
int fs_bn_bwd_apply2(const FsBnBwdArgs* a0, const FsBnBwdArgs* a1, int dtype, void* stream);

int fs_maxpool_fwd(const void* x, void* y, uint8_t* idx, int N, int H, int W, int C, int dtype, void* stream);
int fs_maxpool_bwd(const void* dy, const uint8_t* idx, const void* addend, void* dx, int N, int H, int W, int C,
                   int dtype, void* stream);
int fs_maxpool_fwd2(const void* x, void* y, uint8_t* idx, int N, const void* x1, void* y1, uint8_t* idx1, int N1, int H,
                    int W, int C, int dtype, void* stream);
int fs_maxpool_bwd2(const void* dy, const uint8_t* idx, const void* addend, void* dx, int N, const void* dy1,
                    const uint8_t* idx1, const void* addend1, void* dx1, int N1, int H, int W, int C, int dtype,
                    void* stream);
int fs_upcat_pad_fwd(const void* a, const void* b, void* out, int N, int h, int w, int Ca, int Cb, int dtype,
                     void* stream);
int fs_upcat_pad_bwd(const void* dpad, void* da, void* db, int N, int h, int w, int Ca, int Cb, int dtype,
                     void* stream);
int fs_upcat_pad_bwd_bn(const void* dpad, void* da, void* db, int N, int h, int w, int Ca, int Cb, const void* y,
                        const void* x, const float* mean, const float* invstd, double* sums, int dtype, void* stream);
int fs_channel_sum(const void* x, float* out, int64_t M, int C, int Creal, int dtype, void* stream);
int fs_channel_sum_multi(const void* const* x, float* const* out, const int64_t* M, const int32_t* C, const int32_t* Creal,
                         int n, int dtype, void* stream);

int fs_depth_head_fwd(const float* logits, const float* bins, float* depth, float* disp, int64_t M, int K, int Cl,
                      float min_depth, float max_depth, void* stream);
int fs_depth_head_bwd(const float* logits, const float* bins, const float* d_depth, const float* d_disp,
                      void* dlogits, int64_t M, int K, int Cl, float min_depth, float max_depth, int dtype,
                      void* stream);

#define FS_HEAD_MAX 4
typedef struct FsHeadBatch {
  const float* logits[4];
  float* depth[4];
  float* disp[4];
  const float* d_depth[4];
  const float* d_disp[4];
  void* dlogits[4];
  int64_t M[4];
  int32_t n;
  int32_t nimg;
  const float* P2;
  float base_fx;
  int32_t reserved;
} FsHeadBatch;
int fs_depth_head_fwd_multi(const FsHeadBatch* batch, const float* bins, int K, int Cl, float min_depth,
                            float max_depth, void* stream);
int fs_depth_head_bwd_multi(const FsHeadBatch* batch, const float* bins, int K, int Cl, float min_depth,
                            float max_depth, int dtype, void* stream);

int fs_pose_tail_fwd(const float* x, float* axisangle, float* translation, float* T, int B, int hw, int Cx,
                     int nframes, int invert, float scale, void* stream);
int fs_pose_tail_bwd(const float* x, const float* dT, void* dx, int B, int hw, int Cx, int nframes, int invert,
                     float scale, int dtype, void* stream);

typedef struct FsPhotoArgs {
  const float* img0;
  const float* img_src[2];
  const double* patched_mask;
  const float* depth[4];
  const float* geo;
  float* pred;
  uint8_t* ov;
  float* ident;
  uint8_t* sel;
  double* loss_sums;
  double* mask_sum;
  float* d_depth[4];
  float* dP;
  const double* gout;
  int32_t dh[4], dw[4];
  int32_t B, H, W, S;
  int32_t noise_seed;
  const int32_t* noise_seed_ptr;
  const float* const* lut_ptrs;
  const float* mei;
  const float* warp_mask;
  const float* motion_mask;
  int32_t no_overlap_mask;
  int32_t reserved0;
} FsPhotoArgs;
int fs_photo_setup(const float* P2, const float* T0, const float* T1, float* geo, int B, int* seed_counter,
                   int fisheye, void* stream);
int fs_photo_identity(const FsPhotoArgs* args, void* stream);
int fs_photo_identity_rows(const FsPhotoArgs* args, void* stream);
int fs_photo_identity_strip_rows(void);
int fs_photo_fused_fwd(const FsPhotoArgs* args, void* stream);
int fs_photo_fused_bwd(const FsPhotoArgs* args, void* stream);
int64_t fs_photo_fused_bwd_tiles(int H, int W);
int fs_photo_pose_grad(const float* geo, const float* dP, float* dT0, float* dT1, int B, int S, int tiles,
                       void* stream);

int fs_mei_lut(float* lut, int H, int W, float gamma1, float gamma2, float u0, float v0, double k1, double k2,
               double xi, void* stream);
int fs_mei_stage_mask(const float* const* lut_ptrs, const double* patched_mask, float* warp_mask, int B, int H, int W,
                      void* stream);
int fs_mei_points(const float* const* lut_ptrs, const float* norm, float* points, int B, int H, int W, void* stream);

typedef struct FsSmoothArgs {
  const float* disp[4];
  const float* color[4];
  float* d_disp[4];
  double* disp_sum;
  double* sm_sums;
  double* dot;
  const double* gout;
  int32_t h[4], w[4], scale_id[4];
  int32_t B, S;
} FsSmoothArgs;
int fs_color_pyramid(const float* img, float* out, int B, int H, int W, int h, int w, void* stream);
int fs_color_pyramid_multi(const float* img, float* const* outs, const int32_t* hs, const int32_t* ws, int n, int B,
                           int H, int W, void* stream);
int fs_smooth_mean(const FsSmoothArgs* args, void* stream);
int fs_smooth_fwd(const FsSmoothArgs* args, void* stream);
int fs_smooth_bwd(const FsSmoothArgs* args, void* stream);
int fs_loss_finalize(const double* loss_sums, const double* mask_sum, const double* sm_sums,
                     const FsSmoothArgs* args, double* out, double* total_out, void* stream);

int fs_sumsq(const float* g, int64_t n, double* out, int* step_counter, void* stream);
int fs_counter_incr(int32_t* counter, void* stream);
int fs_adam_step(float* p, const float* g, float* m, float* v, int64_t n, float lr, float beta1, float beta2,
                 float eps, float weight_decay, int step, float max_norm, const double* sumsq, float grad_scale,
                 const int32_t* step_ptr, const float* lr_ptr, void* stream);
#define FS_MAX_RUNS 4096
int fs_adamw_step(float* p, const float* g, float* m, float* v, int64_t n, float lr, float beta1, float beta2,
                  float eps, float weight_decay, int decoupled, int step, float max_norm, const double* sumsq,
                  float grad_scale, const int32_t* step_ptr, const float* lr_ptr, const int64_t* runs, int n_runs,
                  void* stream);
int fs_sgd_step(float* p, const float* g, float* buf, int64_t n, float lr, float momentum, float dampening,
                int nesterov, float weight_decay, int step, float max_norm, const double* sumsq, float grad_scale,
                const int32_t* step_ptr, const float* lr_ptr, const int64_t* runs, int n_runs, void* stream);

#ifdef __cplusplus
}
#endif
#endif
```

Before: 2346 samples/s.

## Fuse conv bias gradient reduction into BN-backward apply and depth-head backward kernels

The BN backward apply kernel and the depth-head backward kernel now accumulate per-channel sums of the gradient they write, rounded to bf16 the same way it is stored, and add them atomically into double slot buffers. A small fold kernel then reduces the slots into the bias gradients. This replaces the separate channel_sum passes that re-read the full gradient tensors. The cost is extra shared-memory reductions and double atomics in the apply kernels, capped head grids, and new slot buffers. The path is on by default through an environment flag.

```diff
diff --git a/fsnet_amd/csrc/bn.hip b/fsnet_amd/csrc/bn.hip
--- a/fsnet_amd/csrc/bn.hip
+++ b/fsnet_amd/csrc/bn.hip
@@ -657,7 +657,42 @@
   reduce_tail<V>(p, red, s1, s2, z, CGB, cgl, pl, c, act);
 }
 
-template <typename T, bool POOL = false>
+template <typename T>
+__device__ __forceinline__ void store_summed(T* p, const float* o, float* acc) {
+  constexpr int V = VecN<T>::N;
+  const uint4 u = Unit<T>::pack(o);
+  *reinterpret_cast<uint4*>(p) = u;
+  float r[V];
+  Unit<T>::unpack(u, r);
+#pragma unroll
+  for (int j = 0; j < V; ++j) acc[j] += r[j];
+}
+
+template <int V>
+__device__ __forceinline__ void bias_tail(double* slot, const float* bs, float* smem, int SCG, int scg_sh) {
+  const int t = threadIdx.x, SC = SCG * V, parts = 256 / SC;
+  float* red = smem;
+  float* red2 = smem + V * 256;
+  __syncthreads();
+#pragma unroll
+  for (int j = 0; j < V; ++j) red[j * 256 + t] = bs[j];
+  __syncthreads();
+  {
+    const int cl = t & (SC - 1), part = t / SC, g = cl / V, j = cl % V;
+    float acc = 0.f;
+#pragma unroll
+    for (int k = 0; k < V; ++k) acc += red[j * 256 + ((part * V + k) << scg_sh) + g];
+    red2[t] = acc;
+  }
+  __syncthreads();
+  if (t < SC) {
+    float acc = 0.f;
+    for (int k = 0; k < parts; ++k) acc += red2[k * SC + t];
+    atomicAdd(slot + t, (double)acc);
+  }
+}
+
+template <typename T, bool POOL = false, bool BIAS = false>
 __global__ __launch_bounds__(256) void bn_bwd_apply_kernel(const FsDual<FsBnBwdArgs, FsNoGeom> d) {
   extern __shared__ float bn_smem[];
   int G, z;
@@ -690,9 +725,14 @@
   T* __restrict__ dx = reinterpret_cast<T*>(p.dx);
   T* __restrict__ gout = reinterpret_cast<T*>(p.g_out);
   const long stride = (long)gridDim.x * 256;
+  float bs[V];
+#pragma unroll
+  for (int j = 0; j < V; ++j) bs[j] = 0.f;
+  bool dense_done = false;
   if constexpr (!POOL) {
     if (scg_sh >= 0 && dense_grad(p)) {
-      if (i0 >= total) return;
+      const bool has = i0 < total;
+      if (!BIAS && !has) return;
       const int cl = (int)(i0 & (SCG - 1)) * V;
       const long rows = stride >> scg_sh, step = rows * C;
       long off = ((long)z * Mg + (i0 >> scg_sh)) * C + c0 + cl;
@@ -714,10 +754,11 @@
       float g[V], xr[V], o[V];
 #pragma unroll
       for (int j = 0; j < V; ++j) { g[j] = pg[j]; xr[j] = px[j]; }
-      for (;;) {
+      if (has) for (;;) {
 #pragma unroll
         for (int j = 0; j < V; ++j) o[j] = bn_dx(g[j], xr[j], km[j], ki[j], kk[j], ka[j], kb[j]);
-        storev<T>(dx + off, o);
+        if constexpr (BIAS) store_summed<T>(dx + off, o, bs);
+        else storev<T>(dx + off, o);
         if (gout) storev<T>(gout + off, g);
         if (--left == 0) break;
         off += step;
@@ -734,10 +775,11 @@
           if (relu) y2 = *reinterpret_cast<const uint4*>(yv + off + 2 * step);
         }
       }
-      return;
-    }
-  }
-  for (long i = i0; i < total; i += stride) {
+      if constexpr (!BIAS) return;
+      dense_done = true;
+    }
+  }
+  if (!dense_done) for (long i = i0; i < total; i += stride) {
     int cg; long m;
     split_vec(i, SCG, scg_sh, cg, m);
     m += (long)z * Mg;
@@ -756,8 +798,13 @@
     if constexpr (POOL) pool_mask<T>(p, yv, m, c, xr, s_k + cl, bn_smem + 5 * SC + cl, g);
 #pragma unroll
     for (int j = 0; j < V; ++j) o[j] = bn_dx(g[j], xr[j], s_mean[cl + j], s_istd[cl + j], s_k[cl + j], s_a[cl + j], s_b[cl + j]);
-    storev<T>(dx + m * C + c, o);
+    if constexpr (BIAS) store_summed<T>(dx + m * C + c, o, bs);
+    else storev<T>(dx + m * C + c, o);
     if (gout) storev<T>(gout + m * C + c, g);
+  }
+  if constexpr (BIAS) {
+    if (!p.bias_slots || (long)blockIdx.x * 256 >= total) return;
+    bias_tail<V>(p.bias_slots + (long)(blockIdx.x % FS_STAT_SLOTS) * C + c0, bs, bn_smem, SCG, scg_sh);
   }
 }
 
@@ -809,6 +856,7 @@
   if (a->C % 8 != 0 || a->C > MAXC || a->M <= 0) return FS_EINVAL;
   const int G = bn_groups(*a);
   if (a->M % G != 0) return FS_EINVAL;
+  if (a->bias_slots && (!apply || a->pool_dy)) return FS_EINVAL;
   if (a->pool_dy) {
     if (!a->pool_idx || !a->gamma || a->fold || a->g_out || a->H <= 0 || a->W <= 0 || (a->H & 1) || (a->W & 1)) return FS_EINVAL;
     if (a->relu && !a->y && !a->beta) return FS_EINVAL;
@@ -945,6 +993,13 @@
   }
   const long items = pr.larger([&](const FsBnBwdArgs& x, int G) { return (long)(x.M / G) * (x.C / vec); });
   dim3 grid(std::min(grid_for(items / nslab), std::max(32, grid_for(1L << 40) / nslab)), nslab, nz);
+  if (a->bias_slots || (b && b->bias_slots)) {
+    if ((CG & (CG - 1)) != 0 || (dtype != FS_DTYPE_BF16 && dtype != FS_DTYPE_F32)) return FS_EINVAL;
+    const unsigned blds = std::max<unsigned>(lds, (vec + 1) * 256u * sizeof(float));
+    return by_dtype(dtype, [&](auto e) {
+      hipLaunchKernelGGL((bn_bwd_apply_kernel<typename decltype(e)::type, false, true>), grid, dim3(256), blds, st, pr.d);
+    });
+  }
   return by_dtype(dtype, [&](auto e) {
     using T = typename decltype(e)::type;
     if (a->pool_dy) hipLaunchKernelGGL((bn_bwd_apply_kernel<T, true>), grid, dim3(256), lds, st, pr.d);
diff --git a/fsnet_amd/csrc/heads.hip b/fsnet_amd/csrc/heads.hip
--- a/fsnet_amd/csrc/heads.hip
+++ b/fsnet_amd/csrc/heads.hip
@@ -32,11 +32,24 @@
   disp[m] = (1.f / d - 1.f / max_d) * inv_rng;
 }
 
-template <int K, typename T>
+template <typename T> __device__ __forceinline__ void store4_summed(T* p, const float v[4], float* acc);
+template <> __device__ __forceinline__ void store4_summed<float>(float* p, const float v[4], float* acc) {
+  store4<float>(p, v);
+#pragma unroll
+  for (int j = 0; j < 4; ++j) acc[j] += v[j];
+}
+template <> __device__ __forceinline__ void store4_summed<bf16>(bf16* p, const float v[4], float* acc) {
+  uint2 t; t.x = pack_bf16x2(v[0], v[1]); t.y = pack_bf16x2(v[2], v[3]);
+  *reinterpret_cast<uint2*>(p) = t;
+  acc[0] += bf16_bits_to_f(t.x & 0xffffu); acc[1] += __uint_as_float(t.x & 0xffff0000u);
+  acc[2] += bf16_bits_to_f(t.y & 0xffffu); acc[3] += __uint_as_float(t.y & 0xffff0000u);
+}
+
+template <int K, typename T, bool BIAS = false>
 __device__ __forceinline__ void head_bwd_row(const float* __restrict__ logits, const float* sb,
                                              const float* __restrict__ d_depth, const float* __restrict__ d_disp,
                                              T* __restrict__ dlogits, long m, int Cl, float inv_rng,
-                                             float sc = 0.f, float min_d = 0.f, float max_d = 0.f) {
+                                             float sc = 0.f, float min_d = 0.f, float max_d = 0.f, float* acc = nullptr) {
   float v[K], raw[K];
   float mx = -INFINITY;
 #pragma unroll
@@ -64,7 +77,10 @@
     o[k] = inside ? pk * (sb[k] - d) * g : 0.f;
   }
 #pragma unroll
-  for (int k = 0; k < K; k += 4) store4<T>(dlogits + m * Cl + k, &o[k]);
+  for (int k = 0; k < K; k += 4) {
+    if constexpr (BIAS) store4_summed<T>(dlogits + m * Cl + k, &o[k], acc + k);
+    else store4<T>(dlogits + m * Cl + k, &o[k]);
+  }
 }
 
 template <int K>
@@ -114,7 +130,7 @@
   }
 }
 
-template <int K, typename T>
+template <int K, typename T, bool BIAS = false>
 __global__ __launch_bounds__(256) void depth_head_bwd_multi_kernel(const FsHeadBatch hb, const HeadBlocks blk,
                                                                    const float* __restrict__ bins, int Cl, float min_d,
                                                                    float max_d) {
@@ -126,6 +142,31 @@
   while (s + 1 < hb.n && (int)blockIdx.x >= blk.start[s + 1]) ++s;
   const long nb = blk.start[s + 1] - blk.start[s], lb = blockIdx.x - blk.start[s];
   const long rows_img = hb.nimg > 0 ? hb.M[s] / hb.nimg : 0;
+  if constexpr (BIAS) {
+    if (hb.bias_slots[s]) {
+      __shared__ float wsum[4][K];
+      float acc[K];
+#pragma unroll
+      for (int k = 0; k < K; ++k) acc[k] = 0.f;
+      for (long m = lb * 256 + threadIdx.x; m < hb.M[s]; m += nb * 256) {
+        const float sc = hb.P2 ? hb.P2[(m / rows_img) * 12] / hb.base_fx : 0.f;
+        head_bwd_row<K, T, true>(hb.logits[s], sb, hb.d_depth[s], hb.d_disp[s], reinterpret_cast<T*>(hb.dlogits[s]), m, Cl,
+                                 inv_rng, sc, min_d, max_d, acc);
+      }
+#pragma unroll
+      for (int k = 0; k < K; ++k) {
+        const float w = wave_sum(acc[k]);
+        if ((threadIdx.x & 63) == 0) wsum[threadIdx.x >> 6][k] = w;
+      }
+      __syncthreads();
+      if (threadIdx.x < K) {
+        const int k = threadIdx.x;
+        const float a = (wsum[0][k] + wsum[1][k]) + (wsum[2][k] + wsum[3][k]);
+        atomicAdd(hb.bias_slots[s] + (lb % FS_STAT_SLOTS) * Cl + k, (double)a);
+      }
+      return;
+    }
+  }
   for (long m = lb * 256 + threadIdx.x; m < hb.M[s]; m += nb * 256) {
     const float sc = hb.P2 ? hb.P2[(m / rows_img) * 12] / hb.base_fx : 0.f;
     head_bwd_row<K, T>(hb.logits[s], sb, hb.d_depth[s], hb.d_disp[s], reinterpret_cast<T*>(hb.dlogits[s]), m, Cl, inv_rng,
@@ -270,6 +311,7 @@
 }
 
 namespace {
+constexpr int HEAD_BIAS_BLOCKS = 128 * FS_STAT_SLOTS;
 bool head_blocks(const FsHeadBatch* hb, bool bwd, HeadBlocks& blk, int& total) {
   if (!hb || hb->n < 1 || hb->n > FS_HEAD_MAX) return false;
   if (hb->P2 && (hb->nimg < 1 || !(hb->base_fx > 0.f))) return false;
@@ -279,7 +321,7 @@
     if (hb->P2 && hb->M[s] % hb->nimg != 0) return false;
     if (bwd ? !hb->dlogits[s] : (!hb->depth[s] || !hb->disp[s])) return false;
     blk.start[s] = total;
-    total += grid_for(hb->M[s]);
+    total += (bwd && hb->bias_slots[s]) ? std::min(grid_for(hb->M[s]), HEAD_BIAS_BLOCKS) : grid_for(hb->M[s]);
   }
   blk.start[hb->n] = total;
   return true;
@@ -305,6 +347,18 @@
   if (!bins || Cl < K || !head_blocks(hb, true, blk, total)) return FS_EINVAL;
   hipStream_t st = reinterpret_cast<hipStream_t>(stream);
   dim3 grid(total);
+  bool bias = false;
+  for (int s = 0; s < hb->n; ++s) bias = bias || hb->bias_slots[s] != nullptr;
+  if (bias) {
+#define FS_DHB(KK, TT) hipLaunchKernelGGL((depth_head_bwd_multi_kernel<KK, TT, true>), grid, dim3(256), 0, st, *hb, blk, bins, Cl, min_depth, max_depth)
+    if (dtype == FS_DTYPE_BF16) {
+      if (K == 16) FS_DHB(16, bf16); else if (K == 32) FS_DHB(32, bf16); else return FS_EINVAL;
+    } else if (dtype == FS_DTYPE_F32) {
+      if (K == 16) FS_DHB(16, float); else if (K == 32) FS_DHB(32, float); else return FS_EINVAL;
+    } else return FS_EINVAL;
+#undef FS_DHB
+    return fs_launch_status();
+  }
 #define FS_DHM(KK, TT) hipLaunchKernelGGL((depth_head_bwd_multi_kernel<KK, TT>), grid, dim3(256), 0, st, *hb, blk, bins, Cl, min_depth, max_depth)
   if (dtype == FS_DTYPE_BF16) {
     if (K == 16) FS_DHM(16, bf16); else if (K == 32) FS_DHM(32, bf16); else if (K == 64) FS_DHM(64, bf16); else return FS_EINVAL;
diff --git a/fsnet_amd/csrc/pool_upsample.hip b/fsnet_amd/csrc/pool_upsample.hip
--- a/fsnet_amd/csrc/pool_upsample.hip
+++ b/fsnet_amd/csrc/pool_upsample.hip
@@ -298,11 +298,35 @@
   channel_sum_body<T, VL>(reinterpret_cast<const T*>(c.x[k]), c.out[k], c.M[k], c.C[k], c.Creal[k], c.CGB[k], lb % gx, lb / gx, gx);
 }
 
+struct FoldBatch { const double* slots[FS_CSUM_MAX]; float* out[FS_CSUM_MAX]; int C[FS_CSUM_MAX], Creal[FS_CSUM_MAX]; };
+__global__ __launch_bounds__(256) void bias_fold_multi_kernel(const FoldBatch f) {
+  const int k = blockIdx.x, C = f.C[k];
+  const double* __restrict__ sl = f.slots[k];
+  for (int c = threadIdx.x; c < f.Creal[k]; c += 256) {
+    double a = 0.0;
+#pragma unroll
+    for (int s = 0; s < FS_STAT_SLOTS; ++s) a += sl[(long)s * C + c];
+    atomicAdd(f.out[k] + c, (float)a);
+  }
+}
+
 int grid_for(long items) {
   long b = (items + 255) / 256;
   return (int)std::max<long>(1, std::min<long>(b, 8192));
 }
 
+}
+
+extern "C" int fs_bias_fold_multi(const double* const* slots, float* const* out, const int32_t* C, const int32_t* Creal,
+                                  int n, void* stream) {
+  if (!slots || !out || !C || !Creal || n < 1 || n > FS_CSUM_MAX) return FS_EINVAL;
+  FoldBatch f;
+  for (int i = 0; i < n; ++i) {
+    if (!slots[i] || !out[i] || C[i] <= 0 || Creal[i] < 0 || Creal[i] > C[i]) return FS_EINVAL;
+    f.slots[i] = slots[i]; f.out[i] = out[i]; f.C[i] = C[i]; f.Creal[i] = Creal[i];
+  }
+  hipLaunchKernelGGL(bias_fold_multi_kernel, dim3(n), dim3(256), 0, reinterpret_cast<hipStream_t>(stream), f);
+  return fs_launch_status();
 }
 
 #define DISPATCH(KERNEL, GRID, ...)                                                                   \
diff --git a/fsnet_amd/engine/nets.py b/fsnet_amd/engine/nets.py
--- a/fsnet_amd/engine/nets.py
+++ b/fsnet_amd/engine/nets.py
@@ -45,9 +45,11 @@
             return None
         return self.buf[oa:ob + b.numel()]
 
-    def take(self, C, groups=1):
-        n = groups * STAT_SLOTS * 2 * C
-        shape = (STAT_SLOTS, 2, C) if groups == 1 else (groups, STAT_SLOTS, 2, C)
+    def take(self, C, groups=1, kinds=2):
+        n = groups * STAT_SLOTS * kinds * C
+        shape = (STAT_SLOTS, kinds, C) if groups == 1 else (groups, STAT_SLOTS, kinds, C)
+        if kinds == 1:
+            shape = shape[:-2] + (C,)
         if self.off + n > self.buf.numel():
             return torch.zeros(shape, dtype=torch.float64, device=self.buf.device)
         v = self.buf[self.off:self.off + n].view(shape)
@@ -79,13 +81,14 @@
 
 def _run_param_grads(*item, bias_later=None):
     lanes = item[1] if item[0] == "lanes" else [item]
-    run_specs([op.wgrad_spec(dc, x, gw, pro=pro) for (op, dc, x, gw, gb, nb, pro) in lanes])
-    for (op, dc, x, gw, gb, nb, pro) in lanes:
+    run_specs([op.wgrad_spec(dc, x, gw, pro=pro) for (op, dc, x, gw, gb, nb, pro, slots) in lanes])
+    for (op, dc, x, gw, gb, nb, pro, slots) in lanes:
         if gb is not None:
+            src = dc if slots is None else slots
             if bias_later is not None:
-                bias_later.append((dc, gb, nb))
+                bias_later.append((src, gb, nb))
             else:
-                ops.channel_sum(dc, gb, nb)
+                ops.bias_grads_multi([(src, gb, nb)])
 
 
 _INLINE_BIAS = {}
@@ -110,7 +113,7 @@
             continue
         chain, items = ent
         with torch.cuda.stream(chain):
-            ops.channel_sum_multi(items)
+            ops.bias_grads_multi(items)
         items.clear()
 
 
@@ -123,7 +126,7 @@
             if gb is not None:
                 ops.channel_sum(dc, gb, cl.m.bias.numel())
             continue
-        lanes.append((op, dc, x, gw, gb, cl.m.bias.numel() if gb is not None else 0, pro))
+        lanes.append((op, dc, x, gw, gb, cl.m.bias.numel() if gb is not None else 0, pro, None))
     if not lanes:
         return
     item = lanes[0] if len(lanes) == 1 else ("lanes", lanes)
@@ -178,7 +181,7 @@
         for it in mine:
             _run_param_grads(*it, bias_later=sums)
         if sums:
-            ops.channel_sum_multi(sums)
+            ops.bias_grads_multi(sums)
         if RT._marks is not None:
             RT.mark(tag + ".end(%d)" % len(mine))
     _PENDING_JOIN.add((chain, ws))
@@ -352,7 +355,7 @@
             for it in items:
                 _run_param_grads(*it, bias_later=sums)
             if sums:
-                ops.channel_sum_multi(sums)
+                ops.bias_grads_multi(sums)
             runner.tail_pending = False
             if RT.dp is not None and runner.m._pending == 0:
                 RT.dp.grads_ready(runner.m)
@@ -511,14 +514,14 @@
     def bias(self):
         return self._bias
 
-    def accumulate_param_grads(self, op, dc, x, pro=None):
+    def accumulate_param_grads(self, op, dc, x, pro=None, bias_slots=None):
         gw = grad_of(self.m.weight)
         gb = grad_of(self.m.bias) if self.m.bias is not None else None
         if gw is None:
             if gb is not None:
-                ops.channel_sum(dc, gb, self.m.bias.numel())
+                ops.bias_grads_multi([(dc if bias_slots is None else bias_slots, gb, self.m.bias.numel())])
             return
-        item = (op, dc, x, gw, gb, self.m.bias.numel() if gb is not None else 0, pro)
+        item = (op, dc, x, gw, gb, self.m.bias.numel() if gb is not None else 0, pro, bias_slots if gb is not None else None)
         if _TAIL_SINK[0] is not None:
             _TAIL_SINK[0].append(item)
             return
@@ -564,7 +567,26 @@
     return _BWD_POOLS[(c.device, raw_stream(c.device.index))].take(c.shape[-1], st.groups)
 
 
-def _bn_bwd(dout, y, c, bn, st, H, W, relu=True, fold=False, g_out=None, sums=None):
+BIAS_BYPRODUCT = os.environ.get("FSNET_AMD_BIAS_BYPRODUCT", "1").strip().lower() not in ("0", "off", "false", "no")
+
+
+def _bias_slots(C, device):
+    p = _BWD_POOLS.get((device, raw_stream(device.index)))
+    if p is not None and p.epoch == ops.PREZERO_EPOCH[0]:
+        return p.take(C, kinds=1)
+    return torch.zeros(STAT_SLOTS, C, dtype=torch.float64, device=device)
+
+
+def _bias_byproduct(cl, c, pow2=True):
+    if not BIAS_BYPRODUCT or cl.m.bias is None or grad_of(cl.m.bias) is None or not c.is_cuda:
+        return None
+    lanes = c.shape[-1] * c.element_size() // 16
+    if pow2 and (lanes < 1 or lanes & (lanes - 1) or c.dtype not in (torch.bfloat16, torch.float32)):
+        return None
+    return _bias_slots(c.shape[-1], c.device)
+
+
+def _bn_bwd(dout, y, c, bn, st, H, W, relu=True, fold=False, g_out=None, sums=None, bias_slots=None):
     dc = torch.empty_like(c)
     reduced = sums is not None
     if sums is None:
@@ -572,7 +594,7 @@
     sync = RT.dp is not None and st.count != float("inf")
     ops.bn_backward(dout, y, c, bn.weight.data, st, dc, grad_of(bn.weight), grad_of(bn.bias), H, W, relu=relu,
                     fold=fold, g_out=g_out, sums=sums, sums_zeroed=True, reduced=reduced,
-                    allreduce=(RT.dp.allreduce_small if sync else None))
+                    allreduce=(RT.dp.allreduce_small if sync else None), bias_slots=bias_slots)
     return dc
 
 
@@ -1197,7 +1219,7 @@
         feats = ctx["feats"]
 
         sc = [i for i in range(5) if i in m.scales and (g_depth.get(i) is not None or g_disp.get(i) is not None)]
-        dls = {}
+        dls, head_slots = {}, {}
         if sc and getattr(m, "sigmoid_head", False):
             a, bq = 1.0 / float(m.max_depth), 1.0 / float(m.min_depth) - 1.0 / float(m.max_depth)
             for i in sc:
@@ -1207,10 +1229,12 @@
                     du = du - g_depth[i] * depth * (bq / (a + bq * u))
                 dls[i] = ops.sigmoid_head_bwd(u, du, self.disp[i].ready(dt, dev).Co_p, dt)
         elif sc:
+            hsl = [_bias_byproduct(self.disp[i], ctx["lv"][i]["logits"], pow2=False) if K <= 32 else None for i in sc]
             res = ops.depth_head_bwd_multi([ctx["lv"][i]["logits"] for i in sc], m.depth_bins,
                                            [g_depth.get(i) for i in sc], [g_disp.get(i) for i in sc], K, m.min_depth,
-                                           m.max_depth, dt, P2=ctx["P2"], base_fx=ctx["base_fx"])
+                                           m.max_depth, dt, P2=ctx["P2"], base_fx=ctx["base_fx"], bias_slots=hsl)
             dls = dict(zip(sc, res))
+            head_slots = dict(zip(sc, hsl))
 
         def disp_grad(i):
             lv = ctx["lv"][i]
@@ -1220,7 +1244,7 @@
                 cld = self.disp[i]
                 opd = cld.ready(dt, dev)
                 dl = dls[i]
-                cld.accumulate_param_grads(opd, dl, y1p)
+                cld.accumulate_param_grads(opd, dl, y1p, bias_slots=head_slots.get(i))
                 G = opd.dgrad(dl, y1p.shape[1], y1p.shape[2])
             if i in self.unc and g_unc.get(i) is not None:
                 clu = self.unc[i]
@@ -1244,8 +1268,9 @@
             cl1, bn1 = self.up1[i]
             op1 = cl1.ready(dt, dev)
             y1_int = lv["y1p"][:, 1:-1, 1:-1]
-            dc1 = _bn_bwd(Gp, y1_int, lv["c1"], bn1, lv["s1"], H2, W2, relu=True, fold=True)
-            cl1.accumulate_param_grads(op1, dc1, lv["xcat"])
+            sl1 = _bias_byproduct(cl1, lv["c1"])
+            dc1 = _bn_bwd(Gp, y1_int, lv["c1"], bn1, lv["s1"], H2, W2, relu=True, fold=True, bias_slots=sl1)
+            cl1.accumulate_param_grads(op1, dc1, lv["xcat"], bias_slots=sl1)
             dxcat = op1.dgrad(dc1, H2 + 2, W2 + 2)
             cl0, bn0 = self.up0[i]
             op0 = cl0.ready(dt, dev)
@@ -1253,8 +1278,9 @@
             d_y0, d_skip = ops.upcat_pad_bwd(dxcat, h, w, op0.Co_p, lv["Cs"], bn=(lv["y0"], lv["c0"], lv["s0"], sums0))
             if i > 0 and lv["Cs"]:
                 gfeats[i - 1] = d_skip
-            dc0 = _bn_bwd(d_y0, None, lv["c0"], bn0, lv["s0"], h, w, sums=sums0)
-            cl0.accumulate_param_grads(op0, dc0, lv["x"])
+            sl0 = _bias_byproduct(cl0, lv["c0"])
+            dc0 = _bn_bwd(d_y0, None, lv["c0"], bn0, lv["s0"], h, w, sums=sums0, bias_slots=sl0)
+            cl0.accumulate_param_grads(op0, dc0, lv["x"], bias_slots=sl0)
             if i < 4:
                 Gp, fresh = disp_grad(i + 1)
                 interior = Gp[:, 1:-1, 1:-1]
diff --git a/fsnet_amd/hip/binding.py b/fsnet_amd/hip/binding.py
--- a/fsnet_amd/hip/binding.py
+++ b/fsnet_amd/hip/binding.py
@@ -83,7 +83,7 @@
         ("logits", C.c_void_p * 4), ("depth", C.c_void_p * 4), ("disp", C.c_void_p * 4),
         ("d_depth", C.c_void_p * 4), ("d_disp", C.c_void_p * 4), ("dlogits", C.c_void_p * 4),
         ("M", C.c_int64 * 4), ("n", C.c_int32), ("nimg", C.c_int32), ("P2", C.c_void_p), ("base_fx", C.c_float),
-        ("reserved", C.c_int32),
+        ("reserved", C.c_int32), ("bias_slots", C.c_void_p * 4),
     ]
 
 
@@ -126,6 +126,7 @@
         ("M", C.c_int32), ("C", C.c_int32), ("H", C.c_int32), ("W", C.c_int32),
         ("relu", C.c_int32), ("fold", C.c_int32), ("groups", C.c_int32),
         ("pool_dy", C.c_void_p), ("pool_idx", C.c_void_p), ("beta", C.c_void_p),
+        ("bias_slots", C.c_void_p),
     ]
 
 
diff --git a/fsnet_amd/hip/ops.py b/fsnet_amd/hip/ops.py
--- a/fsnet_amd/hip/ops.py
+++ b/fsnet_amd/hip/ops.py
@@ -107,15 +107,16 @@
 
 
 def bn_backward(dout, y, x, gamma, st, dx, dgamma, dbeta, H, W, relu=True, fold=False, g_out=None, sums=None,
-                allreduce=None, sums_zeroed=False, reduced=False, phase="all", glob=None, pool=None):
+                allreduce=None, sums_zeroed=False, reduced=False, phase="all", glob=None, pool=None, bias_slots=None):
     bn_backward_multi([dict(dout=dout, y=y, x=x, gamma=gamma, st=st, dx=dx, dgamma=dgamma, dbeta=dbeta, H=H, W=W, relu=relu,
-                            fold=fold, g_out=g_out, sums=sums, sums_zeroed=sums_zeroed, reduced=reduced, glob=glob, pool=pool)],
+                            fold=fold, g_out=g_out, sums=sums, sums_zeroed=sums_zeroed, reduced=reduced, glob=glob, pool=pool,
+                            bias_slots=bias_slots)],
                       allreduce=allreduce, phase=phase)
     return None if phase == "reduce" else dx
 
 
 def _bn_bwd_call(dout, y, x, gamma, st, dx, dgamma, dbeta, H, W, relu=True, fold=False, g_out=None, sums=None,
-                 sums_zeroed=False, reduced=False, glob=None, pool=None):
+                 sums_zeroed=False, reduced=False, glob=None, pool=None, bias_slots=None):
     if reduced:
         assert sums is not None and not fold and g_out is None
         relu, y = False, None
@@ -133,6 +134,9 @@
     else:
         assert dout is not None
     a.sums = sums.data_ptr()
+    if bias_slots is not None:
+        assert bias_slots.dtype == torch.float64 and bias_slots.is_contiguous() and bias_slots.numel() == STAT_SLOTS * Cc
+        a.bias_slots = bias_slots.data_ptr()
     a.gamma, a.save_mean, a.save_invstd = gamma.data_ptr(), st.mean.data_ptr(), st.invstd.data_ptr()
     a.dgamma, a.dbeta = _p(dgamma), _p(dbeta)
     a.count = st.count
@@ -152,8 +156,13 @@
 def bn_backward_multi(calls, allreduce=None, phase="all", span=None):
     cs = [_bn_bwd_call(**c) for c in calls]
     if phase != "apply":
+        slots = [c["a"].bias_slots for c in cs]
+        for c in cs:
+            c["a"].bias_slots = None
         run_specs([Spec(["bn_bwd_reduce"], c["a"], c["code"], "bn_bwd_reduce", c["nb"] * (1 + c["has_dout"] + c["has_y"]), c["shp"], None,
                         "bn_bwd_reduce") for c in cs if not c["reduced"]])
+        for c, sl in zip(cs, slots):
+            c["a"].bias_slots = sl
     if phase == "reduce":
         return
     pending = [c for c in cs if c["glob"] is None] if allreduce is not None else []
@@ -269,6 +278,31 @@
                                             stream_ptr()), "channel_sum"), tag=str(tuple(x.shape)))
 
 
+def bias_fold_multi(items):
+    items = list(items)
+    for i in range(0, len(items), 16):
+        chunk = items[i:i + 16]
+        n = len(chunk)
+        for sl, o, cr in chunk:
+            assert sl.dtype == torch.float64 and sl.is_contiguous() and sl.shape[0] == STAT_SLOTS and o.dtype == torch.float32
+        sls = (C.c_void_p * n)(*[sl.data_ptr() for sl, _, _ in chunk])
+        outs = (C.c_void_p * n)(*[o.data_ptr() for _, o, _ in chunk])
+        Cs = (C.c_int32 * n)(*[sl.numel() // STAT_SLOTS for sl, _, _ in chunk])
+        Cr = (C.c_int32 * n)(*[int(cr) for _, _, cr in chunk])
+        _timed("bias_fold", sum(sl.numel() * 8 for sl, _, _ in chunk),
+               lambda: check(lib.fs_bias_fold_multi(sls, outs, Cs, Cr, n, stream_ptr()), "bias_fold_multi"),
+               tag=lambda: "%d layers: C = %s" % (n, " ".join(str(sl.numel() // STAT_SLOTS) for sl, _, _ in chunk)))
+
+
+def bias_grads_multi(items):
+    folds = [it for it in items if it[0].dtype == torch.float64]
+    sums = [it for it in items if it[0].dtype != torch.float64]
+    if folds:
+        bias_fold_multi(folds)
+    if sums:
+        channel_sum_multi(sums)
+
+
 def channel_sum_multi(items):
     items = list(items)
     if len(items) == 1:
@@ -285,7 +319,7 @@
         Cr = (C.c_int32 * n)(*[int(cr) for _, _, cr in chunk])
         _timed("channel_sum", sum(x.numel() * x.element_size() for x, _, _ in chunk),
                lambda: check(lib.fs_channel_sum_multi(xs, outs, Ms, Cs, Cr, n, code, stream_ptr()), "channel_sum_multi"),
-               tag="%d tensors" % n)
+               tag=lambda: "%d tensors: %s" % (n, " ".join(str(tuple(x.shape)).replace(" ", "") for x, _, _ in chunk)))
 
 
 def depth_head_fwd(logits, bins, K, min_depth, max_depth):
@@ -333,7 +367,8 @@
     return outs
 
 
-def depth_head_bwd_multi(logits_list, bins, d_depths, d_disps, K, min_depth, max_depth, dtype, P2=None, base_fx=None):
+def depth_head_bwd_multi(logits_list, bins, d_depths, d_disps, K, min_depth, max_depth, dtype, P2=None, base_fx=None,
+                         bias_slots=None):
     from .binding import FsHeadBatch
     hb = FsHeadBatch()
     _head_scale(hb, logits_list, P2, base_fx)
@@ -346,6 +381,10 @@
         dl = torch.empty(N, H, W, Cl, dtype=dtype, device=lg.device)
         hb.logits[s], hb.dlogits[s], hb.M[s] = lg.data_ptr(), dl.data_ptr(), N * H * W
         hb.d_depth[s], hb.d_disp[s] = _p(d_depths[s]), _p(d_disps[s])
+        if bias_slots is not None and bias_slots[s] is not None:
+            sl = bias_slots[s]
+            assert sl.dtype == torch.float64 and sl.is_contiguous() and sl.numel() == STAT_SLOTS * Cl
+            hb.bias_slots[s] = sl.data_ptr()
         outs.append(dl)
     check(lib.fs_depth_head_bwd_multi(C.byref(hb), bins.data_ptr(), K, Cl, float(min_depth), float(max_depth),
                                       dtype_code(dtype), stream_ptr()), "depth_head_bwd_multi")
diff --git a/fsnet_amd/hip/signatures.py b/fsnet_amd/hip/signatures.py
--- a/fsnet_amd/hip/signatures.py
+++ b/fsnet_amd/hip/signatures.py
@@ -72,6 +72,7 @@
     "fs_upcat_pad_bwd_bn": (C.c_int, [P, P, P, I, I, I, I, I, P, P, P, P, P, I, P]),
     "fs_channel_sum": (C.c_int, [P, P, L, I, I, I, P]),
     "fs_channel_sum_multi": (C.c_int, [P, P, P, P, P, I, I, P]),
+    "fs_bias_fold_multi": (C.c_int, [P, P, P, P, I, P]),
     "fs_depth_head_fwd": (C.c_int, [P, P, P, P, L, I, I, F, F, P]),
     "fs_depth_head_bwd": (C.c_int, [P, P, P, P, P, L, I, I, F, F, I, P]),
     "fs_depth_head_fwd_multi": (C.c_int, [P, P, I, I, F, F, P]),
diff --git a/include/fsnet_hip.h b/include/fsnet_hip.h
--- a/include/fsnet_hip.h
+++ b/include/fsnet_hip.h
@@ -293,6 +293,7 @@
   int32_t relu, fold;
   int32_t groups;
   const void* pool_dy; const uint8_t* pool_idx; const float* beta;
+  double* bias_slots;
 } FsBnBwdArgs;
 int fs_bn_bwd_reduce(const FsBnBwdArgs* args, int dtype, void* stream);
 int fs_bn_bwd_apply(const FsBnBwdArgs* args, int dtype, void* stream);
@@ -316,6 +317,8 @@
 int fs_channel_sum(const void* x, float* out, int64_t M, int C, int Creal, int dtype, void* stream);
 int fs_channel_sum_multi(const void* const* x, float* const* out, const int64_t* M, const int32_t* C, const int32_t* Creal,
                          int n, int dtype, void* stream);
+int fs_bias_fold_multi(const double* const* slots, float* const* out, const int32_t* C, const int32_t* Creal, int n,
+                       void* stream);
 
 int fs_depth_head_fwd(const float* logits, const float* bins, float* depth, float* disp, int64_t M, int K, int Cl,
                       float min_depth, float max_depth, void* stream);
@@ -337,6 +340,7 @@
   const float* P2;
   float base_fx;
   int32_t reserved;
+  double* bias_slots[4];
 } FsHeadBatch;
 int fs_depth_head_fwd_multi(const FsHeadBatch* batch, const float* bins, int K, int Cl, float min_depth,
                             float max_depth, void* stream);
```

New measurement: 2352 samples/s (median of 6 runs). Within noise of the previous version (+0.3%).
